# YuvalBahat/Explorable-Super-Resolution

Measured on AMD Instinct MI355X. Metric: HR pixels/sec (RRDB-23 x4, 128->512, bs32 per GPU, fwd + CEM), higher is better.
Workload: dtype bf16x3 (bf16 hi+lo operands = 16 significand bits per operand in every product, three MFMAs, f32 accumulate)

## Files before the change

### explorable-super-resolution_amd/csrc/esr_conv.hip

```cpp
#include "esr_common.h"
#include <type_traits>
#include <vector>

namespace {

constexpr int NW = 4;
constexpr int NTHREADS = 64 * NW;
constexpr int MAXS_BASE = 3;
constexpr int WGS_MT1 = 2, WGS_MT2 = 2;
constexpr int r_of(int mt) { return 3; }
constexpr int maxs_of(int mt) { return r_of(mt) > 3 ? MAXS_BASE + 1 : MAXS_BASE; }

typedef __attribute__((ext_vector_type(4))) unsigned int u32x4;
constexpr int EPI_RES1 = 1, EPI_RES2 = 2, EPI_MASK = 4, EPI_NCHW = 8, EPI_OUT2 = 16;
constexpr int EPI_RESIN = 32;
constexpr int EPI_PS = 64;

struct ConvArgs {
    int tiles_x, tiles_y, ntiles;
    int xcd_q, xcd_r;
    unsigned m_tx, m_ty;
    unsigned i_tx, i_ty;
    int TH, TW, P, NPIX_T, NPIX_L, nslots;
    unsigned m_P, m_ups;
    int H, W, Win_p, ups;
    unsigned share[NW];
    int ncp, lo_chunks, reverse, B;
    DView in0, in1;
    const uint4* wpack;
    long long wchunk;
    long long wslice;
    int wtap;
    int nslices;
    const float* zero_bias;
    int bias_stride;
    const float* bias;
    int cout, ncg_out;
    float act_slope, alpha, beta1, beta2;
    DView res1, res2, out, out2, mask;
    float* out_nchw;
    int mask_cg0, mask_cg1;
    float mask_slope;
    int resin_g0;
    float resin_scale;
    int ps, ps_rg0;
    unsigned m_ns, i_ns;
    int ph_off;
    int ksplit, kz_groups;
    long long kz_slab;
    int nchw_ctot;
    int stages_hint;
    unsigned* range_flag;
    unsigned range_tag;
#ifdef ESR_TRACE
    unsigned long long* trace;
#endif
};

typedef __attribute__((ext_vector_type(8))) _Float16 f16x8;
typedef __attribute__((ext_vector_type(2))) float f32x2;
template <int FMT>
__device__ __forceinline__ f32x16 mfma(uint4 a, uint4 b, f32x16 c) {
    if (FMT) return __builtin_amdgcn_mfma_f32_32x32x16_f16(__builtin_bit_cast(f16x8, a), __builtin_bit_cast(f16x8, b), c, 0, 0, 0);
    return __builtin_amdgcn_mfma_f32_32x32x16_bf16(__builtin_bit_cast(bf16x8, a), __builtin_bit_cast(bf16x8, b), c, 0, 0, 0);
}
template <int FMT>
__device__ __forceinline__ uint32_t cvt_pk(float lo, float hi);

__device__ __forceinline__ uint32_t cvt_pk_bf16(float lo, float hi) {
    uint32_t r;
    asm("v_cvt_pk_bf16_f32 %0, %1, %2" : "=v"(r) : "v"(lo), "v"(hi));
    return r;
}
template <> __device__ __forceinline__ uint32_t cvt_pk<0>(float lo, float hi) { return cvt_pk_bf16(lo, hi); }
template <> __device__ __forceinline__ uint32_t cvt_pk<1>(float lo, float hi) { return f2h(lo) | (f2h(hi) << 16); }

__device__ __forceinline__ void glds16s(const uint4* sbase, unsigned voff, unsigned lds_dst) {
    asm volatile("s_mov_b32 m0, %2\n\ts_nop 0\n\tglobal_load_lds_dwordx4 %0, %1" : : "v"(voff), "s"(sbase), "s"(__builtin_amdgcn_readfirstlane(lds_dst)) : "memory");
}

__device__ __forceinline__ unsigned udiv_magic(unsigned n, unsigned m, unsigned i) { return __umulhi(n, m) + n * i; }

__device__ __forceinline__ const uint4* in_plane(const ConvArgs& a, int g, int b, bool lo) {
    if (g < a.in0.ncg) return (lo ? a.in0.lo : a.in0.hi) + b * a.in0.bs + g * a.in0.cs;
    int g1 = g - a.in0.ncg;
    if (g1 >= a.in1.ncg) g1 = 0;
    return (lo ? a.in1.lo : a.in1.hi) + b * a.in1.bs + g1 * a.in1.cs;
}

template <int MAXS>
struct FetchState {
    unsigned soff[MAXS];
    int slot[MAXS];
};

template <int MAXS>
__device__ __forceinline__ FetchState<MAXS> setup_tile(const ConvArgs& a, int x0, int y0, int wave, int lane) {
    FetchState<MAXS> f;
#pragma unroll
    for (int s = 0; s < MAXS; ++s) {
        f.slot[s] = (wave + s * NW) < a.nslots ? wave + s * NW : wave;
        const unsigned p = (unsigned)f.slot[s] * 64 + lane;
        const unsigned rr = __umul24(p, a.m_P) >> 20, cc = p - rr * a.P;
        const unsigned Yp = y0 + rr, Xp = x0 + cc;
        const bool inb = (p < (unsigned)a.NPIX_T) && (Yp < (unsigned)a.H + 2) && (Xp < (unsigned)a.W + 2);
        const unsigned sy = __umul24(Yp + a.ups - 1, a.m_ups) >> 16, sx = __umul24(Xp + a.ups - 1, a.m_ups) >> 16;
        f.soff[s] = p >= (unsigned)a.NPIX_L ? ~0u : (inb ? (sy * a.Win_p + sx) * 16 : 0);
    }
    return f;
}

template <int NPL>
struct Bases {
    const uint4* p[2 * NPL];
    const uint4* w;
    int wtap;
};
template <int NPL, int MT, int NPW>
__device__ __forceinline__ Bases<NPL> make_bases(const ConvArgs& a, int cp, int b) {
    Bases<NPL> r;
#pragma unroll
    for (int i = 0; i < 2 * NPL; ++i) r.p[i] = in_plane(a, 2 * cp + i / NPL, b, (i % NPL) == 1);
    r.w = a.wpack + (size_t)cp * a.wchunk;
    r.wtap = a.wtap;
    return r;
}

struct DmaShare {
    int nsl;
    int w0, wc;
};
__device__ __forceinline__ DmaShare unpack_share(unsigned w) { return DmaShare{(int)(w & 0xFF), (int)((w >> 8) & 0xFF), (int)(w >> 16)}; }
template <int NPL, int MT = 1, int NPW = 1, int TMODE = 0>
__device__ __forceinline__ int dma_count(const DmaShare& d, bool xlo) { return (xlo ? 2 * NPL : 2) * d.nsl + (TMODE != 0 ? MT * NPW : d.wc); }

template <int NPL, int MT, int NPW, int TMODE = 0>
__device__ __forceinline__ void dma_chunk(const FetchState<maxs_of(MT)>& f, const Bases<NPL>& bs, const DmaShare& d, unsigned stage, int plane_bytes, bool xlo,
                                          int tsel = 0, int wave = 0) {
    constexpr int MAXS = maxs_of(MT);
#pragma unroll
    for (int s = 0; s < MAXS; ++s) {
        if (s >= d.nsl) break;
        const unsigned dst = stage + (unsigned)f.slot[s] * 1024;
        if (f.soff[s] != ~0u) {
#pragma unroll
            for (int cgpl = 0; cgpl < 2 * NPL; ++cgpl) {
                if (!xlo && (cgpl % NPL) == 1) continue;
                glds16s(bs.p[cgpl], f.soff[s], dst + cgpl * plane_bytes);
            }
        }
    }
    const unsigned vlane = (unsigned)(threadIdx.x & 63) * 16;
    if constexpr (TMODE == 0 && MT == 1) {
        for (int j = d.w0; j < d.w0 + d.wc; ++j) glds16s(bs.w + ((j / NPW) * bs.wtap + j % NPW) * 64, vlane, stage + 2 * NPL * plane_bytes + j * 1024);
    } else if constexpr (TMODE == 0) {
        for (int j = d.w0; j < d.w0 + d.wc; ++j) glds16s(bs.w + j * 64, vlane, stage + 2 * NPL * plane_bytes + j * 1024);
    } else {
        static_assert(TMODE == 0 || NW == 4, "one live tap per wave");
#pragma unroll
        for (int m = 0; m < MT; ++m) {
            const int r0 = TMODE == 1 ? 1 - (tsel >> 1) : tsel, c0 = TMODE == 1 ? 1 - (tsel & 1) : m;
            const int tap = (r0 + (wave >> 1)) * 3 + c0 + (wave & 1);
#pragma unroll
            for (int pl = 0; pl < NPW; ++pl) {
                const int j = (tap * MT + m) * NPW + pl;
                glds16s(bs.w + j * 64, vlane, stage + 2 * NPL * plane_bytes + j * 1024);
            }
        }
    }
}

template <int MAXN>
__device__ __forceinline__ void wait_vm_upto(int n) {
#define ESR_VMC(k) case k: if constexpr (k <= MAXN) { asm volatile("s_waitcnt vmcnt(" #k ")" ::: "memory"); break; }
    switch (n) {
        ESR_VMC(1) ESR_VMC(2) ESR_VMC(3) ESR_VMC(4) ESR_VMC(5) ESR_VMC(6) ESR_VMC(7) ESR_VMC(8) ESR_VMC(9) ESR_VMC(10) ESR_VMC(11) ESR_VMC(12)
        ESR_VMC(13) ESR_VMC(14) ESR_VMC(15) ESR_VMC(16) ESR_VMC(17) ESR_VMC(18) ESR_VMC(19) ESR_VMC(20) ESR_VMC(21) ESR_VMC(22) ESR_VMC(23)
        ESR_VMC(24) ESR_VMC(25) ESR_VMC(26) ESR_VMC(27) ESR_VMC(28) ESR_VMC(29) ESR_VMC(30) ESR_VMC(31) ESR_VMC(32)
        default: asm volatile("s_waitcnt vmcnt(0)" ::: "memory"); break;
    }
#undef ESR_VMC
}

struct ResRaw { uint4 h, l; };
__device__ __forceinline__ void swap_halves(const uint4& x, uint32_t (&d)[2][2]) {
    const auto s0 = __builtin_amdgcn_permlane32_swap(x.x, x.z, false, false);
    const auto s1 = __builtin_amdgcn_permlane32_swap(x.y, x.w, false, false);
    d[0][0] = s0[0]; d[0][1] = s1[0]; d[1][0] = s0[1]; d[1][1] = s1[1];
}
template <int FMT>
__device__ __forceinline__ void res_unpack(const ResRaw& q, bool has_lo, f32x2 (&rv)[2][2]) {
    uint32_t d[2][2];
    swap_halves(q.h, d);
#pragma unroll
    for (int k = 0; k < 2; ++k)
#pragma unroll
        for (int j = 0; j < 2; ++j) rv[k][j] = f32x2{e2f<FMT>(d[k][j] & 0xFFFF), e2f<FMT>(d[k][j] >> 16)};
    if (has_lo) {
        swap_halves(q.l, d);
#pragma unroll
        for (int k = 0; k < 2; ++k)
#pragma unroll
            for (int j = 0; j < 2; ++j) rv[k][j] += f32x2{e2f<FMT>(d[k][j] & 0xFFFF), e2f<FMT>(d[k][j] >> 16)};
    }
}

template <int NPL, int MT, int R, int FMT>
__device__ __forceinline__ void resin_accumulate(f32x16 (&acc)[MT][R], const ConvArgs& a, const unsigned char* stage, int cp, bool xlo, int P,
                                                 int plane_bytes, int wave, int lane) {
#pragma unroll
    for (int sgrp = 0; sgrp < 2; ++sgrp) {
        const int og = 2 * cp + sgrp - a.resin_g0;
        if (og < 0 || og * 8 >= a.cout) continue;
        float x[R][4];
#pragma unroll
        for (int r = 0; r < R; ++r) {
            const unsigned char* const pr = stage + sgrp * NPL * plane_bytes + ((wave + r * NW) * 32 + (lane & 31) + P + 1) * 16 + (lane >> 5) * 8;
            const uint2 h = *(const uint2*)pr;
            x[r][0] = e2f<FMT>(h.x & 0xFFFF); x[r][1] = e2f<FMT>(h.x >> 16); x[r][2] = e2f<FMT>(h.y & 0xFFFF); x[r][3] = e2f<FMT>(h.y >> 16);
            if (NPL == 2 && xlo) {
                const uint2 l = *(const uint2*)(pr + plane_bytes);
                x[r][0] += e2f<FMT>(l.x & 0xFFFF); x[r][1] += e2f<FMT>(l.x >> 16); x[r][2] += e2f<FMT>(l.y & 0xFFFF); x[r][3] += e2f<FMT>(l.y >> 16);
            }
        }
        auto add = [&](auto MG) {
            constexpr int mg = decltype(MG)::value;
            if constexpr (mg < MT * 4) {
#pragma unroll
                for (int r = 0; r < R; ++r)
#pragma unroll
                    for (int i = 0; i < 4; ++i) acc[mg / 4][r][(mg % 4) * 4 + i] = fmaf(a.resin_scale, x[r][i], acc[mg / 4][r][(mg % 4) * 4 + i]);
            }
        };
        switch (og) {
            case 0: add(std::integral_constant<int, 0>{}); break;
            case 1: add(std::integral_constant<int, 1>{}); break;
            case 2: add(std::integral_constant<int, 2>{}); break;
            case 3: add(std::integral_constant<int, 3>{}); break;
            case 4: add(std::integral_constant<int, 4>{}); break;
            case 5: add(std::integral_constant<int, 5>{}); break;
            case 6: add(std::integral_constant<int, 6>{}); break;
            default: add(std::integral_constant<int, 7>{}); break;
        }
    }
}

template <int NPL, int MT, int R, int NPW, int FMT, bool XLO, int NTERM_CAP, int TM0 = 0x1FF, int TM1 = 0x1FF>
__device__ __forceinline__ void chunk_mfma(f32x16 (&acc)[MT][R], const unsigned char* sa, const unsigned char* sb, int P, int plane_bytes) {
    constexpr int TMU = TM0 | (MT == 2 ? TM1 : 0);
#define ESR_TAP_LIVE(t, m) ((((m) == 0 ? TM0 : TM1) >> (t)) & 1)
    constexpr int NPB = XLO ? NPL : 1;
    constexpr int NT_FULL = 1 + (NPW == 2 ? 1 : 0) + (NPB == 2 ? 1 : 0);
    constexpr int NTERM = NT_FULL < NTERM_CAP ? NT_FULL : NTERM_CAP;
    constexpr int NM = MT * R * NTERM;
    constexpr int NLA = MT * NPW, NLB = R * NPB, NL = NLA + NLB;
    constexpr int NSLOT = NM > NL ? NM : NL;
    uint4 fa[2][MT][NPW], fb[2][R][NPB];
    auto load_frag = [&](int t, int k, int buf) {
        const int tapoff = ((t / 3) * P + (t % 3)) * 16;
        if (!((TMU >> t) & 1)) return;
        if (k < MT) {
            const int pl = NPW == 2 ? 1 : 0;
            if (ESR_TAP_LIVE(t, k)) fa[buf][k][pl] = *(const uint4*)(sa + ((t * MT + k) * NPW + pl) * 1024);
        } else if (k < MT + R) {
            fb[buf][k - MT][0] = *(const uint4*)(sb + (k - MT) * NW * 512 + tapoff);
        } else if (NPW == 2 && k < 2 * MT + R) {
            const int idx = k - MT - R;
            if (ESR_TAP_LIVE(t, idx)) fa[buf][idx][0] = *(const uint4*)(sa + ((t * MT + idx) * NPW) * 1024);
        } else {
            const int idx = k - (NPW == 2 ? 2 * MT + R : MT + R);
            fb[buf][idx][NPB - 1] = *(const uint4*)(sb + idx * NW * 512 + tapoff + (NPB - 1) * plane_bytes);
        }
    };
#pragma unroll
    for (int k = 0; k < NL; ++k) load_frag(0, k, 0);
#pragma unroll
    for (int t = 0; t < 9; ++t) {
        const int cb = t & 1;
#pragma unroll
        for (int i = 0; i < NSLOT; ++i) {
            if (i < NM) {
                const int ti = i / (MT * R), rem = i % (MT * R), r = rem % R, m = rem / R;
                constexpr int has0 = NPW == 2 ? 1 : 0, has1 = NPB == 2 ? 1 : 0;
                const int skip = NT_FULL - NTERM;
                const int idx = ti + skip;
                const int term = (idx < has0) ? 0 : ((idx < has0 + has1) ? 1 : 2);
                const int pa = term == 0 ? 1 : 0, pb = term == 1 ? 1 : 0;
                if (!ESR_TAP_LIVE(t, m)) {
                } else acc[m][r] = mfma<FMT>(fa[cb][m][pa], fb[cb][r][pb], acc[m][r]);
            }
            if (t < 8 && i < NL) load_frag(t + 1, i, cb ^ 1);
            __builtin_amdgcn_sched_barrier(0);
        }
    }
}

#undef ESR_TAP_LIVE

constexpr int S2D_FWD[4] = {432, 216, 54, 27}, S2D_FLIP[4] = {27, 54, 216, 432};

template <int R>
struct EpiCoord {
    int lim[R];
    unsigned poff[R];
};
template <int R, int KIND>
__device__ __forceinline__ EpiCoord<R> epi_coords(const ConvArgs& a, int x0, int y0, int wave, int lane) {
    EpiCoord<R> e;
    const int half = lane >> 5;
#pragma unroll
    for (int r = 0; r < R; ++r) {
        const unsigned q = (wave + r * NW) * 32 + (lane & 31);
        const unsigned rr = __umul24(q, a.m_P) >> 20, cc = q - rr * a.P;
        const unsigned Y = y0 + rr, X = x0 + cc;
        const bool valid = (rr < (unsigned)a.TH) && (cc < (unsigned)a.TW) && (Y < (unsigned)a.H) && (X < (unsigned)a.W);
        e.lim[r] = valid ? (KIND == 1 ? a.ncg_out : a.ncg_out - half) : (KIND == 1 ? 0 : -1);
        if (KIND == 1) e.poff[r] = (__umul24(Y, a.W) + X) * 4;
        else if (KIND == 2) e.poff[r] = (Y << 16) | X;
        else if (KIND == 3) e.poff[r] = valid ? (__umul24(2 * Y + 1, 2 * a.W + 2) + 2 * X + 1) * 16 : 0;
        else e.poff[r] = valid ? (__umul24(Y + 1, a.W + 2) + X + 1) * 16 : 0;
    }
    return e;
}

template <int NPL, int MT, int R, int EPI, int FMT, bool PARTLO, bool PHASE = false>
__device__ __forceinline__ void conv_epilogue(const ConvArgs& a, f32x16 (&acc)[MT][R], const int b, const EpiCoord<R>& ec, const int lane) {
    constexpr bool HAS_R1 = (EPI & EPI_RES1) != 0, HAS_R2 = (EPI & EPI_RES2) != 0, HAS_MK = (EPI & EPI_MASK) != 0;
    constexpr bool NCHW = (EPI & EPI_NCHW) != 0, OUT2 = (EPI & EPI_OUT2) != 0, PS = (EPI & EPI_PS) != 0;
    const int half = lane >> 5;
    const long long bl = b;
    const f32x2 slope2 = {a.act_slope, a.act_slope}, alpha2 = {a.alpha, a.alpha};
    const char *r1h = nullptr, *r1l = nullptr, *r2h = nullptr, *r2l = nullptr, *mkh = nullptr;
    unsigned h1 = 0, h2 = 0, ho = 0, ho2 = 0;
    if constexpr (HAS_R1) {
        r1h = (const char*)(a.res1.hi + bl * a.res1.bs);
        r1l = a.res1.lo ? (const char*)(a.res1.lo + bl * a.res1.bs) : nullptr;
        h1 = half ? (unsigned)a.res1.cs * 16 : 0;
    }
    if constexpr (HAS_R2) {
        r2h = (const char*)(a.res2.hi + bl * a.res2.bs);
        r2l = a.res2.lo ? (const char*)(a.res2.lo + bl * a.res2.bs) : nullptr;
        h2 = half ? (unsigned)a.res2.cs * 16 : 0;
    }
    if constexpr (HAS_MK) {
        mkh = (const char*)(a.mask.hi + bl * a.mask.bs);
    }
    char *oh = nullptr, *ol = nullptr, *o2h = nullptr, *o2l = nullptr;
    if constexpr (!NCHW) {
        oh = (char*)(a.out.hi + bl * a.out.bs);
        ol = (NPL == 2 && a.out.lo) ? (char*)(a.out.lo + bl * a.out.bs) : nullptr;
        ho = half ? (unsigned)a.out.cs * 16 : 0;
        if constexpr (OUT2) {
            o2h = (char*)(a.out2.hi + bl * a.out2.bs);
            o2l = (NPL == 2 && a.out2.lo) ? (char*)(a.out2.lo + bl * a.out2.bs) : nullptr;
            ho2 = half ? (unsigned)a.out2.cs * 16 : 0;
        }
    }
    constexpr int OPREGS_R = MT * 2 * (((HAS_R1 ? 1 : 0) + (HAS_R2 ? 1 : 0)) * NPL + (HAS_MK ? 1 : 0)) * 4;
    constexpr bool ALL_FIRST = OPREGS_R * R <= 96;
    constexpr int RQ = ALL_FIRST ? R : 1;
    ResRaw q1[HAS_R1 ? RQ : 1][MT * 2], q2[HAS_R2 ? RQ : 1][MT * 2];
    uint4 qm[HAS_MK ? RQ : 1][MT * 2];
    unsigned big = 0;
    auto issue = [&](const int r) {
        const int rq = ALL_FIRST ? r : 0;
#pragma unroll
        for (int mp = 0; mp < MT * 2; ++mp) {
            const int cg0 = mp * 2;
            const bool ok = cg0 < ec.lim[r];
            if constexpr (HAS_R1) {
                const unsigned off = ok ? ec.poff[r] + h1 + cg0 * ((unsigned)a.res1.cs * 16) : 0;
                q1[rq][mp].h = *(const uint4*)(r1h + off);
                if (NPL == 2 && r1l) q1[rq][mp].l = *(const uint4*)(r1l + off);
            }
            if constexpr (HAS_R2) {
                const unsigned off = ok ? ec.poff[r] + h2 + cg0 * ((unsigned)a.res2.cs * 16) : 0;
                q2[rq][mp].h = *(const uint4*)(r2h + off);
                if (NPL == 2 && r2l) q2[rq][mp].l = *(const uint4*)(r2l + off);
            }
            if constexpr (HAS_MK) {
                const int cgm = cg0 + half - a.mask_cg0;
                const bool okm = ok && cgm >= 0 && cg0 + half < a.mask_cg1;
                const unsigned off = okm ? ec.poff[r] + (unsigned)cgm * ((unsigned)a.mask.cs * 16) : 0;
                qm[rq][mp] = *(const uint4*)(mkh + off);
            }
        }
    };
    if constexpr (ALL_FIRST && (HAS_R1 || HAS_R2 || HAS_MK)) {
#pragma unroll
        for (int r = 0; r < R; ++r) issue(r);
    }
#pragma unroll
    for (int r = 0; r < R; ++r) {
        if constexpr (!ALL_FIRST && (HAS_R1 || HAS_R2 || HAS_MK)) issue(r);
        const int rq = ALL_FIRST ? r : 0;
#pragma unroll
        for (int m = 0; m < MT; ++m) {
#pragma unroll
            for (int gp = 0; gp < 2; ++gp) {
                const int cg0 = (PHASE ? 0 : m * 4) + gp * 2;
                if (!(cg0 < ec.lim[r] + (NCHW ? 0 : half))) continue;
                const bool store = cg0 < ec.lim[r];
                f32x2 v[2][2];
#pragma unroll
                for (int k = 0; k < 2; ++k)
#pragma unroll
                    for (int j = 0; j < 2; ++j) {
                        v[k][j] = f32x2{acc[m][r][(gp * 2 + k) * 4 + 2 * j], acc[m][r][(gp * 2 + k) * 4 + 2 * j + 1]} * alpha2;
                        v[k][j] = __builtin_elementwise_max(v[k][j], v[k][j] * slope2);
                    }
                if constexpr (HAS_R1) {
                    f32x2 rv[2][2];
                    res_unpack<FMT>(q1[rq][m * 2 + gp], NPL == 2 && a.res1.lo != nullptr, rv);
                    const f32x2 bb = {a.beta1, a.beta1};
#pragma unroll
                    for (int k = 0; k < 2; ++k)
#pragma unroll
                        for (int j = 0; j < 2; ++j) v[k][j] = __builtin_elementwise_fma(bb, rv[k][j], v[k][j]);
                }
                if constexpr (HAS_R2) {
                    f32x2 rv[2][2];
                    res_unpack<FMT>(q2[rq][m * 2 + gp], NPL == 2 && a.res2.lo != nullptr, rv);
                    const f32x2 bb = {a.beta2, a.beta2};
#pragma unroll
                    for (int k = 0; k < 2; ++k)
#pragma unroll
                        for (int j = 0; j < 2; ++j) v[k][j] = __builtin_elementwise_fma(bb, rv[k][j], v[k][j]);
                }
                if constexpr (HAS_MK) {
                    uint32_t d[2][2];
                    swap_halves(qm[rq][m * 2 + gp], d);
#pragma unroll
                    for (int k = 0; k < 2; ++k) {
                        const int cg = cg0 + k;
                        const float ms = (cg < a.mask_cg0 || cg >= a.mask_cg1) ? 1.f : a.mask_slope;
#pragma unroll
                        for (int j = 0; j < 2; ++j) {
                            const f32x2 s = v[k][j] * f32x2{ms, ms};
                            v[k][j].x = (int)(d[k][j] << 16) > 0 ? v[k][j].x : s.x;
                            v[k][j].y = (int)d[k][j] > 0xFFFF ? v[k][j].y : s.y;
                        }
                    }
                }
                if constexpr (NCHW) {
                    char* const ob = (char*)(a.out_nchw + bl * a.nchw_ctot * a.H * a.W);
                    const unsigned hw4 = (unsigned)(a.H * a.W) * 4;
#pragma unroll
                    for (int k = 0; k < 2; ++k) {
                        const int ch0 = (cg0 + k) * 8 + half * 4;
#pragma unroll
                        for (int i = 0; i < 4; ++i)
                            if (ch0 + i < a.cout) *(float*)(ob + (ec.poff[r] + (unsigned)(ch0 + i) * hw4)) = v[k][i >> 1][i & 1];
                    }
                    continue;
                }
                uint32_t hi[2][2], lo[2][2];
#pragma unroll
                for (int k = 0; k < 2; ++k)
#pragma unroll
                    for (int j = 0; j < 2; ++j) {
                        const uint32_t h = cvt_pk<FMT>(v[k][j].x, v[k][j].y);
                        hi[k][j] = h;
                        if constexpr (FMT == 1) big |= (h & 0x7FFF7FFFu) + 0x08000800u;
                        lo[k][j] = 0;
                        if (NPL == 2) lo[k][j] = cvt_pk<FMT>(v[k][j].x - e2f<FMT>(h & 0xFFFF), v[k][j].y - e2f<FMT>(h >> 16));
                    }
                const auto s0 = __builtin_amdgcn_permlane32_swap(hi[0][0], hi[1][0], false, false);
                const auto s1 = __builtin_amdgcn_permlane32_swap(hi[0][1], hi[1][1], false, false);
                const uint4 hv = make_uint4(s0[0], s1[0], s0[1], s1[1]);
                uint4 lv = hv;
                if (NPL == 2) {
                    const auto t0 = __builtin_amdgcn_permlane32_swap(lo[0][0], lo[1][0], false, false);
                    const auto t1 = __builtin_amdgcn_permlane32_swap(lo[0][1], lo[1][1], false, false);
                    lv = make_uint4(t0[0], t1[0], t0[1], t1[1]);
                }
                unsigned off;
                if constexpr (PS) {
                    const int cgs = cg0 + half, rg = a.ps_rg0 + cgs, r2 = a.ps * a.ps, sp = rg % r2;
                    const int Y = ec.poff[r] >> 16, X = ec.poff[r] & 0xFFFF;
                    off = ((unsigned)(rg / r2) * (unsigned)a.out.cs + (unsigned)(a.ps * Y + sp / a.ps + 1) * (a.ps * a.W + 2) + (a.ps * X + sp % a.ps + 1)) * 16;
                } else off = ec.poff[r] + ho + cg0 * ((unsigned)a.out.cs * 16) + (PHASE ? (unsigned)a.ph_off + m * 16 : 0u);
                if (store) {
                    *(uint4*)(oh + off) = hv;
                    if (NPL == 2 && (!PARTLO || ol)) *(uint4*)(ol + off) = lv;
                    if constexpr (OUT2) {
                        const unsigned off2 = ec.poff[r] + ho2 + cg0 * ((unsigned)a.out2.cs * 16);
                        *(uint4*)(o2h + off2) = hv;
                        if (NPL == 2 && o2l) *(uint4*)(o2l + off2) = lv;
                    }
                }
            }
        }
    }
    if constexpr (FMT == 1 && !NCHW) {
        if (a.range_flag && (big & 0x80008000u)) atomicMin(a.range_flag, a.range_tag);
    }
}

template <int MT>
__device__ __forceinline__ void bias_seed(const float* bias, int half, float (&bz)[MT][16]) {
    typedef const __attribute__((address_space(4))) float* cptr;
    const cptr cb = (cptr)(uintptr_t)bias;
#pragma unroll
    for (int m = 0; m < MT; ++m)
#pragma unroll
        for (int j = 0; j < 4; ++j)
#pragma unroll
            for (int k = 0; k < 4; ++k) {
                const int c0 = (m * 4 + j) * 8;
                const float lo = cb[c0 + k], hi = cb[c0 + 4 + k];
                bz[m][j * 4 + k] = half ? hi : lo;
            }
}

template <int NPL, int MT, int EPI, int NST, int FMT, int NPW, bool PARTLO, int TMODE = 0>
__global__ __launch_bounds__(NTHREADS, NST >= 2 ? 1 : (MT == 1 ? WGS_MT1 : WGS_MT2)) void conv3x3_tile_kernel(const ConvArgs a_in) {
    ConvArgs a = a_in;
    unsigned slice = blockIdx.y, tile3 = 0;
    if constexpr (TMODE == 3) {
        static_assert(TMODE != 3 || (MT == 2 && EPI == 0), "the phase launch: two phases per workgroup, plain epilogue");
        const unsigned xcd3 = blockIdx.x & 7;
        unsigned wg = xcd3 * a.xcd_q + (xcd3 < (unsigned)a.xcd_r ? xcd3 : (unsigned)a.xcd_r) + (blockIdx.x >> 3);
        if (a.reverse) wg = (unsigned)a.ntiles * a.nslices - 1 - wg;
        tile3 = udiv_magic(wg, a.m_ns, a.i_ns);
        slice = wg - tile3 * a.nslices;
        const long long blk = slice >> 1;
        a.wpack += (long long)slice * a.wslice;
        a.bias += blk * 32 * a.bias_stride;
        a.out.hi += blk * 4 * a.out.cs;
        if (a.out.lo) a.out.lo += blk * 4 * a.out.cs;
        a.ncg_out = a.ncg_out - 4 * (int)blk < 4 ? a.ncg_out - 4 * (int)blk : 4;
        a.ph_off = (slice & 1) ? (2 * a.W + 2) * 16 : 0;
    } else {
        const long long sl = blockIdx.y;
        a.wpack += sl * a.wslice;
        a.bias += sl * (MT * 32) * a.bias_stride;
        auto shift = [&](DView& v) { if (v.hi) { v.hi += sl * (MT * 4) * v.cs; if (v.lo) v.lo += sl * (MT * 4) * v.cs; } };
        shift(a.out); shift(a.out2); shift(a.res1); shift(a.res2);
        a.mask_cg0 -= (int)sl * (MT * 4);
        a.mask_cg1 -= (int)sl * (MT * 4);
        if constexpr ((EPI & EPI_RESIN) != 0) a.resin_g0 += (int)sl * (MT * 4);
        if constexpr ((EPI & EPI_NCHW) != 0) {
            a.out_nchw += sl * (MT * 32) * (long long)a.H * a.W;
            if (a.ksplit > 1) {
                const long long kz = blockIdx.z;
                a.in1.hi += kz * a.kz_groups * a.in1.cs;
                if (a.in1.lo) a.in1.lo += kz * a.kz_groups * a.in1.cs;
                a.wpack += kz * a.ncp * (9 * MT * NPW * 64);
                a.out_nchw += kz * a.kz_slab;
                if (kz) a.bias = a.zero_bias;
            }
        }
    }
    static_assert(!PARTLO || NPL == 2, "partial lo needs hi+lo activations");
    static_assert(NPW <= NPL, "a lo weight plane needs hi+lo activations");
    constexpr int R = r_of(MT), MAXS = maxs_of(MT);
    extern __shared__ __attribute__((aligned(16))) unsigned char smem[];
    const int tid = threadIdx.x;
    const int lane = tid & 63;
    const int wave = __builtin_amdgcn_readfirstlane(tid >> 6);
    const int P = a.P;
    const int plane_bytes = a.NPIX_L * 16;
    constexpr int NWI = 9 * MT * NPW;
    constexpr int MAXCNT = 2 * NPL * MAXS + (NWI + NW - 1) / NW;
    const int stage_bytes = 2 * NPL * plane_bytes + NWI * 1024;
    const unsigned xcd = blockIdx.x & 7;
    const unsigned tile_f = xcd * a.xcd_q + (xcd < (unsigned)a.xcd_r ? xcd : (unsigned)a.xcd_r) + (blockIdx.x >> 3);
    const unsigned tile = TMODE == 3 ? tile3 : (a.reverse ? a.ntiles - 1 - tile_f : tile_f);
    const unsigned trow = udiv_magic(tile, a.m_tx, a.i_tx);
    const int b = udiv_magic(trow, a.m_ty, a.i_ty);
    const int x0 = (tile - trow * a.tiles_x) * a.TW, y0 = (trow - b * a.tiles_y) * a.TH;
    const DmaShare share = unpack_share(a_in.share[wave]);
    const unsigned lds0 = (unsigned)(size_t)(__attribute__((address_space(3))) unsigned char*)smem;
#ifdef ESR_TRACE
    unsigned long long* const tr = a.trace ? a.trace + (size_t)blockIdx.x * 128 : nullptr;
    int tslot = 2;
    if (tr && tid == 0) { tr[0] = __builtin_amdgcn_s_getreg((31 << 11) | 4); tr[1] = __builtin_amdgcn_s_getreg((31 << 11) | 20); tr[126] = wall_clock64(); }
#define ESR_TR() do { if (tr && tid == 0 && tslot < 126) tr[tslot++] = __builtin_readcyclecounter(); } while (0)
    ESR_TR();
#else
#define ESR_TR() do { } while (0)
#endif
    const FetchState<MAXS> fs = setup_tile<MAXS>(a, x0, y0, wave, lane);
    ESR_TR();
    static_assert((TMODE != 2 && TMODE != 3) || MT == 2, "M-tile tap masks come in pairs");
    const unsigned char* const sb0 = smem + (lane >> 5) * NPL * plane_bytes + (wave * 32 + (lane & 31)) * 16;
    const unsigned char* const sa0 = smem + 2 * NPL * plane_bytes + lane * 16;
    constexpr int NTERM_CAP = 3;
    auto tsel_of = [&](const int c) { return TMODE == 1 ? ((c >> 1) & 3) : (TMODE == 2 || TMODE == 3 ? (int)(slice & 1) : 0); };
    auto issue = [&](const int c, const unsigned stage, const bool xlo) {
        const Bases<NPL> bs = make_bases<NPL, MT, NPW>(a, c, b);
        dma_chunk<NPL, MT, NPW, TMODE>(fs, bs, share, stage, plane_bytes, xlo, tsel_of(c), wave);
    };
    if (NST == 4) {
        static_assert(NST != 4 || !PARTLO, "the four-stage ring counts its copies per chunk: one count for all chunks");
#pragma unroll
        for (int c = 0; c < 3; ++c)
            if (c < a.ncp) issue(c, lds0 + c * stage_bytes, true);
    }
    constexpr int EKIND = TMODE == 3 ? 3 : ((EPI & EPI_NCHW) ? 1 : ((EPI & EPI_PS) ? 2 : 0));
    constexpr bool EARLY_COORDS = NST >= 2 || (MT == 1 && NPL == 1);
    f32x16 acc[MT][R];
    EpiCoord<R> ec;
    auto seed = [&]() {
        int lane_o = lane;
        asm volatile("" : "+v"(lane_o));
        constexpr int MB = TMODE == 3 ? 1 : MT;
        float bz[MB][16];
        bias_seed<MB>(a.bias, lane_o >> 5, bz);
#pragma unroll
        for (int m = 0; m < MT; ++m)
#pragma unroll
            for (int r = 0; r < R; ++r)
#pragma unroll
                for (int i = 0; i < 16; ++i) acc[m][r][i] = bz[m % MB][i];
        if constexpr (EARLY_COORDS) ec = epi_coords<R, EKIND>(a, x0, y0, wave, lane_o);
    };
    if (NST != 4) issue(0, lds0, !PARTLO || 0 < a.lo_chunks);
    __builtin_amdgcn_sched_barrier(0);
    ESR_TR();
    seed();
    ESR_TR();
    auto step = [&](auto XLO_T, const int cp) {
        constexpr bool xlo = decltype(XLO_T)::value;
        const int st = NST == 4 ? (cp & 3) : (NST >= 2 ? (cp & 1) : 0);
        const unsigned char* const sb = sb0 + st * stage_bytes;
        const unsigned char* const sa = sa0 + st * stage_bytes;
        ESR_TR();
        if (NST == 1) {
            if (cp > 0) issue(cp, lds0, xlo);
            ESR_TR();
            asm volatile("s_waitcnt vmcnt(0)" ::: "memory");
        } else if (NST == 4) {
            if (cp + 3 < a.ncp) issue(cp + 3, lds0 + ((cp + 3) & 3) * stage_bytes, true);
            const int ahead = a.ncp - 1 - cp < 3 ? a.ncp - 1 - cp : 3;
            ESR_TR();
            wait_vm_upto<3 * MAXCNT < 32 ? 3 * MAXCNT : 32>(ahead * dma_count<NPL, MT, NPW, TMODE>(share, true));
        } else {
            const bool more = cp + 1 < a.ncp;
            const bool xlo_next = !PARTLO || cp + 1 < a.lo_chunks;
            if (more) issue(cp + 1, lds0 + ((cp + 1) & 1) * stage_bytes, xlo_next);
            ESR_TR();
            wait_vm_upto<MAXCNT>(more ? dma_count<NPL, MT, NPW, TMODE>(share, xlo_next) : 0);
        }
        ESR_TR();
        __syncthreads();
        ESR_TR();
        if constexpr (TMODE == 1) {
            switch ((cp >> 1) & 3) {
                case 0: chunk_mfma<NPL, MT, R, NPW, FMT, xlo, NTERM_CAP, S2D_FWD[0], S2D_FWD[0]>(acc, sa, sb, P, plane_bytes); break;
                case 1: chunk_mfma<NPL, MT, R, NPW, FMT, xlo, NTERM_CAP, S2D_FWD[1], S2D_FWD[1]>(acc, sa, sb, P, plane_bytes); break;
                case 2: chunk_mfma<NPL, MT, R, NPW, FMT, xlo, NTERM_CAP, S2D_FWD[2], S2D_FWD[2]>(acc, sa, sb, P, plane_bytes); break;
                default: chunk_mfma<NPL, MT, R, NPW, FMT, xlo, NTERM_CAP, S2D_FWD[3], S2D_FWD[3]>(acc, sa, sb, P, plane_bytes); break;
            }
        } else if constexpr (TMODE == 2) {
            if (blockIdx.y & 1) chunk_mfma<NPL, MT, R, NPW, FMT, xlo, NTERM_CAP, S2D_FLIP[2], S2D_FLIP[3]>(acc, sa, sb, P, plane_bytes);
            else chunk_mfma<NPL, MT, R, NPW, FMT, xlo, NTERM_CAP, S2D_FLIP[0], S2D_FLIP[1]>(acc, sa, sb, P, plane_bytes);
        } else if constexpr (TMODE == 3) {
            const int py = slice & 1;
            chunk_mfma<NPL, MT, R, NPW, FMT, xlo, NTERM_CAP, S2D_FLIP[0], S2D_FLIP[1]>(acc, sa + py * (3 * MT * NPW * 1024), sb + py * (P * 16), P, plane_bytes);
        } else {
            chunk_mfma<NPL, MT, R, NPW, FMT, xlo, NTERM_CAP>(acc, sa, sb, P, plane_bytes);
        }
        if constexpr ((EPI & EPI_RESIN) != 0) resin_accumulate<NPL, MT, R, FMT>(acc, a, smem + st * stage_bytes, cp, xlo, P, plane_bytes, wave, lane);
        ESR_TR();
        __syncthreads();
    };
    const int lo_end = PARTLO ? (a.lo_chunks < a.ncp ? a.lo_chunks : a.ncp) : a.ncp;
    for (int cp = 0; cp < lo_end; ++cp) step(std::true_type{}, cp);
    if constexpr (PARTLO)
        for (int cp = lo_end; cp < a.ncp; ++cp) step(std::false_type{}, cp);
    ESR_TR();
    if constexpr (!EARLY_COORDS) ec = epi_coords<R, EKIND>(a, x0, y0, wave, lane);
    conv_epilogue<NPL, MT, R, EPI, FMT, PARTLO, TMODE == 3>(a, acc, b, ec, lane);
    ESR_TR();
#ifdef ESR_TRACE
    if (tr && tid == 0) tr[127] = wall_clock64();
#endif
}

__device__ __forceinline__ float fold2_tap(const float* w9, int t, int phase) {
    const int py = phase >> 1, px = phase & 1, ty = t / 3, tx = t % 3;
    if (ty < py || ty > py + 1 || tx < px || tx > px + 1) return 0.f;
    const int r0 = ty == py ? 0 : py + 1, r1 = ty == py ? py : 2;
    const int c0 = tx == px ? 0 : px + 1, c1 = tx == px ? px : 2;
    float a = w9[r0 * 3 + c0];
    if (r1 != r0) a = __fadd_rn(a, w9[r1 * 3 + c0]);
    if (c1 != c0) {
        float b = w9[r0 * 3 + c1];
        if (r1 != r0) b = __fadd_rn(b, w9[r1 * 3 + c1]);
        a = __fadd_rn(a, b);
    }
    return a;
}
__global__ void pack_weights_kernel(const float* __restrict__ w, int dim0, int dim1, const int* __restrict__ kmap, int ncg_in,
                                    const int* __restrict__ mmap, int mtiles, int transposed, int npl, int f16, float scale, uint4* __restrict__ out, int total) {
    const int idx = blockIdx.x * blockDim.x + threadIdx.x;
    if (idx >= total) return;
    const int lane = idx & 63;
    const int m = (idx >> 6) % mtiles;
    const int ks = (idx >> 6) / mtiles;
    const int cp = ks / 9, t = ks % 9;
    const int cg = 2 * cp + (lane >> 5);
    const int mch = mmap[m * 32 + (lane & 31)];
    float v8[8];
#pragma unroll
    for (int e = 0; e < 8; ++e) {
        const int kch = cg < ncg_in ? kmap[cg * 8 + e] : -1;
        float v = 0.f;
        if (kch >= 0 && mch >= 0) {
            if (transposed >= 2) v = fold2_tap(w + ((long long)mch * dim1 + kch) * 9, t, (transposed - 2 + m) & 3);
            else v = transposed ? w[((long long)kch * dim1 + mch) * 9 + (8 - t)] : w[((long long)mch * dim1 + kch) * 9 + t];
        }
        v8[e] = v * scale;
    }
    uint4* o = out + ((size_t)(ks * mtiles + m) * npl) * 64 + lane;
    store8(o, npl == 2 ? o + 64 : nullptr, 0, v8, f16 ? ESR_FMT_F16 : ESR_FMT_BF16);
}

struct PackEntry {
    const float* w; const int* kmap; const int* mmap; uint4* out;
    int dim0, dim1, ncg_in, mtiles, transposed, npl, f16, total; float scale;
};
__global__ __launch_bounds__(256) void pack_weights_batch_kernel(const PackEntry* __restrict__ table, const int2* __restrict__ map) {
    constexpr int PITCH = 16 * 9 + 1;
    __shared__ float tile[32 * PITCH];
    __shared__ int kch_s[16], mch_s[32];
    const int2 m = map[blockIdx.x];
    const PackEntry e = table[m.x];
    const int cp = m.y / e.mtiles, mt = m.y % e.mtiles;
    if (threadIdx.x < 16) {
        const int cg = 2 * cp + (threadIdx.x >> 3);
        kch_s[threadIdx.x] = cg < e.ncg_in ? e.kmap[cg * 8 + (threadIdx.x & 7)] : -1;
    } else if (threadIdx.x >= 32 && threadIdx.x < 64) mch_s[threadIdx.x - 32] = e.mmap[mt * 32 + (threadIdx.x - 32)];
    __syncthreads();
#pragma unroll
    for (int j = 0; j < 18; ++j) {
        const int f = j * 256 + threadIdx.x;
        int mr, kc, t;
        if (e.transposed == 1) { kc = f / 288; const int c = f - kc * 288; mr = c / 9; t = 8 - (c - mr * 9); }
        else { mr = f / 144; const int c = f - mr * 144; kc = c / 9; t = c - kc * 9; }
        const int kch = kch_s[kc], mch = mch_s[mr];
        float v = 0.f;
        if (kch >= 0 && mch >= 0) v = e.transposed == 1 ? e.w[((long long)kch * e.dim1 + mch) * 9 + (8 - t)] : e.w[((long long)mch * e.dim1 + kch) * 9 + t];
        tile[mr * PITCH + kc * 9 + t] = v;
    }
    __syncthreads();
    for (int v = threadIdx.x; v < 9 * 64; v += 256) {
        const int t = v >> 6, lane = v & 63;
        const float* src = tile + (lane & 31) * PITCH + (lane >> 5) * 72 + t;
        float x8[8];
#pragma unroll
        for (int c = 0; c < 8; ++c) x8[c] = (e.transposed >= 2 ? fold2_tap(src + c * 9 - t, t, (e.transposed - 2 + mt) & 3) : src[c * 9]) * e.scale;
        uint4* o = e.out + ((size_t)((cp * 9 + t) * e.mtiles + mt) * e.npl) * 64 + lane;
        store8(o, e.npl == 2 ? o + 64 : nullptr, 0, x8, e.f16 ? ESR_FMT_F16 : ESR_FMT_BF16);
    }
}

struct TileCfg { int TH, TW, P, NPIX_T, NPIX_L, tiles_x, tiles_y; size_t lds; };
constexpr size_t stage_bytes(int npl, int npix_l, int mt, int npw) { return (size_t)2 * npl * npix_l * 16 + (size_t)9 * mt * npw * 1024; }

TileCfg pick_tile_search(int H, int W, int npl, int mt, int nwg);
TileCfg pick_tile(int H, int W, int npl, int mt, int nwg) {
    struct Entry { int H, W, npl, mt, nwg; TileCfg cfg; };
    static thread_local Entry cache[8];
    static thread_local int next = 0;
    for (const Entry& e : cache)
        if (e.H == H && e.W == W && e.npl == npl && e.mt == mt && e.nwg == nwg && e.cfg.P) return e.cfg;
    Entry& e = cache[next];
    next = (next + 1) % 8;
    e = Entry{H, W, npl, mt, nwg, pick_tile_search(H, W, npl, mt, nwg)};
    return e.cfg;
}
TileCfg pick_tile_search(int H, int W, int npl, int mt, int nwg) {
    const int R = r_of(mt), MAXS = maxs_of(mt);
    TileCfg best{};
    double best_cost = -1;
    const size_t budget = 160 * 1024;
    const int max_px = 32 * NW * R;
    for (int ntx = 1; ntx <= W; ++ntx) {
        const int TW = (W + ntx - 1) / ntx;
        const int P = TW + 2;
        if (P > max_px) continue;
        if (ntx > 1 && TW < 6) break;
        int THmax = max_px / P;
        if (THmax > H) THmax = H;
        for (int TH = THmax; TH >= 1 && TH >= THmax - 6; --TH) {
            const int npix_t = (TH + 2) * P;
            int npix_l = max_px + 2 * P + 2;
            if (npix_l < npix_t) npix_l = npix_t;
            if (npix_l > MAXS * NW * 64) continue;
            const size_t lds = nwg * stage_bytes(npl, npix_l, mt, npl);
            if (lds > budget) continue;
            const int nty = (H + TH - 1) / TH;
            const double halo = (double)(TH + 2) * P / ((double)TH * TW);
            const double cost = (double)ntx * nty * (1.0 + 0.05 * halo);
            if (best_cost < 0 || cost < best_cost) {
                best_cost = cost;
                best = TileCfg{TH, TW, P, npix_t, npix_l, ntx, nty, lds};
            }
        }
    }
    return best;
}

#ifdef ESR_TRACE
unsigned long long* g_trace = nullptr;
#endif

__device__ float g_zero_bias[64];
const float* zero_bias() {
    static const float* ptr[64] = {};
    int dev = 0;
    (void)hipGetDevice(&dev);
    const float*& p = ptr[dev & 63];
    if (!p) {
        void* q = nullptr;
        if (hipGetSymbolAddress(&q, HIP_SYMBOL(g_zero_bias)) != hipSuccess) return nullptr;
        p = (const float*)q;
    }
    return p;
}

void dma_share_host(int npl, int nwi, int nslots, unsigned (&out)[NW]) {
    const int target = (2 * npl * nslots + nwi + NW - 1) / NW;
    int start = 0;
    for (int v = 0; v < NW; ++v) {
        const int nv = nslots > v ? (nslots - v + NW - 1) / NW : 0;
        int c = target - 2 * npl * nv;
        c = c < 0 ? 0 : c;
        if (c > nwi - start || v == NW - 1) c = nwi - start;
        out[v] = (unsigned)nv | ((unsigned)start << 8) | ((unsigned)c << 16);
        start += c;
    }
}

constexpr int CONV_SMALL_WGS = 320;

struct ConvPlan {
    bool phases, mslice;
    int npl, ps, nslices, mt;
    int mt_k, kslices;
    TileCfg tile;
    int ups, fmt, wpl;
    bool partlo;
    int in0g, ncp, lo_chunks;
    int tmode, epi, nst, S;
    int resin_g0;
    float resin_scale;
    dim3 grid;
    size_t lds;
};

template <int... V> struct Ints {};
template <int... V> constexpr bool among(Ints<V...>, int v) { return ((v == V) || ...); }

typedef Ints<0, EPI_RES1, EPI_RES1 | EPI_RES2, EPI_RESIN, EPI_RESIN | EPI_RES2, EPI_NCHW, EPI_OUT2, EPI_RES1 | EPI_MASK, EPI_MASK, EPI_PS> ConvEpis;
constexpr bool has_ring4(int mt, int epi, int fmt, bool partlo, int tmode) { return (epi == 0 || epi == EPI_NCHW) && !partlo && fmt == 0 && mt == 2 && tmode != 3; }
constexpr bool two_stages_only(int npl, int tmode) { return (tmode == 1 || tmode == 2) && npl == 2; }

constexpr bool conv_kernel_exists(int npl, int mt, int epi, int nst, int fmt, int npw, bool partlo, int tmode) {
    if (fmt == 0 ? (npw != npl || partlo) : (npw > npl || (partlo && npl == 1))) return false;
    if (nst == 4 ? !has_ring4(mt, epi, fmt, partlo, tmode) : (nst == 1 && two_stages_only(npl, tmode))) return false;
    if (tmode == 0) return among(ConvEpis{}, epi);
    if (mt != 2 || partlo) return false;
    return tmode == 3 ? epi == 0 : (fmt == 0 && (epi == 0 || epi == EPI_NCHW));
}

typedef void (*ConvKernel)(const ConvArgs);
template <int NPL, int MT, int EPI, int NST, int FMT, int NPW, int PARTLO, int TMODE>
ConvKernel conv_pick(Ints<NPL, MT, EPI, NST, FMT, NPW, PARTLO, TMODE>, const int*) {
    if constexpr (conv_kernel_exists(NPL, MT, EPI, NST, FMT, NPW, PARTLO != 0, TMODE)) {
        ConvKernel k = conv3x3_tile_kernel<NPL, MT, EPI, NST, FMT, NPW, PARTLO != 0, TMODE>;
        ESR_ALLOW_160K_LDS(k);
        return k;
    } else return nullptr;
}
template <int... C, int... V, class... More>
ConvKernel conv_pick(Ints<C...>, const int* v, Ints<V...>, More... more) {
    ConvKernel k = nullptr;
    ((*v == V ? void(k = conv_pick(Ints<C..., V>{}, v + 1, more...)) : void()), ...);
    return k;
}
ConvKernel conv_kernel(const ConvPlan& p) {
    const int v[8] = {p.npl, p.mt_k, p.epi, p.nst, p.fmt, p.wpl, p.partlo, p.tmode};
    return conv_pick(Ints<>{}, v, Ints<1, 2>{}, Ints<1, 2>{}, ConvEpis{}, Ints<1, 2, 4>{}, Ints<0, 1>{}, Ints<1, 2>{}, Ints<0, 1>{}, Ints<0, 1, 2, 3>{});
}

__global__ void splitk_finish_kernel(const float* __restrict__ ws, int S, long long slab, DView out, int C, int H, int W, long long total) {
    const long long idx = (long long)blockIdx.x * blockDim.x + threadIdx.x;
    if (idx >= total) return;
    const ActPos q = act_pos(idx, C >> 3, H, W);
    const int b = q.b, cg = q.cg, y = q.y, x = q.x;
    float v8[8];
#pragma unroll
    for (int e = 0; e < 8; ++e) {
        const float* p = ws + ((long long)(b * C + cg * 8 + e) * H + y) * W + x;
        float v = 0.f;
        for (int k = 0; k < S; ++k) v += p[k * slab];
        v8[e] = v;
    }
    store8(mut(out.hi), mut(out.lo), act_off(out.bs, out.cs, W, b, cg, y, x), v8, ESR_FMT_BF16);
}

}

#ifdef ESR_TRACE
extern "C" void esr_debug_trace(void* buf) { g_trace = (unsigned long long*)buf; }
#endif

extern "C" size_t esr_conv_wpack_bytes(int ncg_in, int cout, int split) {
    const int ncp = (ncg_in + 1) / 2, mt = (cout + 31) / 32;
    return (size_t)ncp * 9 * mt * ((split == 1 || split == 3) ? 2 : 1) * 64 * 16;
}

extern "C" int esr_pack_conv_weights(const float* w, int cout_w, int cin_w, const int32_t* kmap, int ncg_in, const int32_t* mmap,
                                     int mtiles, int transposed, int split, float scale, void* wpack, esr_stream_t stream) {
    if (!w || !kmap || !mmap || !wpack || ncg_in <= 0 || mtiles <= 0 || transposed < 0 || transposed > 5) return ESR_E_ARG;
    const int ncp = (ncg_in + 1) / 2;
    const int total = ncp * 9 * mtiles * 64;
    ESR_CLEAR_ERR();
    hipLaunchKernelGGL(pack_weights_kernel, dim3((total + 255) / 256), dim3(256), 0, (hipStream_t)stream, w, cout_w, cin_w, kmap,
                       ncg_in, mmap, mtiles, transposed, (split == 1 || split == 3) ? 2 : 1, split >= 2 ? 1 : 0, scale, (uint4*)wpack, total);
    ESR_CHECK_LAUNCH();
    return ESR_OK;
}

static int64_t pack_batch_blocks(const esr_pack_desc* descs, int n) {
    int64_t nb = 0;
    for (int i = 0; i < n; ++i) {
        if (!descs[i].w || !descs[i].kmap || !descs[i].mmap || !descs[i].wpack || descs[i].ncg_in <= 0 || descs[i].mtiles <= 0 || descs[i].transposed < 0 ||
            descs[i].transposed > 5)
            return ESR_E_ARG;
        nb += (int64_t)((descs[i].ncg_in + 1) / 2) * descs[i].mtiles;
    }
    return nb;
}

extern "C" int64_t esr_pack_batch_workspace_bytes(const esr_pack_desc* descs, int n) {
    if (!descs || n <= 0) return ESR_E_ARG;
    const int64_t nb = pack_batch_blocks(descs, n);
    if (nb < 0) return nb;
    return ((int64_t)n * sizeof(PackEntry) + 255) / 256 * 256 + nb * (int64_t)sizeof(int2);
}

extern "C" int64_t esr_pack_batch_upload(const esr_pack_desc* descs, int n, void* workspace, int64_t workspace_bytes, esr_stream_t stream) {
    if (!descs || n <= 0 || !workspace) return ESR_E_ARG;
    const int64_t need = esr_pack_batch_workspace_bytes(descs, n);
    if (need < 0 || workspace_bytes < need) return ESR_E_ARG;
    const int64_t nb = pack_batch_blocks(descs, n);
    std::vector<PackEntry> table(n);
    std::vector<int2> map((size_t)nb);
    int64_t b = 0;
    for (int i = 0; i < n; ++i) {
        PackEntry& e = table[i];
        e.w = descs[i].w; e.kmap = descs[i].kmap; e.mmap = descs[i].mmap; e.out = (uint4*)descs[i].wpack;
        e.dim0 = descs[i].cout_w; e.dim1 = descs[i].cin_w; e.ncg_in = descs[i].ncg_in; e.mtiles = descs[i].mtiles;
        e.transposed = descs[i].transposed; e.npl = (descs[i].split == 1 || descs[i].split == 3) ? 2 : 1; e.f16 = descs[i].split >= 2 ? 1 : 0; e.scale = descs[i].scale;
        e.total = ((descs[i].ncg_in + 1) / 2) * 9 * descs[i].mtiles * 64;
        for (int j = 0; j < ((descs[i].ncg_in + 1) / 2) * descs[i].mtiles; ++j) map[(size_t)b++] = make_int2(i, j);
    }
    const size_t tb = ((size_t)n * sizeof(PackEntry) + 255) / 256 * 256;
    hipStream_t s = (hipStream_t)stream;
    if (hipMemcpyAsync(workspace, table.data(), (size_t)n * sizeof(PackEntry), hipMemcpyHostToDevice, s) != hipSuccess) return ESR_E_LAUNCH;
    if (hipMemcpyAsync((char*)workspace + tb, map.data(), (size_t)nb * sizeof(int2), hipMemcpyHostToDevice, s) != hipSuccess) return ESR_E_LAUNCH;
    return nb;
}

extern "C" int esr_pack_batch_run(const void* workspace, int n, int64_t nblocks, esr_stream_t stream) {
    if (!workspace || n <= 0 || nblocks <= 0) return ESR_E_ARG;
    const size_t tb = ((size_t)n * sizeof(PackEntry) + 255) / 256 * 256;
    ESR_CLEAR_ERR();
    hipLaunchKernelGGL(pack_weights_batch_kernel, dim3((unsigned)nblocks), dim3(256), 0, (hipStream_t)stream, (const PackEntry*)workspace,
                       (const int2*)((const char*)workspace + tb));
    ESR_CHECK_LAUNCH();
    return ESR_OK;
}


static bool all_taps(const int32_t (&m)[4]) { return (m[0] == 0 || m[0] == 0x1FF) && (m[1] == 0 || m[1] == 0x1FF) && (m[2] == 0 || m[2] == 0x1FF) && (m[3] == 0 || m[3] == 0x1FF); }
static bool same_taps(const int32_t (&m)[4], const int (&p)[4]) { return m[0] == p[0] && m[1] == p[1] && m[2] == p[2] && m[3] == p[3]; }

static int conv_validate(const esr_conv3x3_desc* d) {
    if (!d || !d->in1.hi || !d->wpack || d->B <= 0 || d->H <= 0 || d->W <= 0 || d->cout <= 0) return ESR_E_ARG;
    if (!d->out.hi && !d->out_nchw) return ESR_E_ARG;
    const int ups = d->upsample <= 0 ? 1 : d->upsample;
    if (ups > 8 || ups == 5 || ups == 7) return ESR_E_UNSUPPORTED;
    if (ups > 1 && d->in0.hi) return ESR_E_UNSUPPORTED;
    if (d->upsample_phases != 0 && d->upsample_phases != 2) return ESR_E_UNSUPPORTED;
    const bool phases = d->upsample_phases == 2;
    if (phases) {
        if (ups > 1) return ESR_E_ARG;
        if (d->in0.hi || d->res1.hi || d->res2.hi || d->mask_src.hi || d->out2.hi || d->out_nchw || d->pixel_shuffle > 1) return ESR_E_UNSUPPORTED;
        if (!d->out.hi || d->out.H != 2 * d->H || d->out.W != 2 * d->W) return ESR_E_ARG;
    }
    if (d->in1.H * ups != d->H || d->in1.W * ups != d->W) return ESR_E_ARG;
    if (d->in0.hi && (d->in0.H != d->H || d->in0.W != d->W)) return ESR_E_ARG;
    const bool split = d->in1.lo != nullptr;
    if ((d->in0.hi && d->in0.fmt != d->in1.fmt) || (d->out.hi && d->out.fmt != d->in1.fmt) || (d->out2.hi && d->out2.fmt != d->in1.fmt) ||
        (d->res1.hi && d->res1.fmt != d->in1.fmt) || (d->res2.hi && d->res2.fmt != d->in1.fmt))
        return ESR_E_ARG;
    if (d->in0.hi && ((d->in0.lo != nullptr) != split)) return ESR_E_ARG;
    if (!phases && d->cout > 64 && (d->cout % 64 || d->out_nchw || d->pixel_shuffle > 1 || !d->out.hi)) return ESR_E_UNSUPPORTED;
    const int ps = d->pixel_shuffle > 1 ? d->pixel_shuffle : 0;
    if (ps) {
        if (!d->out.hi || d->out_nchw || d->out2.hi || d->res1.hi || d->res2.hi || d->mask_src.hi || d->cout % 8) return ESR_E_UNSUPPORTED;
        if (d->out.H != ps * d->H || d->out.W != ps * d->W || (d->ps_rowgroup0 + d->cout / 8 + ps * ps - 1) / (ps * ps) > d->out.ncg) return ESR_E_ARG;
    } else if (!phases && d->out.hi && (d->out.H != d->H || d->out.W != d->W)) return ESR_E_ARG;
    if (!ps && d->out.hi && d->out.ncg * 8 < d->cout) return ESR_E_ARG;
    if (d->out.hi && d->out.lo && !split) return ESR_E_ARG;
    if (d->out2.hi && (!d->out.hi || (d->out2.lo && !d->out.lo))) return ESR_E_ARG;
    if (d->act_slope < 0.f || d->act_slope > 1.f || !(d->alpha >= 0.f)) return ESR_E_ARG;
    auto fits = [](const esr_act_view& v) { return !v.hi || (long long)v.ncg * v.cg_stride * 16 < 0x100000000ll; };
    if (d->H + 2 >= 32768 || d->W + 2 >= 32768 || !fits(d->in0) || !fits(d->in1) || !fits(d->out) || !fits(d->out2) || !fits(d->res1) || !fits(d->res2) ||
        !fits(d->mask_src) || (d->out_nchw && (long long)d->cout * d->H * d->W * 4 >= 0x100000000ll))
        return ESR_E_UNSUPPORTED;
    return ESR_OK;
}

static int conv_plan_shape(const esr_conv3x3_desc* d, ConvPlan& p) {
    p.phases = d->upsample_phases == 2;
    if (!p.phases && d->cout > 64 && d->cout % 64) return ESR_E_UNSUPPORTED;
    p.nslices = p.phases ? 2 * ((d->cout + 31) / 32) : (d->cout > 64 ? d->cout / 64 : 1);
    p.mt = p.nslices > 1 ? 2 : (d->cout + 31) / 32;
    p.npl = d->in1.lo ? 2 : 1;
    p.ps = d->pixel_shuffle > 1 ? d->pixel_shuffle : 0;
    p.mslice = false;
    if (p.nslices == 1 && p.mt == 2 && d->cout == 64 && !d->out_nchw && !p.ps && d->lds_stages == 0 && !d->k_split_ws && all_taps(d->tap_mask_k) &&
        all_taps(d->tap_mask_m) && (!d->mask_src.hi || (d->mask_cg0 == 0 && d->mask_cg1 >= 8))) {
        const TileCfg t2 = pick_tile(d->H, d->W, p.npl, 2, WGS_MT2);
        p.mslice = t2.TH != 0 && (long long)t2.tiles_x * t2.tiles_y * d->B <= CONV_SMALL_WGS;
    }
    p.mt_k = p.mslice ? 1 : p.mt;
    p.kslices = p.mslice ? 2 : p.nslices;
    p.tile = pick_tile(d->H, d->W, p.npl, p.mt_k, p.mt_k == 1 ? WGS_MT1 : WGS_MT2);
    return p.tile.TH ? ESR_OK : ESR_E_UNSUPPORTED;
}

static int conv_plan(const esr_conv3x3_desc* d, ConvPlan& p) {
    if (int rc = conv_plan_shape(d, p)) return rc;
    const TileCfg& t = p.tile;
    const bool split = p.npl == 2, f16 = d->in1.fmt == ESR_FMT_F16;
    const int ntiles = t.tiles_x * t.tiles_y * d->B;
    if ((p.phases && (long long)ntiles * p.nslices * p.nslices >= 0x100000000ll) || (long long)ntiles * t.tiles_x >= 0x100000000ll ||
        (long long)d->B * t.tiles_y * t.tiles_y >= 0x100000000ll)
        return ESR_E_UNSUPPORTED;
    const int ncg_all = (d->cout + 7) >> 3;
    if ((d->res1.hi && d->res1.ncg < ncg_all) || (d->res2.hi && d->res2.ncg < ncg_all)) return ESR_E_ARG;
    if (d->mask_src.hi && d->mask_src.ncg < (d->mask_cg1 < ncg_all ? d->mask_cg1 : ncg_all) - d->mask_cg0) return ESR_E_ARG;
    p.ups = d->upsample <= 0 ? 1 : d->upsample;
    p.fmt = f16 ? 1 : 0;
    p.in0g = d->in0.hi ? d->in0.ncg : 0;
    p.ncp = (p.in0g + d->in1.ncg + 1) / 2;

    p.epi = d->res1.hi ? EPI_RES1 : 0;
    if (p.nslices == 1 && d->res1.hi && d->act_slope == 1.f && d->alpha != 0.f && p.ups == 1 && !d->mask_src.hi && !d->out_nchw &&
        d->res1.batch_stride == d->in1.batch_stride && d->res1.cg_stride == d->in1.cg_stride && ((d->res1.lo != nullptr) == split) &&
        d->in1_lo_groups >= 0) {
        const long long unit = (long long)d->in1.cg_stride * 16;
        const long long off = (const char*)d->res1.hi - (const char*)d->in1.hi;
        const bool lo_ok = !split || ((const char*)d->res1.lo - (const char*)d->in1.lo) == off;
        if (lo_ok && off >= 0 && off % unit == 0 && off / unit + (d->cout + 7) / 8 <= d->in1.ncg) {
            p.resin_g0 = p.in0g + (int)(off / unit);
            p.resin_scale = d->beta1 / d->alpha;
            p.epi = EPI_RESIN;
        }
    }
    p.epi |= (d->res2.hi ? EPI_RES2 : 0) | (d->mask_src.hi ? EPI_MASK : 0) | (d->out_nchw ? EPI_NCHW : 0) | (d->out2.hi ? EPI_OUT2 : 0) | (p.ps ? EPI_PS : 0);
    if ((p.epi & EPI_NCHW) && d->out.hi) return ESR_E_UNSUPPORTED;
    p.wpl = d->weight_planes ? d->weight_planes : (f16 ? 1 : p.npl);
    if (p.wpl < 1 || p.wpl > p.npl || (!f16 && p.wpl != p.npl)) return ESR_E_ARG;
    p.lo_chunks = p.ncp;
    p.partlo = split && (d->in1_lo_groups < 0 || (d->in1_lo_groups > 0 && d->in1_lo_groups < d->in1.ncg) || (d->out.hi && !d->out.lo));
    if (split && d->in1_lo_groups > 0 && d->in1_lo_groups < d->in1.ncg) p.lo_chunks = (p.in0g + d->in1_lo_groups + 1) / 2;
    if (split && d->in1_lo_groups < 0) p.lo_chunks = 0;
    if (p.partlo && !f16) return ESR_E_UNSUPPORTED;
    if (p.phases && p.partlo) return ESR_E_UNSUPPORTED;
    if (!among(ConvEpis{}, p.epi) || (f16 && p.epi == (EPI_RES1 | EPI_MASK))) return ESR_E_UNSUPPORTED;

    const bool plain = p.epi == 0 && !f16 && !p.partlo && p.mt == 2 && p.in0g == 0;
    const bool tm1 = plain && same_taps(d->tap_mask_k, S2D_FWD) && d->tap_mask_k_shift == 1 && all_taps(d->tap_mask_m) && (d->in1.ncg % 4) == 0;
    const bool tm2 = plain && !tm1 && same_taps(d->tap_mask_m, S2D_FLIP) && all_taps(d->tap_mask_k);
    p.tmode = p.phases ? 3 : (tm1 ? 1 : (tm2 ? 2 : 0));
    const int gslices = p.mslice || (p.nslices > 1 && p.ncp) ? p.kslices : 1;
    p.S = 1;
    if (!p.phases && plain && d->k_split_ws && d->act_slope == 1.f && p.ups == 1 && d->cout % 64 == 0) {
        const long long slab = (long long)d->B * d->cout * d->H * d->W, wgs = (long long)ntiles * p.nslices;
        for (int c = 8; c >= 2 && p.S == 1; c /= 2) {
            if (p.ncp % c || p.ncp / c < 8 || (tm1 && (p.ncp / c) % 8)) continue;
            if (wgs * c <= CONV_SMALL_WGS && slab * c <= d->k_split_ws_floats) p.S = c;
        }
        if (p.S > 1) p.epi = EPI_NCHW;
    }

    const int force = (d->lds_stages == 1 || d->lds_stages == 2) ? d->lds_stages : 0;
    const bool small = ntiles * gslices * p.S <= CONV_SMALL_WGS;
    const size_t stage = stage_bytes(p.npl, t.NPIX_L, p.mt_k, p.wpl);
    if (has_ring4(p.mt_k, p.epi, p.fmt, p.partlo, p.tmode) && !force && small && p.ncp / p.S >= (p.epi == EPI_NCHW ? 8 : 16) && 4 * stage <= 160 * 1024) p.nst = 4;
    else if (two_stages_only(p.npl, p.tmode)) p.nst = 2;
    else p.nst = force ? force : (small ? 2 : 1);
    p.lds = p.nst * stage;
    p.grid = p.tmode == 3 ? dim3(ntiles * gslices) : dim3(ntiles, gslices, p.S);
    return ESR_OK;
}

static ConvArgs conv_args(const esr_conv3x3_desc* d, const ConvPlan& p, const float* zero) {
    const TileCfg& t = p.tile;
    ConvArgs a{};
    a.in0 = to_dview(d->in0); a.in1 = to_dview(d->in1);
    a.ups = p.ups; a.Win_p = d->in1.W + 2;
    a.wpack = (const uint4*)d->wpack;
    a.zero_bias = zero;
    a.bias = d->bias ? d->bias : zero; a.bias_stride = d->bias ? 1 : 0;
    a.cout = p.mslice ? 32 : (p.nslices > 1 && !p.phases ? 64 : d->cout);
    a.nslices = p.kslices;
    a.B = d->B; a.H = d->H; a.W = d->W;
    a.TH = t.TH; a.TW = t.TW; a.P = t.P; a.NPIX_T = t.NPIX_T; a.NPIX_L = t.NPIX_L;
    a.tiles_x = t.tiles_x; a.tiles_y = t.tiles_y;
    a.ntiles = a.tiles_x * a.tiles_y * a.B;
    const long long wgs = p.phases ? (long long)a.ntiles * p.nslices : a.ntiles;
    a.xcd_q = (int)(wgs / 8); a.xcd_r = (int)(wgs % 8);
    if (p.phases) a.m_ns = (unsigned)((0x100000000ull + p.nslices - 1) / p.nslices);
    a.m_tx = a.tiles_x == 1 ? 0 : (unsigned)((0x100000000ull + a.tiles_x - 1) / a.tiles_x);
    a.m_ty = a.tiles_y == 1 ? 0 : (unsigned)((0x100000000ull + a.tiles_y - 1) / a.tiles_y);
    a.i_tx = a.tiles_x == 1; a.i_ty = a.tiles_y == 1;
    a.m_P = ((1u << 20) + a.P - 1) / a.P; a.m_ups = ((1u << 16) + p.ups - 1) / p.ups;
    a.nslots = (a.NPIX_L + 63) / 64;
    a.ncg_out = (a.cout + 7) >> 3;
    a.ncp = p.ncp / p.S; a.lo_chunks = p.lo_chunks;
    a.act_slope = d->act_slope; a.alpha = d->alpha; a.beta1 = d->beta1; a.beta2 = d->beta2;
    a.res1 = to_dview(d->res1); a.res2 = to_dview(d->res2); a.mask = to_dview(d->mask_src);
    a.out = to_dview(d->out); a.out2 = to_dview(d->out2);
    a.out_nchw = d->out_nchw; a.nchw_ctot = d->cout;
    a.mask_cg0 = d->mask_cg0; a.mask_cg1 = d->mask_cg1; a.mask_slope = d->mask_slope;
    a.resin_g0 = p.resin_g0; a.resin_scale = p.resin_scale;
    a.reverse = d->reverse_order;
    a.stages_hint = (d->lds_stages == 1 || d->lds_stages == 2) ? d->lds_stages : 0;
    a.range_flag = p.fmt ? d->range_flag : nullptr; a.range_tag = d->range_tag;
    a.ps = p.ps; a.ps_rg0 = d->ps_rowgroup0;
#ifdef ESR_TRACE
    a.trace = g_trace;
#endif
    a.wslice = p.mslice ? (long long)p.wpl * 64 : (p.nslices > 1 ? (long long)p.ncp * 9 * 2 * p.wpl * 64 : 0);
    a.wchunk = (long long)9 * p.mt * p.wpl * 64;
    a.wtap = p.mt * p.wpl;
    dma_share_host(p.npl, 9 * p.mt_k * p.wpl, a.nslots, a.share);
    if (p.S > 1) {
        a.ksplit = p.S;
        a.kz_groups = 2 * a.ncp;
        a.in1.ncg = a.kz_groups;
        a.kz_slab = (long long)d->B * d->cout * d->H * d->W;
        a.out_nchw = d->k_split_ws;
    }
    return a;
}

static int conv_launch(const esr_conv3x3_desc* d, const ConvPlan& p, const ConvArgs& a, hipStream_t s) {
    const ConvKernel k = conv_kernel(p);
    if (!k) return ESR_E_UNSUPPORTED;
    ESR_CLEAR_ERR();
    hipLaunchKernelGGL(k, p.grid, dim3(NTHREADS), p.lds, s, a);
    ESR_CHECK_LAUNCH();
    if (p.S > 1) {
        const long long total = (long long)d->B * (d->cout / 8) * d->H * d->W;
        ESR_CLEAR_ERR();
        hipLaunchKernelGGL(splitk_finish_kernel, dim3((unsigned)((total + 255) / 256)), dim3(256), 0, s, (const float*)d->k_split_ws, p.S, a.kz_slab, a.out,
                           d->cout, d->H, d->W, total);
        ESR_CHECK_LAUNCH();
    }
    return ESR_OK;
}

extern "C" int esr_conv3x3_tiling(const esr_conv3x3_desc* d, int32_t* tiling) {
    if (!d || !tiling || d->B <= 0 || d->H <= 0 || d->W <= 0 || d->cout <= 0) return ESR_E_ARG;
    ConvPlan p{};
    if (int rc = conv_plan_shape(d, p)) return rc;
    tiling[0] = p.tile.tiles_x; tiling[1] = p.tile.tiles_y;
    tiling[2] = p.mt_k; tiling[3] = p.kslices;
    return ESR_OK;
}

extern "C" int esr_conv3x3(const esr_conv3x3_desc* d, esr_stream_t stream) {
    if (int rc = conv_validate(d)) return rc;
    ConvPlan p{};
    if (int rc = conv_plan(d, p)) return rc;
    const float* zero = zero_bias();
    if (!zero) return ESR_E_LAUNCH;
    return conv_launch(d, p, conv_args(d, p, zero), (hipStream_t)stream);
}
```

### explorable-super-resolution_amd/csrc/esr_run.hip

```cpp
#include "esr_common.h"

extern "C" int esr_run(const esr_cmd* cmds, int n, int* failed, esr_stream_t stream) {
    if (failed) *failed = -1;
    if (n < 0 || (n > 0 && !cmds)) return ESR_E_ARG;
    for (int i = 0; i < n; ++i) {
        const esr_cmd& c = cmds[i];
        int rc;
        switch (c.op) {
            case ESR_OP_CONV3X3: rc = esr_conv3x3(&c.u.conv, stream); break;
            case ESR_OP_PACK_NCHW: {
                const esr_cmd_pack_nchw& a = c.u.pack_nchw;
                rc = esr_pack_nchw(a.src, a.src_batch_stride, a.B, a.C, a.h, a.w, a.c0, a.nc, a.pad, a.down, &a.dst, stream);
            } break;
            case ESR_OP_UNPACK_GRAD_NCHW: {
                const esr_cmd_unpack_grad_nchw& a = c.u.unpack_grad_nchw;
                rc = esr_unpack_grad_nchw(&a.G, a.dst, a.dst_batch_stride, a.B, a.C, a.h, a.w, a.c0, a.nc, a.pad, a.down, a.accumulate, stream);
            } break;
            case ESR_OP_ACT_COMBINE: {
                const esr_cmd_act_combine& a = c.u.act_combine;
                rc = esr_act_combine(a.A.hi ? &a.A : nullptr, a.alpha, a.Bv.hi ? &a.Bv : nullptr, a.beta, a.s, a.mask.hi ? &a.mask : nullptr, a.mask_slope,
                                     &a.out, a.B, stream);
            } break;
            case ESR_OP_PIXEL_UNSHUFFLE: rc = esr_pixel_unshuffle(&c.u.pixel_unshuffle.src, c.u.pixel_unshuffle.r, &c.u.pixel_unshuffle.dst, c.u.pixel_unshuffle.B, stream); break;
            case ESR_OP_GRAD_ABSMAX: rc = esr_grad_absmax(&c.u.grad_absmax.v, c.u.grad_absmax.B, c.u.grad_absmax.slot, stream); break;
            case ESR_OP_GRAD_SCALE: {
                const esr_cmd_grad_scale& a = c.u.grad_scale;
                rc = esr_grad_scale(&a.src, &a.dst, a.B, a.slot, a.exp, a.scale_in, a.scale_den, a.scale_out, stream);
            } break;
            case ESR_OP_WGRAD_BATCH_RUN: rc = esr_conv3x3_wgrad_batch_run(c.u.wgrad_batch_run.workspace, &c.u.wgrad_batch_run.plan, stream); break;
            case ESR_OP_PACK_BATCH_RUN: rc = esr_pack_batch_run(c.u.pack_batch_run.workspace, c.u.pack_batch_run.n, c.u.pack_batch_run.nblocks, stream); break;
            case ESR_OP_ZERO: rc = esr_zero(c.u.zero.p, c.u.zero.n16, stream); break;
            case ESR_OP_UNPACK_NCHW: rc = esr_unpack_nchw(&c.u.unpack_nchw.src, c.u.unpack_nchw.B, c.u.unpack_nchw.nc, c.u.unpack_nchw.dst, stream); break;
            case ESR_OP_WGRAD: rc = esr_conv3x3_wgrad(&c.u.wgrad, stream); break;
            case ESR_OP_BN_REDUCE: rc = esr_bn_reduce(&c.u.bn.d, c.u.bn.mode, c.u.bn.sums, stream); break;
            case ESR_OP_BN_APPLY: rc = esr_bn_apply(&c.u.bn.d, c.u.bn.mode, stream); break;
            case ESR_OP_BN_FINALIZE: {
                const esr_cmd_bn_finalize& a = c.u.bn_finalize;
                rc = esr_bn_finalize(a.sums, a.groups, a.C, a.n_per_group, a.eps, a.momentum, a.gamma, a.beta, a.mean, a.rstd, a.scale, a.shift, a.running_mean,
                                     a.running_var, stream);
            } break;
            case ESR_OP_BN_PARAM_GRADS: {
                const esr_cmd_bn_param_grads& a = c.u.bn_param_grads;
                rc = esr_bn_param_grads(a.sums2, a.sums3, a.rstd, a.groups, a.C, a.n_per_group, a.dgamma, a.dbeta, a.g_gamma, stream);
            } break;
            case ESR_OP_BN_FINALIZE_APPLY: rc = esr_bn_finalize_apply(&c.u.bn_finalize_apply.d, &c.u.bn_finalize_apply.f, stream); break;
            default: rc = ESR_E_ARG;
        }
        if (rc != ESR_OK) {
            if (failed) *failed = i;
            return rc;
        }
    }
    return ESR_OK;
}

extern "C" int64_t esr_cmd_bytes(void) { return (int64_t)sizeof(esr_cmd); }
```

### explorable-super-resolution_amd/esr_hip/_lib.py

```python
import ctypes as C
import os

_HERE = os.path.dirname(os.path.abspath(__file__))
_LIB_NAME = 'libesr_hip.so'


class EsrError(RuntimeError):
    pass


class ActView(C.Structure):
    _fields_ = [('hi', C.c_void_p), ('lo', C.c_void_p), ('ncg', C.c_int32), ('H', C.c_int32), ('W', C.c_int32),
                ('batch_stride', C.c_int64), ('cg_stride', C.c_int64), ('fmt', C.c_int32)]


class Conv3x3Desc(C.Structure):
    _fields_ = [('in0', ActView), ('in1', ActView), ('upsample', C.c_int32), ('wpack', C.c_void_p), ('bias', C.c_void_p),
                ('cout', C.c_int32), ('B', C.c_int32), ('H', C.c_int32), ('W', C.c_int32),
                ('act_slope', C.c_float), ('alpha', C.c_float),
                ('res1', ActView), ('beta1', C.c_float), ('res2', ActView), ('beta2', C.c_float),
                ('out', ActView), ('out2', ActView), ('out_nchw', C.c_void_p),
                ('mask_src', ActView), ('mask_cg0', C.c_int32), ('mask_cg1', C.c_int32), ('mask_slope', C.c_float),
                ('reverse_order', C.c_int32), ('weight_planes', C.c_int32), ('in1_lo_groups', C.c_int32),
                ('pixel_shuffle', C.c_int32), ('ps_rowgroup0', C.c_int32), ('tap_mask_k', C.c_int32 * 4), ('tap_mask_k_shift', C.c_int32),
                ('tap_mask_m', C.c_int32 * 4), ('k_split_ws', C.c_void_p), ('k_split_ws_floats', C.c_int64), ('lds_stages', C.c_int32),
                ('range_flag', C.c_void_p), ('range_tag', C.c_uint32), ('upsample_phases', C.c_int32)]


class WgradDesc(C.Structure):
    _fields_ = [('dy', ActView), ('x', ActView), ('xlat', ActView), ('lat', C.c_int32), ('upsample', C.c_int32), ('cout', C.c_int32),
                ('cin_main', C.c_int32), ('B', C.c_int32), ('H', C.c_int32), ('W', C.c_int32), ('alpha', C.c_float), ('dw', C.c_void_p),
                ('db', C.c_void_p), ('workspace', C.c_void_p), ('workspace_floats', C.c_int64), ('tap_masks', C.c_int32 * 4)]


class WgradBatchPlan(C.Structure):
    _fields_ = [('nwg', C.c_int64), ('table_bytes', C.c_int64), ('n', C.c_int32), ('max_red', C.c_int32), ('split', C.c_int32), ('f16', C.c_int32), ('s2d', C.c_int32), ('reserved', C.c_int32)]


class PackDesc(C.Structure):
    _fields_ = [('w', C.c_void_p), ('cout_w', C.c_int32), ('cin_w', C.c_int32), ('kmap', C.c_void_p), ('ncg_in', C.c_int32), ('mmap', C.c_void_p),
                ('mtiles', C.c_int32), ('transposed', C.c_int32), ('split', C.c_int32), ('scale', C.c_float), ('wpack', C.c_void_p)]


class BnDesc(C.Structure):
    _fields_ = [('y', ActView), ('dz', ActView), ('u', ActView), ('out0', ActView), ('out1', ActView), ('B', C.c_int32), ('groups', C.c_int32),
                ('C', C.c_int32), ('scale', C.c_void_p), ('shift', C.c_void_p), ('mean', C.c_void_p), ('rstd', C.c_void_p), ('gamma', C.c_void_p),
                ('sums2', C.c_void_p), ('sums3', C.c_void_p), ('slope', C.c_float), ('const_stats', C.c_int32), ('s2d', C.c_int32)]


class AdamTensor(C.Structure):
    _fields_ = [('p', C.c_void_p), ('g', C.c_void_p), ('m', C.c_void_p), ('v', C.c_void_p), ('n', C.c_int64)]


OP_CONV3X3, OP_PACK_NCHW, OP_UNPACK_GRAD_NCHW, OP_ACT_COMBINE, OP_PIXEL_UNSHUFFLE, OP_GRAD_ABSMAX, OP_GRAD_SCALE, OP_WGRAD_BATCH_RUN, \
    OP_PACK_BATCH_RUN, OP_ZERO, OP_UNPACK_NCHW, OP_WGRAD, OP_BN_REDUCE, OP_BN_APPLY, OP_BN_FINALIZE, OP_BN_PARAM_GRADS, \
    OP_BN_FINALIZE_APPLY = range(1, 18)


class CmdPackNchw(C.Structure):
    _fields_ = [('src', C.c_void_p), ('src_batch_stride', C.c_int64), ('B', C.c_int32), ('C', C.c_int32), ('h', C.c_int32), ('w', C.c_int32),
                ('c0', C.c_int32), ('nc', C.c_int32), ('pad', C.c_int32), ('down', C.c_int32), ('dst', ActView)]


class CmdUnpackGradNchw(C.Structure):
    _fields_ = [('G', ActView), ('dst', C.c_void_p), ('dst_batch_stride', C.c_int64), ('B', C.c_int32), ('C', C.c_int32), ('h', C.c_int32),
                ('w', C.c_int32), ('c0', C.c_int32), ('nc', C.c_int32), ('pad', C.c_int32), ('down', C.c_int32), ('accumulate', C.c_int32)]


class CmdActCombine(C.Structure):
    _fields_ = [('A', ActView), ('alpha', C.c_float), ('Bv', ActView), ('beta', C.c_float), ('s', C.c_int32), ('mask', ActView),
                ('mask_slope', C.c_float), ('out', ActView), ('B', C.c_int32)]


class CmdPixelUnshuffle(C.Structure):
    _fields_ = [('src', ActView), ('r', C.c_int32), ('dst', ActView), ('B', C.c_int32)]


class CmdGradAbsmax(C.Structure):
    _fields_ = [('v', ActView), ('B', C.c_int32), ('slot', C.c_void_p)]


class CmdGradScale(C.Structure):
    _fields_ = [('src', ActView), ('dst', ActView), ('B', C.c_int32), ('slot', C.c_void_p), ('exp', C.c_int32), ('scale_in', C.c_void_p),
                ('scale_den', C.c_void_p), ('scale_out', C.c_void_p)]


class CmdWgradBatchRun(C.Structure):
    _fields_ = [('workspace', C.c_void_p), ('plan', WgradBatchPlan)]


class CmdPackBatchRun(C.Structure):
    _fields_ = [('workspace', C.c_void_p), ('n', C.c_int32), ('nblocks', C.c_int64)]


class CmdZero(C.Structure):
    _fields_ = [('p', C.c_void_p), ('n16', C.c_int64)]


class CmdUnpackNchw(C.Structure):
    _fields_ = [('src', ActView), ('B', C.c_int32), ('nc', C.c_int32), ('dst', C.c_void_p)]


class CmdBn(C.Structure):
    _fields_ = [('d', BnDesc), ('mode', C.c_int32), ('sums', C.c_void_p)]


class CmdBnFinalize(C.Structure):
    _fields_ = [('sums', C.c_void_p), ('groups', C.c_int32), ('C', C.c_int32), ('n_per_group', C.c_int64), ('eps', C.c_float), ('momentum', C.c_float),
                ('gamma', C.c_void_p), ('beta', C.c_void_p), ('mean', C.c_void_p), ('rstd', C.c_void_p), ('scale', C.c_void_p), ('shift', C.c_void_p),
                ('running_mean', C.c_void_p), ('running_var', C.c_void_p)]


class CmdBnFinalizeApply(C.Structure):
    _fields_ = [('d', BnDesc), ('f', CmdBnFinalize)]


class CmdBnParamGrads(C.Structure):
    _fields_ = [('sums2', C.c_void_p), ('sums3', C.c_void_p), ('rstd', C.c_void_p), ('groups', C.c_int32), ('C', C.c_int32), ('n_per_group', C.c_int64),
                ('dgamma', C.c_void_p), ('dbeta', C.c_void_p), ('g_gamma', C.c_void_p)]


class CmdUnion(C.Union):
    _fields_ = [('conv', Conv3x3Desc), ('pack_nchw', CmdPackNchw), ('unpack_grad_nchw', CmdUnpackGradNchw), ('act_combine', CmdActCombine),
                ('pixel_unshuffle', CmdPixelUnshuffle), ('grad_absmax', CmdGradAbsmax), ('grad_scale', CmdGradScale),
                ('wgrad_batch_run', CmdWgradBatchRun), ('pack_batch_run', CmdPackBatchRun), ('zero', CmdZero), ('unpack_nchw', CmdUnpackNchw),
                ('wgrad', WgradDesc), ('bn', CmdBn), ('bn_finalize', CmdBnFinalize), ('bn_param_grads', CmdBnParamGrads), ('bn_finalize_apply', CmdBnFinalizeApply)]


class Cmd(C.Structure):
    _fields_ = [('op', C.c_int32), ('reserved', C.c_int32), ('u', CmdUnion)]


CMD_MEMBER = {OP_CONV3X3: 'conv', OP_PACK_NCHW: 'pack_nchw', OP_UNPACK_GRAD_NCHW: 'unpack_grad_nchw', OP_ACT_COMBINE: 'act_combine',
              OP_PIXEL_UNSHUFFLE: 'pixel_unshuffle', OP_GRAD_ABSMAX: 'grad_absmax', OP_GRAD_SCALE: 'grad_scale',
              OP_WGRAD_BATCH_RUN: 'wgrad_batch_run', OP_PACK_BATCH_RUN: 'pack_batch_run', OP_ZERO: 'zero', OP_UNPACK_NCHW: 'unpack_nchw',
              OP_WGRAD: 'wgrad', OP_BN_REDUCE: 'bn', OP_BN_APPLY: 'bn', OP_BN_FINALIZE: 'bn_finalize', OP_BN_PARAM_GRADS: 'bn_param_grads', OP_BN_FINALIZE_APPLY: 'bn_finalize_apply'}


_SIGS = {
    'esr_bn_reduce': (C.c_int, [C.POINTER(BnDesc), C.c_int, C.c_void_p, C.c_void_p]),
    'esr_bn_apply': (C.c_int, [C.POINTER(BnDesc), C.c_int, C.c_void_p]),
    'esr_bn_finalize_apply': (C.c_int, [C.POINTER(BnDesc), C.POINTER(CmdBnFinalize), C.c_void_p]),
    'esr_bn_finalize': (C.c_int, [C.c_void_p, C.c_int, C.c_int, C.c_int64, C.c_float, C.c_float, C.c_void_p, C.c_void_p, C.c_void_p, C.c_void_p, C.c_void_p,
                                  C.c_void_p, C.c_void_p, C.c_void_p, C.c_void_p]),
    'esr_bn_param_grads': (C.c_int, [C.c_void_p, C.c_void_p, C.c_void_p, C.c_int, C.c_int, C.c_int64, C.c_void_p, C.c_void_p, C.c_void_p, C.c_void_p]),
    'esr_adam_workspace_bytes': (C.c_int64, [C.POINTER(AdamTensor), C.c_int]),
    'esr_adam_upload': (C.c_int64, [C.POINTER(AdamTensor), C.c_int, C.c_void_p, C.c_int64, C.c_void_p]),
    'esr_adam_table': (C.c_int64, [C.POINTER(AdamTensor), C.c_int, C.c_void_p, C.c_int64]),
    'esr_adam_run': (C.c_int, [C.c_void_p, C.c_int, C.c_int64, C.c_float, C.c_float, C.c_float, C.c_float, C.c_float, C.c_float, C.c_float, C.c_void_p]),
    'esr_run': (C.c_int, [C.POINTER(Cmd), C.c_int, C.POINTER(C.c_int), C.c_void_p]),
    'esr_cmd_bytes': (C.c_int64, []),
    'esr_version': (C.c_int, []),
    'esr_conv3x3': (C.c_int, [C.POINTER(Conv3x3Desc), C.c_void_p]),
    'esr_conv3x3_tiling': (C.c_int, [C.POINTER(Conv3x3Desc), C.POINTER(C.c_int32)]),
    'esr_pixel_unshuffle': (C.c_int, [C.POINTER(ActView), C.c_int, C.POINTER(ActView), C.c_int, C.c_void_p]),
    'esr_conv_wpack_bytes': (C.c_size_t, [C.c_int, C.c_int, C.c_int]),
    'esr_pack_conv_weights': (C.c_int, [C.c_void_p, C.c_int, C.c_int, C.c_void_p, C.c_int, C.c_void_p, C.c_int, C.c_int, C.c_int,
                                        C.c_float, C.c_void_p, C.c_void_p]),
    'esr_pack_batch_workspace_bytes': (C.c_int64, [C.POINTER(PackDesc), C.c_int]),
    'esr_pack_batch_upload': (C.c_int64, [C.POINTER(PackDesc), C.c_int, C.c_void_p, C.c_int64, C.c_void_p]),
    'esr_pack_batch_run': (C.c_int, [C.c_void_p, C.c_int, C.c_int64, C.c_void_p]),
    'esr_pack_nchw': (C.c_int, [C.c_void_p, C.c_int64, C.c_int, C.c_int, C.c_int, C.c_int, C.c_int, C.c_int, C.c_int, C.c_int,
                                C.POINTER(ActView), C.c_void_p]),
    'esr_unpack_nchw': (C.c_int, [C.POINTER(ActView), C.c_int, C.c_int, C.c_void_p, C.c_void_p]),
    'esr_zero': (C.c_int, [C.c_void_p, C.c_int64, C.c_void_p]),
    'esr_act_combine': (C.c_int, [C.POINTER(ActView), C.c_float, C.POINTER(ActView), C.c_float, C.c_int, C.POINTER(ActView), C.c_float,
                                  C.POINTER(ActView), C.c_int, C.c_void_p]),
    'esr_grad_absmax': (C.c_int, [C.POINTER(ActView), C.c_int, C.c_void_p, C.c_void_p]),
    'esr_grad_scale': (C.c_int, [C.POINTER(ActView), C.POINTER(ActView), C.c_int, C.c_void_p, C.c_int, C.c_void_p, C.c_void_p, C.c_void_p, C.c_void_p]),
    'esr_unpack_grad_nchw': (C.c_int, [C.POINTER(ActView), C.c_void_p, C.c_int64, C.c_int, C.c_int, C.c_int, C.c_int, C.c_int, C.c_int, C.c_int,
                                       C.c_int, C.c_int, C.c_void_p]),
    'esr_cem_adjoint': (C.c_int, [C.c_void_p, C.c_int, C.c_int, C.c_int, C.c_int, C.c_int, C.c_int, C.c_int, C.c_int, C.c_void_p, C.c_int,
                                  C.c_int, C.c_int, C.c_int, C.c_int, C.c_void_p, C.c_int, C.c_void_p]),
    'esr_cem_adjoint_sep': (C.c_int, [C.c_void_p, C.c_int, C.c_int, C.c_int, C.c_int, C.c_int, C.c_int, C.c_int, C.c_int, C.c_void_p, C.c_void_p, C.c_int,
                                      C.c_int, C.c_int, C.c_int, C.c_int, C.c_void_p, C.c_void_p, C.c_float, C.c_void_p, C.c_void_p]),
    'esr_conv3x3_wgrad': (C.c_int, [C.POINTER(WgradDesc), C.c_void_p]),
    'esr_conv3x3_wgrad_workspace_floats': (C.c_int64, [C.POINTER(WgradDesc)]),
    'esr_conv3x3_wgrad_tiling': (C.c_int, [C.POINTER(WgradDesc), C.POINTER(C.c_int32)]),
    'esr_conv3x3_wgrad_batch_workspace_bytes': (C.c_int64, [C.POINTER(WgradDesc), C.c_int]),
    'esr_conv3x3_wgrad_batch': (C.c_int, [C.POINTER(WgradDesc), C.c_int, C.c_void_p, C.c_int64, C.c_void_p]),
    'esr_conv3x3_wgrad_batch_upload': (C.c_int, [C.POINTER(WgradDesc), C.c_int, C.c_void_p, C.c_int64, C.POINTER(WgradBatchPlan), C.c_void_p]),
    'esr_conv3x3_wgrad_batch_unit': (C.c_int64, [C.POINTER(WgradDesc), C.c_int]),
    'esr_conv3x3_wgrad_batch_part_workspace_bytes': (C.c_int64, [C.POINTER(WgradDesc), C.c_int, C.c_int64]),
    'esr_conv3x3_wgrad_batch_part_upload': (C.c_int, [C.POINTER(WgradDesc), C.c_int, C.c_void_p, C.c_int64, C.POINTER(WgradBatchPlan), C.c_int64, C.c_void_p]),
    'esr_conv3x3_wgrad_batch_run': (C.c_int, [C.c_void_p, C.POINTER(WgradBatchPlan), C.c_void_p]),
    'esr_conv3x3_wgrad_batch_run_side': (C.c_int, [C.c_void_p, C.POINTER(WgradBatchPlan), C.c_void_p]),
    'esr_conv3x3_wgrad_side_occupancy': (C.c_int, [C.c_int]),
    'esr_conv3x3_wgrad_batch_rebase': (C.c_int, [C.c_void_p, C.POINTER(WgradBatchPlan), C.c_int64, C.c_void_p]),
    'esr_soft_hist_slabs': (C.c_int64, [C.c_int64]),
    'esr_soft_hist_fwd': (C.c_int, [C.c_void_p, C.c_int64, C.c_int, C.c_float, C.c_float, C.c_float, C.c_float, C.c_void_p, C.c_void_p]),
    'esr_soft_hist_bwd': (C.c_int, [C.c_void_p, C.c_int64, C.c_int, C.c_float, C.c_float, C.c_float, C.c_float, C.c_void_p, C.c_void_p, C.c_void_p]),
    'esr_kde_dim_supported': (C.c_int, [C.c_int]),
    'esr_kde_fwd': (C.c_int, [C.c_void_p, C.c_int64, C.c_void_p, C.c_void_p, C.c_int, C.c_int, C.c_float, C.c_float, C.c_void_p, C.c_void_p, C.c_void_p]),
    'esr_kde_bwd': (C.c_int, [C.c_void_p, C.c_int64, C.c_void_p, C.c_int, C.c_void_p, C.c_int, C.c_int, C.c_int, C.c_int, C.c_float, C.c_float,
                              C.c_void_p, C.c_void_p, C.c_void_p, C.c_void_p, C.c_void_p, C.c_void_p]),
    'esr_kde_dedup': (C.c_int, [C.c_void_p, C.c_int, C.c_int, C.c_float, C.c_void_p, C.c_void_p]),
    'esr_img_stats': (C.c_int, [C.c_void_p, C.c_int, C.c_int, C.c_int, C.c_int, C.c_void_p, C.c_int, C.c_int, C.c_void_p, C.c_void_p]),
    'esr_img_stats_grad': (C.c_int, [C.c_void_p, C.c_int, C.c_int, C.c_int, C.c_int, C.c_void_p, C.c_int, C.c_int, C.c_void_p, C.c_void_p, C.c_int, C.c_void_p]),
    'esr_patch_std': (C.c_int, [C.c_void_p, C.c_int, C.c_int, C.c_int, C.c_int, C.c_void_p, C.c_void_p, C.c_void_p, C.c_void_p]),
    'esr_patch_std_grad': (C.c_int, [C.c_void_p, C.c_int, C.c_int, C.c_int, C.c_int, C.c_void_p, C.c_void_p, C.c_void_p, C.c_void_p, C.c_void_p, C.c_int,
                                     C.c_void_p]),
    'esr_shift_l1': (C.c_int, [C.c_void_p, C.c_int, C.c_int, C.c_int, C.c_int, C.c_void_p, C.c_int, C.c_int, C.c_void_p, C.c_void_p, C.c_void_p, C.c_void_p,
                               C.c_void_p, C.c_void_p]),
    'esr_shift_l1_grad': (C.c_int, [C.c_void_p, C.c_int, C.c_int, C.c_int, C.c_int, C.c_void_p, C.c_int, C.c_int, C.c_void_p, C.c_void_p, C.c_void_p,
                                    C.c_void_p, C.c_void_p, C.c_void_p, C.c_void_p, C.c_void_p, C.c_void_p, C.c_int, C.c_void_p]),
    'esr_scribble': (C.c_int, [C.c_void_p, C.c_int, C.c_int, C.c_int, C.c_int, C.c_void_p, C.c_void_p, C.c_void_p, C.c_int, C.c_void_p, C.c_void_p]),
    'esr_scribble_grad': (C.c_int, [C.c_void_p, C.c_int, C.c_int, C.c_int, C.c_int, C.c_void_p, C.c_void_p, C.c_void_p, C.c_int, C.c_void_p, C.c_float,
                                    C.c_void_p, C.c_int, C.c_void_p]),
    'esr_patch_mag_blocks': (C.c_int64, [C.c_int, C.c_int]),
    'esr_patch_mag': (C.c_int, [C.c_void_p, C.c_int, C.c_int, C.c_int, C.c_int, C.c_void_p, C.c_void_p, C.c_int, C.c_void_p, C.c_void_p]),
    'esr_patch_mag_grad': (C.c_int, [C.c_void_p, C.c_int, C.c_int, C.c_int, C.c_int, C.c_void_p, C.c_void_p, C.c_int, C.c_void_p, C.c_void_p, C.c_int,
                                     C.c_void_p]),
    'esr_pairmin_blocks': (C.c_int64, [C.c_int, C.c_int, C.c_int]),
    'esr_pairmin_work_floats': (C.c_int64, [C.c_int, C.c_int, C.c_int, C.c_int, C.c_int, C.c_int, C.c_int]),
    'esr_pairmin': (C.c_int, [C.c_void_p, C.c_int, C.c_int, C.c_int, C.c_int, C.c_int, C.c_int, C.c_int, C.c_void_p, C.c_void_p, C.c_int, C.c_float,
                              C.c_void_p, C.c_void_p, C.c_void_p]),
    'esr_pairmin_grad': (C.c_int, [C.c_void_p, C.c_int, C.c_int, C.c_int, C.c_int, C.c_int, C.c_int, C.c_int, C.c_void_p, C.c_void_p, C.c_int, C.c_float,
                                   C.c_float, C.c_void_p, C.c_void_p, C.c_void_p]),
    'esr_cem_downscale': (C.c_int, [C.c_void_p, C.c_int, C.c_int, C.c_int, C.c_int, C.c_int, C.c_int, C.c_void_p, C.c_int,
                                    C.c_void_p, C.c_int, C.c_void_p, C.c_void_p]),
    'esr_cem_lrfilter': (C.c_int, [C.c_void_p, C.c_int, C.c_int, C.c_int, C.c_int, C.c_void_p, C.c_int, C.c_void_p, C.c_void_p]),
    'esr_cem_upscale': (C.c_int, [C.c_void_p, C.c_void_p, C.c_int, C.c_int, C.c_int, C.c_int, C.c_int, C.c_int, C.c_void_p, C.c_int,
                                  C.c_void_p, C.c_int, C.c_int, C.c_float, C.c_void_p, C.c_void_p, C.c_void_p]),
    'esr_cem_downscale_sep': (C.c_int, [C.c_void_p, C.c_int, C.c_int, C.c_int, C.c_int, C.c_int, C.c_int, C.c_void_p, C.c_void_p, C.c_int,
                                        C.c_void_p, C.c_int, C.c_void_p, C.c_void_p]),
    'esr_cem_lrfilter_sep': (C.c_int, [C.c_void_p, C.c_int, C.c_int, C.c_int, C.c_int, C.c_void_p, C.c_void_p, C.c_int, C.c_void_p, C.c_void_p]),
    'esr_cem_upscale_sep': (C.c_int, [C.c_void_p, C.c_void_p, C.c_int, C.c_int, C.c_int, C.c_int, C.c_int, C.c_int, C.c_void_p, C.c_void_p, C.c_int,
                                      C.c_void_p, C.c_int, C.c_int, C.c_float, C.c_void_p, C.c_void_p, C.c_void_p]),
    'esr_cem_filter_upscale_sep': (C.c_int, [C.c_void_p, C.c_void_p, C.c_int, C.c_int, C.c_int, C.c_int, C.c_int, C.c_int, C.c_void_p, C.c_void_p, C.c_int,
                                             C.c_void_p, C.c_void_p, C.c_int, C.c_void_p, C.c_int, C.c_int, C.c_float, C.c_void_p, C.c_void_p, C.c_void_p]),
    'esr_cem_sep_form': (C.c_int, [C.c_int, C.c_int, C.c_int, C.c_int, C.c_int, C.c_int]),
    'esr_pack_nchw_norm': (C.c_int, [C.c_void_p, C.c_int, C.c_int, C.c_int, C.c_int, C.c_void_p, C.c_void_p, C.POINTER(ActView), C.c_void_p]),
    'esr_unpack_grad_nchw_norm': (C.c_int, [C.POINTER(ActView), C.c_int, C.c_int, C.c_void_p, C.c_void_p, C.c_void_p]),
    'esr_maxpool2x2': (C.c_int, [C.POINTER(ActView), C.POINTER(ActView), C.c_int, C.c_void_p]),
    'esr_maxpool2x2_grad': (C.c_int, [C.POINTER(ActView), C.POINTER(ActView), C.c_int, C.POINTER(ActView), C.c_int, C.c_void_p]),
    'esr_jpeg_compress': (C.c_int, [C.c_void_p, C.c_int, C.c_int, C.c_int, C.c_void_p, C.c_int, C.c_void_p, C.POINTER(ActView), C.c_void_p]),
    'esr_jpeg_extract': (C.c_int, [C.c_void_p, C.c_void_p, C.c_int, C.c_int, C.c_int, C.c_void_p, C.c_void_p, C.c_void_p, C.c_void_p]),
    'esr_jpeg_extract_grad': (C.c_int, [C.c_void_p, C.c_void_p, C.c_int, C.c_int, C.c_int, C.c_void_p, C.c_void_p, C.c_void_p, C.c_void_p]),
    'esr_jpeg_compress_grad': (C.c_int, [C.c_void_p, C.c_int, C.c_int, C.c_int, C.c_void_p, C.c_void_p, C.c_void_p]),
    'esr_jpeg16_compress': (C.c_int, [C.c_void_p, C.c_int, C.c_int, C.c_int, C.c_void_p, C.c_int, C.c_void_p, C.c_void_p]),
    'esr_jpeg16_extract': (C.c_int, [C.c_void_p, C.c_int, C.c_int, C.c_void_p, C.c_int, C.c_int, C.c_int, C.c_int, C.c_void_p, C.c_void_p, C.c_void_p,
                                     C.c_void_p]),
    'esr_jpeg16_extract_grad': (C.c_int, [C.c_void_p, C.c_void_p, C.c_int, C.c_int, C.c_int, C.c_int, C.c_void_p, C.c_void_p, C.c_void_p, C.c_void_p]),
    'esr_jpeg16_compress_grad': (C.c_int, [C.c_void_p, C.c_int, C.c_int, C.c_int, C.c_int, C.c_void_p, C.c_void_p, C.c_void_p]),
    'esr_psnr_ssim_partials': (C.c_int64, [C.c_int, C.c_int, C.c_int, C.c_int]),
    'esr_psnr_ssim': (C.c_int, [C.c_void_p, C.c_void_p, C.c_int, C.c_int, C.c_int, C.c_int, C.c_float, C.c_float, C.c_int, C.c_int, C.c_void_p, C.c_void_p,
                                C.c_void_p]),
    'esr_sample_std_partials': (C.c_int64, [C.c_int, C.c_int, C.c_int]),
    'esr_sample_std': (C.c_int, [C.c_void_p, C.c_int, C.c_int, C.c_int, C.c_int, C.c_int, C.c_void_p, C.c_void_p, C.c_void_p, C.c_void_p]),
}
EXPORTS = tuple(_SIGS)

_lib = None


def library_path():
    return os.environ.get('ESR_HIP_LIBRARY') or os.path.join(_HERE, _LIB_NAME)


def load_library():
    global _lib
    if _lib is not None:
        return _lib
    import torch
    path = library_path()
    if not os.path.exists(path):
        raise EsrError('%s not found: build it with `make -C explorable-super-resolution_amd/csrc` (or __graft_entry__.build()). '
                       'There is no CPU fallback for the RRDB/CEM kernels.' % path)
    try:
        h = C.CDLL(path)
    except OSError as e:
        raise EsrError('cannot load %s: %s' % (path, e))
    for name, (res, args) in _SIGS.items():
        try:
            f = getattr(h, name)
        except AttributeError:
            raise EsrError('%s does not export %s (stale build?)' % (path, name))
        f.restype = res
        f.argtypes = args
    if h.esr_cmd_bytes() != C.sizeof(Cmd):
        raise EsrError('%s: esr_cmd is %d bytes in the library, %d in this binding (stale build?)' % (path, h.esr_cmd_bytes(), C.sizeof(Cmd)))
    _lib = h
    return h


class _LazyLib:
    def __getattr__(self, name):
        return getattr(load_library(), name)


lib = _LazyLib()

ESR_OK, ESR_E_ARG, ESR_E_UNSUPPORTED, ESR_E_LAUNCH = 0, -1, -2, -3
PIXELS_FLOAT, PIXELS_ROUND, PIXELS_RAW = 0, 1, 2
PACK_FOLD2 = 2
_ERR = {-1: 'ESR_E_ARG (bad argument)', -2: 'ESR_E_UNSUPPORTED (unsupported shape)', -3: 'ESR_E_LAUNCH (HIP launch error)'}


def check(rc, what):
    if rc != 0:
        raise EsrError('%s failed: %s' % (what, _ERR.get(rc, rc)))
```

### explorable-super-resolution_amd/esr_hip/act.py

```python
import ctypes as C
import functools
import itertools
import math
import threading

import torch

from . import _lib
from ._image import detach_f32
from ._lib import ActView, EsrError, check


def require_gpu(t, what='tensor'):
    if not (torch.is_tensor(t) and t.is_cuda):
        raise EsrError('%s must live on an AMD GPU: the RRDB/CEM kernels have no CPU fallback' % what)


_tls = threading.local()


def stream_ptr():
    s = getattr(_tls, 'stream', None)
    return s if s is not None else C.c_void_p(torch.cuda.current_stream().cuda_stream)

# ... 248 lines not shown
            require_gpu(w, 'conv weight')
            self._build(w.device)
            self._built = True
        return self

    def _bind_bias(self, n, dev, rows=None):
        bp = self._fwd_bias()
        self._bias_shared = bp is not None and rows is None and bp.dtype == torch.float32 and bp.is_contiguous() and bp.numel() == n
        self.bias = bp.detach() if self._bias_shared else torch.zeros(n, dtype=torch.float32, device=dev)
        if bp is not None and rows is not None:
            self._bias_rows = torch.tensor(rows, dtype=torch.long, device=dev)

    @property
    def needs_after_pack(self):
        return self._fwd_bias() is not None and not self._bias_shared

    def after_pack(self):
        bp = self._fwd_bias()
        if self._bias_shared:
            if self.bias.data_ptr() != bp.data_ptr():
                self.bias = bp.detach()
        elif bp is not None:
            b = bp.detach().float()
            if self._bias_rows is not None:
                b = b[self._bias_rows]
            self.bias[:b.numel()].copy_(b)
        self._key = self.key()

    def get(self):
        if self.stale():
            self.prepare()
            run_pack_jobs(self.jobs(), self.split)
            self.after_pack()
        return self


def _fp32(w):
    wd = w.detach()
    return wd if wd.dtype == torch.float32 and wd.is_contiguous() else wd.float().contiguous()


class PackedConv(_Pack):

    def __init__(self, weight, bias, lat, split=True, transposed=False, m_slice=None, rows=None, fold=None):
        super().__init__(split, transposed, bias)
        self.weight, self.lat = weight, lat
        self.fold = fold
        assert fold is None or not transposed
        self.m_slice = m_slice
        self.rows = rows

    def _maps(self, dev):
        w = self.weight
        cout_w, cin_w = w.shape[0], w.shape[1]
        lat = self.lat
        main = cin_w - lat
        if not self.transposed:
            kmap = []
            if lat:
                kmap += [e if e < lat else -1 for e in range(8)]
            ncg_main = (main + 7) // 8
            kmap += [lat + c if c < main else -1 for c in range(ncg_main * 8)]
            if self.rows is not None:
                mt = (len(self.rows) + 31) // 32
                mmap = list(self.rows) + [-1] * (mt * 32 - len(self.rows))
            else:
                mt = (cout_w + 31) // 32
                mmap = [m if m < cout_w else -1 for m in range(mt * 32)]
        else:
            ncg_k = (cout_w + 7) // 8
            kmap = [c if c < cout_w else -1 for c in range(ncg_k * 8)]
            if self.rows is not None:
                assert len(self.rows) % 8 == 0
                kmap = list(self.rows)
            if self.m_slice == 'latent':
                mlist = list(range(lat))
            else:
                lo, hi = self.m_slice if self.m_slice is not None else (0, main)
                mlist = [lat + c for c in range(lo, hi)]
            mt = (len(mlist) + 31) // 32
            assert 1 <= mt <= 2, 'a data-gradient pack covers at most 64 output channels'
            mmap = mlist + [-1] * (mt * 32 - len(mlist))
        self.ncg_in = len(kmap) // 8
        self.mtiles = mt
        self.m_channels = len([m for m in mmap if m >= 0])
        return (torch.tensor(kmap, dtype=torch.int32, device=dev), torch.tensor(mmap, dtype=torch.int32, device=dev))

    def _build(self, dev):
        self.kmap, self.mmap = self._maps(dev)
        nbytes = _lib.lib.esr_conv_wpack_bytes(self.ncg_in, self.mtiles * 32, fmt_code(self.split))
        if self.wpack is None:
            self.wpack = torch.empty(nbytes, dtype=torch.uint8, device=dev)
        assert self.wpack.numel() == nbytes
        self._bind_bias(self.mtiles * 32, dev, self.rows)

    def jobs(self):
        self._wd = _fp32(self.weight)
        form = _lib.PACK_FOLD2 + self.fold if self.fold is not None else (1 if self.transposed else 0)
        return [(self._wd, self.kmap, self.ncg_in, self.mmap, self.mtiles, form, 1.0, self.wpack.data_ptr())]


class _PackedParts(_Pack):

    def _build_parts(self, ncg_in, m, dev):
        per = _lib.lib.esr_conv_wpack_bytes(ncg_in, m, fmt_code(self.split))
        self.wpack = torch.empty(len(self.parts) * per, dtype=torch.uint8, device=dev)
        for s, pk in enumerate(self.parts):
            pk.wpack = self.wpack[s * per:(s + 1) * per]
            pk.prepare()

    def jobs(self):
        return [j for pk in self.parts for j in pk.jobs()]


class PackedConvSlices(_PackedParts):

    def __init__(self, weight, bias, lat=0, split=True, transposed=False):
        super().__init__(split, transposed, None if transposed else bias)
        self.weight, self.lat = weight, lat
        cout, cin = weight.shape[0], weight.shape[1]
        if transposed:
            assert lat == 0
            if cin > 64 and cin % 64:
                raise EsrError('conv weight %s: the data gradient needs up to 64 or a multiple of 64 input channels' % (tuple(weight.shape),))
            self.parts = [PackedConv(weight, None, 0, split=split, transposed=True, m_slice=(m0, min(cin, m0 + 64))) for m0 in range(0, cin, 64)]
        else:
            assert cout <= 64 or cout % 64 == 0
            self.parts = [PackedConv(weight, None, lat, split=split, rows=list(range(m0, min(cout, m0 + 64)))) for m0 in range(0, cout, 64)]

    def _build(self, dev):
        cout, cin = self.weight.shape[0], self.weight.shape[1]
        if self.transposed:
            self._build_parts((cout + 7) // 8, min(cin, 64), dev)
        else:
            self._build_parts((1 if self.lat else 0) + (cin - self.lat + 7) // 8, min(cout, 64), dev)
        self._bind_bias(cout, dev)


class PackedConvPhases(_PackedParts):

    def __init__(self, weight, bias, split=True):
        super().__init__(split, False, bias)
        self.weight, self.lat, self.parts = weight, 0, []
        cout = weight.shape[0]
        for c in range((cout + 31) // 32):
            rows = [m if m < cout else -1 for m in range(32 * c, 32 * c + 32)]
            self.parts += [PackedConv(weight, None, 0, split=split, rows=rows + rows, fold=p0) for p0 in (0, 2)]

    def _build(self, dev):
        self._build_parts((self.weight.shape[1] + 7) // 8, 64, dev)
        self._bind_bias(32 * (len(self.parts) // 2), dev)


def run_pack_jobs(jobs, split):
    for wd, kmap, ncg_in, mmap, mtiles, transposed, scale, dst in jobs:
        check(_lib.lib.esr_pack_conv_weights(wd.data_ptr(), wd.shape[0], wd.shape[1], kmap.data_ptr(), ncg_in, mmap.data_ptr(), mtiles,
                                             transposed, fmt_code(split), float(scale), dst, stream_ptr()), 'esr_pack_conv_weights')


class PackBatch:

    def __init__(self):
        self.pack_ids, self.wptrs, self.ws, self.n, self.nblocks = None, None, None, 0, 0
        self.epoch, self.npacks, self.post = None, 0, []

    def run(self, packs, epoch=None):
        if epoch is not None:
            same = epoch == self.epoch and len(packs) == self.npacks and self.wptrs is not None
        else:
            ids = tuple(id(pk) for pk in packs)
            wptrs = tuple(w.data_ptr() for pk in packs for w in pk.weights())
            same = ids == self.pack_ids and wptrs == self.wptrs
        if not same:
            jobs = []
            for pk in packs:
                pk.prepare()
                jobs += [j + (fmt_code(pk.split),) for j in pk.jobs()]
            wptrs = tuple(w.data_ptr() for pk in packs for w in pk.weights())
            if any(j[0].dtype != torch.float32 or not j[0].is_contiguous() for j in jobs):
                wptrs = None
            arr = (_lib.PackDesc * len(jobs))()
            for d, (wd, kmap, ncg_in, mmap, mtiles, transposed, scale, dst, code) in zip(arr, jobs):
                d.w, d.cout_w, d.cin_w = wd.data_ptr(), wd.shape[0], wd.shape[1]
                d.kmap, d.ncg_in, d.mmap, d.mtiles = kmap.data_ptr(), ncg_in, mmap.data_ptr(), mtiles
                d.transposed, d.split, d.scale, d.wpack = transposed, code, float(scale), dst
            need = _lib.lib.esr_pack_batch_workspace_bytes(arr, len(jobs))
            check(min(need, 0), 'esr_pack_batch_workspace_bytes')
            self.ws = torch.empty(int(need), dtype=torch.uint8, device=jobs[0][0].device)
            nb = _lib.lib.esr_pack_batch_upload(arr, len(jobs), self.ws.data_ptr(), self.ws.numel(), stream_ptr())
            check(min(nb, 0), 'esr_pack_batch_upload')
            self.n, self.nblocks = len(jobs), int(nb)
            self.pack_ids, self.wptrs, self.epoch, self.npacks = tuple(id(pk) for pk in packs), wptrs, epoch, len(packs)
            self.post = [pk for pk in packs if pk.needs_after_pack]
        check(_lib.lib.esr_pack_batch_run(self.ws.data_ptr(), self.n, self.nblocks, stream_ptr()), 'esr_pack_batch_run')
        for pk in (self.post if same else packs):
            pk.after_pack()


class PackedSum(_Pack):

    def __init__(self, pieces, rows, split=True):
        super().__init__(split, True)
        self.pieces, self.rows = pieces, rows

    def weights(self):
        return tuple(w for w, _ in self.pieces)

    def _build(self, dev):
        nrows = len(self.rows[0])
        mt = (nrows + 31) // 32
        self.mtiles, self.m_channels = mt, nrows
        self.maps, g = [], 0
        for (w, _), rows in zip(self.pieces, self.rows):
            assert w.shape[0] % 16 == 0 and len(rows) == nrows
            kmap = torch.arange(w.shape[0], dtype=torch.int32, device=dev)
            mmap = torch.tensor(list(rows) + [-1] * (mt * 32 - nrows), dtype=torch.int32, device=dev)
            self.maps.append((kmap, mmap, g))
            g += w.shape[0] // 8
        self.ncg_in = g
        self.wpack = torch.empty(_lib.lib.esr_conv_wpack_bytes(g, mt * 32, fmt_code(self.split)), dtype=torch.uint8, device=dev)
        self._bind_bias(mt * 32, dev)
        self.chunk_bytes = _lib.lib.esr_conv_wpack_bytes(2, mt * 32, fmt_code(self.split))

    def jobs(self):
        self._wd = [_fp32(w) for w, _ in self.pieces]
        return [(wd, kmap, wd.shape[0] // 8, mmap, self.mtiles, 1, scale, self.wpack.data_ptr() + (g0 // 2) * self.chunk_bytes)
                for wd, (_, scale), (kmap, mmap, g0) in zip(self._wd, self.pieces, self.maps)]


_launch_parity = 0
LDS_STAGES = 0


def reset_launch_parity():
    global _launch_parity
    _launch_parity = 0


class RangeWatch:

    def __init__(self, device):
        self.flag = torch.full((1,), -1, dtype=torch.int32, device=device)
        self.names = []


_range_watch = None


class watching:

    def __init__(self, w):
        self.w = w

    def __enter__(self):
        global _range_watch
        self.prev, _range_watch = _range_watch, self.w
        return self.w

    def __exit__(self, *exc):
        global _range_watch
        _range_watch = self.prev


def conv3x3(pc, in1, B, H, W, cout, in0=None, upsample=1, act_slope=1.0, alpha=1.0, res1=None, beta1=0.0, res2=None, beta2=0.0,
            out=None, out2=None, out_nchw=None, use_bias=True, mask_src=None, mask_cg=(0, 0), mask_slope=0.2, reverse=None, in1_lo_groups=0,
            pixel_shuffle=0, ps_rowgroup0=0, tap_mask_k=None, tap_mask_k_shift=0, tap_mask_m=None, k_split_ws=None, name=None, upsample_phases=0):
    d = _lib.Conv3x3Desc()
    d.upsample_phases = upsample_phases
    if _range_watch is not None:
        d.range_flag, d.range_tag = _range_watch.flag.data_ptr(), len(_range_watch.names)
        _range_watch.names.append(name or 'conv %d' % len(_range_watch.names))
    d.in0 = in0 if in0 is not None else NO_VIEW
    d.in1 = in1
    d.upsample = upsample
    d.wpack = pc.wpack.data_ptr()
    d.bias = pc.bias.data_ptr() if use_bias else None
    d.cout = cout
    d.B, d.H, d.W = B, H, W
    d.act_slope, d.alpha = act_slope, alpha
    d.res1 = res1 if res1 is not None else NO_VIEW
    d.beta1 = beta1
    d.res2 = res2 if res2 is not None else NO_VIEW
    d.beta2 = beta2
    d.out = out if out is not None else NO_VIEW
    d.out2 = out2 if out2 is not None else NO_VIEW
    d.out_nchw = out_nchw.data_ptr() if out_nchw is not None else None
    d.mask_src = mask_src if mask_src is not None else NO_VIEW
    d.mask_cg0, d.mask_cg1 = mask_cg
    d.mask_slope = mask_slope
    global _launch_parity
    if reverse is None:
        reverse = bool(_launch_parity & 1)
        _launch_parity += 1
    d.reverse_order = 1 if reverse else 0
    d.lds_stages = LDS_STAGES
    d.weight_planes = {0: 1, 1: 2, 2: 1, 3: 2}[fmt_code(pc.split)]
    d.in1_lo_groups = in1_lo_groups
    d.pixel_shuffle, d.ps_rowgroup0 = pixel_shuffle, ps_rowgroup0
    if tap_mask_k is not None:
        d.tap_mask_k[:] = tap_mask_k
        d.tap_mask_k_shift = tap_mask_k_shift
    if tap_mask_m is not None:
        d.tap_mask_m[:] = tap_mask_m
    if k_split_ws is not None:
        d.k_split_ws, d.k_split_ws_floats = k_split_ws.data_ptr(), k_split_ws.numel()
    rec = _rec()
    if rec is not None:
        rec.emit(_lib.OP_CONV3X3, d, ('out_nchw',))
        return
    check(_lib.lib.esr_conv3x3(C.byref(d), stream_ptr()), 'esr_conv3x3')


def pixel_unshuffle(src, r, dst, B):
    rec = _rec()
    if rec is not None:
        rec.emit(_lib.OP_PIXEL_UNSHUFFLE, _lib.CmdPixelUnshuffle(src, r, dst, B))
        return
    check(_lib.lib.esr_pixel_unshuffle(C.byref(src), r, C.byref(dst), B, stream_ptr()), 'esr_pixel_unshuffle')


def act_combine(out, B, A_=None, alpha=1.0, Bv=None, beta=1.0, s=1, mask=None, mask_slope=0.2):
    rec = _rec()
    if rec is not None:
        nv = lambda v: v if v is not None else NO_VIEW
        rec.emit(_lib.OP_ACT_COMBINE, _lib.CmdActCombine(nv(A_), alpha, nv(Bv), beta, s, nv(mask), mask_slope, out, B))
        return
    ref = lambda v: C.byref(v) if v is not None else None
    check(_lib.lib.esr_act_combine(ref(A_), alpha, ref(Bv), beta, s, ref(mask), mask_slope, C.byref(out), B, stream_ptr()), 'esr_act_combine')


class GradScaler:

    def __init__(self, device, first, max_rescales=64):
        self.n = max_rescales
        self.slots = torch.zeros(self.n, dtype=torch.int32, device=device)
        self.scales = torch.ones(self.n + 1, dtype=torch.float32, device=device)
        self.scales[0:1].copy_(first.reshape(1))
        self.i = 0

    @property
    def current(self):
        return self.scales[self.i]

    def _ptr(self, t, i):
        return t.data_ptr() + 4 * i

    def rescale(self, B, views, exp):
        assert self.i < self.n
        slot = self._ptr(self.slots, self.i)
        rec = _rec()
        if rec is not None:
            rec.emit(_lib.OP_GRAD_ABSMAX, _lib.CmdGradAbsmax(views[0], B, slot))
            for j, v in enumerate(views):
                rec.emit(_lib.OP_GRAD_SCALE, _lib.CmdGradScale(v, v, B, slot, exp, self._ptr(self.scales, self.i), None,
                                                               self._ptr(self.scales, self.i + 1) if j == 0 else None))
            self.i += 1
            return
        check(_lib.lib.esr_grad_absmax(C.byref(views[0]), B, slot, stream_ptr()), 'esr_grad_absmax')
        for j, v in enumerate(views):
            check(_lib.lib.esr_grad_scale(C.byref(v), C.byref(v), B, slot, exp, self._ptr(self.scales, self.i), None,
                                          self._ptr(self.scales, self.i + 1) if j == 0 else None, stream_ptr()), 'esr_grad_scale')
        self.i += 1

    def rescaled_copy(self, B, src, dst, scale_then):
        rec = _rec()
        if rec is not None:
            rec.emit(_lib.OP_GRAD_SCALE, _lib.CmdGradScale(src, dst, B, None, 0, self._ptr(self.scales, self.i), scale_then.data_ptr(), None))
            return
        check(_lib.lib.esr_grad_scale(C.byref(src), C.byref(dst), B, None, 0, self._ptr(self.scales, self.i), scale_then.data_ptr(), None,
                                      stream_ptr()), 'esr_grad_scale')


def unpack_grad_nchw(G, dst, C_, h, w, c0, nc, pad=0, down=1, accumulate=False, batch_stride=0):
    require_gpu(dst, 'gradient')
    assert dst.dtype == torch.float32 and dst.is_contiguous()
    rec = _rec()
    if rec is not None:
        rec.emit(_lib.OP_UNPACK_GRAD_NCHW, _lib.CmdUnpackGradNchw(G, dst.data_ptr(), batch_stride, dst.shape[0], C_, h, w, c0, nc, pad, down,
                                                                  1 if accumulate else 0), ('dst',))
        return
    check(_lib.lib.esr_unpack_grad_nchw(C.byref(G), dst.data_ptr(), batch_stride, dst.shape[0], C_, h, w, c0, nc, pad, down,
                                        1 if accumulate else 0, stream_ptr()), 'esr_unpack_grad_nchw')


def conv3x3_nchw_parts(parts, in1, B, H, W, out, **kw):
    m0 = 0
    for pc in parts:
        mc = pc.m_channels
        tmp = out if mc == out.shape[1] else torch.empty(B, mc, H, W, dtype=torch.float32, device=out.device)
        conv3x3(pc, in1, B, H, W, mc, out_nchw=tmp, **kw)
        if tmp is not out:
            out[:, m0:m0 + mc] = tmp
        m0 += mc
    return out


def conv3x3_nchw(x, weight, bias, act_slope=1.0, split=True):
    require_gpu(x, 'conv input')
    x = x.detach()
    x = (x if x.dtype == torch.float32 else x.float()).contiguous()
    B, Cin, H, W = x.shape
    cout = weight.shape[0]
    assert weight.shape[1] == Cin
    ncg = (Cin + 7) // 8
    src = ActBuf(B, ncg, H, W, x.device, split)
    pack_nchw(x, src.view(), 0, Cin)
    parts = [PackedConv(weight.detach()[m0:m0 + 64].contiguous(), None if bias is None else bias.detach()[m0:m0 + 64].contiguous(), 0, split=split).get()
             for m0 in range(0, cout, 64)]
    return conv3x3_nchw_parts(parts, src.view(), B, H, W, torch.empty(B, cout, H, W, dtype=torch.float32, device=x.device), act_slope=act_slope)


def conv3x3_dgrad_nchw(dy, weight, split=True):
    require_gpu(dy, 'gradient')
    dy = dy.detach()
    dy = (dy if dy.dtype == torch.float32 else dy.float()).contiguous()
    B, Cout, H, W = dy.shape
    cin = weight.shape[1]
    assert weight.shape[0] == Cout
    src = ActBuf(B, (Cout + 7) // 8, H, W, dy.device, split)
    pack_nchw(dy, src.view(), 0, Cout)
    parts = [PackedConv(weight, None, 0, split=split, transposed=True, m_slice=(lo, min(cin, lo + 64))).get() for lo in range(0, cin, 64)]
    return conv3x3_nchw_parts(parts, src.view(), B, H, W, torch.empty(B, cin, H, W, dtype=torch.float32, device=dy.device), use_bias=False)


def wgrad_desc(dy, x_main, x_lat, lat, wshape, B, H, W, alpha, upsample, device, out=None, tap_masks=None):
    cout, cin = wshape[0], wshape[1]
    if out is None:
        dw = torch.zeros(cout, cin, 3, 3, dtype=torch.float32, device=device)
        db = torch.zeros(cout, dtype=torch.float32, device=device)
    else:
        dw, db = out
    nlat = lat if x_lat is not None else 0
    d = _lib.WgradDesc()
    d.dy, d.x = dy, x_main
    d.xlat = x_lat if x_lat is not None else NO_VIEW
    d.lat, d.upsample = nlat, upsample
    d.cout, d.cin_main = cout, cin - nlat
    d.B, d.H, d.W = B, H, W
    d.alpha = alpha
    d.dw, d.db = dw.data_ptr(), db.data_ptr()
    if tap_masks is not None:
        d.tap_masks[:] = tap_masks
    return d, dw, db


def conv3x3_wgrad(dy, x_main, x_lat, lat, wshape, B, H, W, alpha, upsample, device, tap_masks=None):
    d, dw, db = wgrad_desc(dy, x_main, x_lat, lat, wshape, B, H, W, alpha, upsample, device, tap_masks=tap_masks)
    need = _lib.lib.esr_conv3x3_wgrad_workspace_floats(C.byref(d))
    check(min(need, 0), 'esr_conv3x3_wgrad_workspace_floats')
    ws = _wgrad_workspace(device, need)
    d.workspace, d.workspace_floats = ws.data_ptr(), ws.numel()
    check(_lib.lib.esr_conv3x3_wgrad(C.byref(d), stream_ptr()), 'esr_conv3x3_wgrad')
    return dw, db


class WgradTable:

    def __init__(self, descs, device, unit=0, ptr=0):
        self.arr, self.unit, self.ptr, n = (_lib.WgradDesc * len(descs))(*descs), unit, ptr, len(descs)
        need = _lib.lib.esr_conv3x3_wgrad_batch_part_workspace_bytes(self.arr, n, unit) if unit else _lib.lib.esr_conv3x3_wgrad_batch_workspace_bytes(self.arr, n)
        check(min(need, 0), 'esr_conv3x3_wgrad_batch_workspace_bytes')
        self.ws, self.plan = torch.empty(int(need), dtype=torch.uint8, device=device), _lib.WgradBatchPlan()
        args = (self.arr, n, self.ws.data_ptr(), self.ws.numel(), C.byref(self.plan))
        if unit:
            check(_lib.lib.esr_conv3x3_wgrad_batch_part_upload(*args, unit, stream_ptr()), 'esr_conv3x3_wgrad_batch_part_upload')
# ... 124 lines not shown
```

### explorable-super-resolution_amd/esr_hip/engine.py

```python
import weakref

import torch

import ctypes as C

from . import _lib
from . import act as A
from ._lib import EsrError


class _Lease:
    pass


class RRDBEngine:
    def __init__(self, net):
        self.net = net
        self.split = True
        self._convs_cache = None
        self._params_cache, self._params_probe = None, None
        self._packed = None
        self._packed_t = None
        self._packed_rdb_t = None
        self._bufs = {}
        self._gpool, self._gpool_key = {}, None
        self._pack_batch = A.PackBatch()
        self._packs_fp = None
        self._pack_sets = 0
        self._pack_gen = [0, 0, 0]
        self._wgb = {}
        self.use_plans = True
        self.stash = 'masks'
        self._ptr_fp, self._ptr_epoch = None, 0
        self.generation = 0
        self._ev = None
        self._watch, self._watch_host, self._watch_ev = None, None, None
        self.wgrad_exchange = None
        self.wgrad_overlap = WGRAD_OVERLAP
        self._side, self._xs = None, None
        self.n_up = 1 if net.upscale == 3 else len([1 for mod in net.model if isinstance(mod, torch.nn.Sequential)])
        self.ng = net.nf // 8
        self.nd = self.ng + 16

    def set_precision(self, precision):
        split = {'split': True, 'bf16': False, 'f16': 'f16', 'f16x2': 'f16x2', 'mixed': 'mixed'}[precision]
        if split != self.split:
            self.split = split
            if self._watch is not None:
                self._watch.flag.fill_(-1)
                self._watch_host.fill_(-1)
                self._watch_ev = None
            self._packed = None
            self._packed_t = None
            self._packed_rdb_t = None
            self._bufs = {}
            self._packs_fp = None
            self._pack_sets += 1

    def _watching(self, device):
        if self.split not in ('f16', 'f16x2', 'mixed'):
            return None
        if self._watch is None or self._watch.flag.device != device:
            self._watch = A.RangeWatch(device)
            self._watch_host = torch.full((1,), -1, dtype=torch.int32).pin_memory()
            self._watch_ev = None
        return self._watch

    def _post_range(self):
        if self._watch is None or A._rec() is not None or torch.cuda.is_current_stream_capturing():
            return
        self._watch_host.copy_(self._watch.flag, non_blocking=True)
        self._watch_ev = torch.cuda.Event()
        self._watch_ev.record()

    def check_range(self, wait=True):
        ev = self._watch_ev
        if self._watch is None or torch.cuda.is_current_stream_capturing():
            return
        if ev is None:
            if not wait:
                return
            self._watch_host.copy_(self._watch.flag)
        elif wait:
            ev.synchronize()
        elif not ev.query():
            return
        self._watch_ev = None
        tag = int(self._watch_host[0])
        if tag == -1:
            return
        names = self._watch.names
        name = names[tag] if 0 <= tag < len(names) else 'launch %d' % tag
        self._watch.flag.fill_(-1)
        self._watch_host.fill_(-1)
        raise EsrError("precision %r: the activations stored by layer '%s' reached fp16's last binade (|x| >= 32768) or are not finite — the "
                       "fp16 modes cannot hold this network's range; use set_precision('split') (fp32-class) or 'bf16'" % (
                           self.split if isinstance(self.split, str) else 'split', name))

    def invalidate(self):
        for d in (self._packed, self._packed_t, self._packed_rdb_t):
            for p in (d or {}).values():
                p._key = None
        self.generation += 1

    def _convs(self):
        if self._convs_cache is None:
            self._convs_cache = self._walk_convs()
        return self._convs_cache

    def parameters(self):
        convs = self._convs()
        probe = (convs[0][1].weight, convs[-1][1].weight)
        if self._params_cache is None or self._params_probe[0] is not probe[0] or self._params_probe[1] is not probe[1]:
            self._params_cache = [p for _, c, _ in convs for p in (c.weight, c.bias) if p is not None]
            self._params_probe = probe
        return self._params_cache

    def _walk_convs(self):
        net = self.net
        m = net.model
        lat_first, lat = net.num_latent_channels if net.latent_input is not None else 0, net._lat_all_layers
        out = [('fea', m[0], lat_first)]
        sub = m[1].sub
        for r in range(net.nb):
            for k, rdb in enumerate((sub[r].RDB1, sub[r].RDB2, sub[r].RDB3)):
                for i in range(5):
                    out.append(('rrdb%d.rdb%d.conv%d' % (r, k, i), rdb.convs[i][0], lat))
        out.append(('lr_conv', sub[net.nb], lat))
        idx = 2
        for j in range(self.n_up):
            out.append(('up%d' % j, m[idx][1] if net.upsample_mode == 'upconv' else m[idx][0], 0))
            idx += 1
        out.append(('hr0', m[idx], lat))
        out.append(('hr1', m[idx + 2], lat))
        return out

    def _refresh_packs(self):
        dicts = (self._packed, self._packed_t, self._packed_rdb_t)
        fp = (tuple((p.data_ptr(), p._version) for p in self.parameters()), tuple(d is not None for d in dicts), self._pack_sets, self.generation)
        if fp == self._packs_fp:
            return
        ptrs = tuple(a for a, _ in fp[0])
        if ptrs != self._ptr_fp:
            self._ptr_fp, self._ptr_epoch = ptrs, self._ptr_epoch + 1
        packs = [p for d in dicts if d for p in d.values()]
        if packs:
            self._pack_batch.run(packs, epoch=(self._ptr_epoch, self._pack_sets))
        self._packs_fp = fp

    def _wfmt(self, rdb):
        if self.split != 'mixed':
            return self.split
        return 'f16x2' if rdb else 'f16x3'

    @property
    def _pshuf(self):
        return 0 if self.net.upsample_mode == 'upconv' else (3 if self.net.upscale == 3 else 2)

    def _ps_rows(self, q=None):
        r2 = self._pshuf ** 2
        groups = range(8 * r2) if q is None else range(8 * q, min(8 * q + 8, 8 * r2))
        return [((g // r2) * 8 + e) * r2 + g % r2 for g in groups for e in range(8)]

    def packed(self):
        if self._packed is None:
            d = {}
            for name, c, lat in self._convs():
                if name.startswith('up') and self._pshuf:
                    for q in range(self._pshuf ** 2):
                        d[name, q] = A.PackedConv(c.weight, c.bias, lat, split=self._wfmt(name.startswith('rrdb')), rows=self._ps_rows(q))
                elif name.startswith('up') and self.net.upscale != 3:
                    d[name] = A.PackedConvPhases(c.weight, c.bias, split='f16x3' if self.split == 'f16x2' else self._wfmt(False))
                    d[name, 'taps9'] = (A.PackedConvSlices if c.weight.shape[0] > 64 else A.PackedConv)(c.weight, c.bias, lat, split=self._wfmt(False))
                elif c.weight.shape[0] > 64:
                    d[name] = A.PackedConvSlices(c.weight, c.bias, lat, split=self._wfmt(name.startswith('rrdb')))
                else:
                    d[name] = A.PackedConv(c.weight, c.bias, lat, split=self._wfmt(name.startswith('rrdb')))
            self._packed = d
            self._pack_sets += 1
            self._pack_gen[0] = self._pack_sets
        self._refresh_packs()
        return self._packed

    def packed_t(self):
        if self._packed_t is None:
            d = {}
            for name, c, lat in self._convs():
                if name.startswith('rrdb'):
                    continue
                main = c.weight.shape[1] - lat
                rows = self._ps_rows() if (name.startswith('up') and self._pshuf) else None
                for j in range((main + 63) // 64):
                    d[name, 'm%d' % j] = A.PackedConv(c.weight, None, lat, split=self._wfmt(False), transposed=True, m_slice=(64 * j, min(main, 64 * j + 64)), rows=rows)
                if lat:
                    d[name, 'z'] = A.PackedConv(c.weight, None, lat, split=self._wfmt(False), transposed=True, m_slice='latent')
            self._packed_t = d
            self._pack_sets += 1
            self._pack_gen[1] = self._pack_sets
        self._refresh_packs()
        return self._packed_t

    def packed_rdb_t(self):
        if self._packed_rdb_t is None:
            d = {}
            mods = {name: (c, lat) for name, c, lat in self._convs()}
            nf = self.net.nf
            for r in range(self.net.nb):
                for k in range(3):
                    name = 'rrdb%d.rdb%d' % (r, k)
                    ws = [mods['%s.conv%d' % (name, i)][0].weight for i in range(5)]
                    lat = mods[name + '.conv0'][1]
                    s4 = 0.2 * (0.2 if k == 2 else 1.0)
                    pieces = [(ws[4], s4), (ws[3], 1.0), (ws[2], 1.0), (ws[1], 1.0), (ws[0], 1.0)]
                    for c in (3, 2, 1, 0):
                        rows = list(range(lat + nf + 32 * c, lat + nf + 32 + 32 * c))
                        d[name, 'g%d' % c] = A.PackedSum(pieces[:4 - c], [rows] * (4 - c), split=self._wfmt(True))
                    for j in range((nf + 63) // 64):
                        d[name, 'gx%d' % j] = A.PackedSum(pieces, [list(range(lat + 64 * j, lat + min(nf, 64 * j + 64)))] * 5, split=self._wfmt(True))
                    if lat:
                        d[name, 'gz'] = A.PackedSum(pieces, [list(range(lat))] * 5, split=self._wfmt(True))
            self._packed_rdb_t = d
            self._pack_sets += 1
            self._pack_gen[2] = self._pack_sets
        self._refresh_packs()
        return self._packed_rdb_t

    def _buffers(self, B, h, w, dev, keep):
        key = (B, h, w, str(dev), keep)
        cached = self._bufs.get(key)
        if cached is not None:
            busy = cached.get('_busy')
            if not keep or busy is None or busy() is None:
                return self._lease(cached) if keep else cached
            fresh = self._new_buffers(B, h, w, dev, keep)
            fresh['_ephemeral'] = True
            return self._lease(fresh)
        if len(self._bufs) > 2:
            self._bufs.clear()
        d = self._new_buffers(B, h, w, dev, keep)
        self._bufs[key] = d
        return self._lease(d) if keep else d

    @staticmethod
    def _lease(d):
        lease = _Lease()
        d['_busy'] = weakref.ref(lease)
        out = dict(d)
        out['_lease'] = lease
        return out

    def _new_buffers(self, B, h, w, dev, keep):
        net, sp = self.net, self.split
        sf, ng = net.upscale, self.ng
        d = {}
        has_lat = net.latent_input is not None and net.num_latent_channels > 0
        if has_lat:
            d['zlr'] = A.ActBuf(B, 1, h, w, dev, sp)
            if net._lat_all_layers:
                d['zhr'] = A.ActBuf(B, 1, sf * h, sf * w, dev, sp)
        d['xin'] = A.ActBuf(B, 1, h, w, dev, sp)
        d['fea'] = A.ActBuf(B, ng, h, w, dev, sp)
        d['rdb'] = [A.ActBuf(B, self.nd, h, w, dev, sp) for _ in range(3 * net.nb if keep is True else 3)]
        if keep == 'masks':
            one_plane = 'f16' if sp in ('mixed', 'f16', 'f16x2', 'f16x3') else False
            d['stash'] = [A.ActBuf(B, 16, h, w, dev, one_plane) for _ in range(3 * net.nb)]
        d['last'] = A.ActBuf(B, ng, h, w, dev, sp)
        d['trunk'] = A.ActBuf(B, ng, h, w, dev, sp)
        ups = []
        s = 1
        for j in range(self.n_up):
            s *= 3 if sf == 3 else 2
            ups.append(A.ActBuf(B, ng, s * h, s * w, dev, sp))
        d['ups'] = ups
        d['hr0'] = A.ActBuf(B, ng, sf * h, sf * w, dev, sp)
        d['_plans'] = {}
        return d

    def forward(self, x, pad=0):
        A.require_gpu(x, 'generator input')
        if torch.is_grad_enabled() and (x.requires_grad or any(p.requires_grad for p in self.parameters())):
            from . import autograd as AG
            return AG.rrdb_forward_with_grad(self, x, pad)
        return self.run_forward(x, pad, keep=False)[0]

    def _check(self, x):
        net = self.net
        sf = net.upscale
        has_lat = net.latent_input is not None and net.num_latent_channels > 0
        lat1 = net.num_latent_channels if has_lat else 0
        if x.shape[1] != lat1 * sf * sf + 3:
            raise EsrError('expected %d input channels (latent %d x sf^2 + 3), got %d' % (lat1 * sf * sf + 3, lat1, x.shape[1]))
        return sf, has_lat, lat1

    def keep_mode(self):
        if self.stash == 'masks' and not any(p.requires_grad for p in self.parameters()):
            return 'masks'
        return True

    def _plan_key(self, kind, *what):
        packs = self._pack_gen[0] if kind == 'fwd' else tuple(self._pack_gen)
        return (kind,) + what + (self.split, self._ptr_epoch, packs, A.LDS_STAGES)

    @A.one_stream
    def run_forward(self, x, pad=0, keep=False):
        net = self.net
        x = x.detach()
        if x.dtype != torch.float32 or not x.is_contiguous():
            x = x.float().contiguous()
        sf, has_lat, lat1 = self._check(x)
        B, Ct, h0, w0 = x.shape
        self.packed()
        self.check_range(wait=False)
        watch = self._watching(x.device)
        bufs = self._buffers(B, h0 + 2 * pad, w0 + 2 * pad, x.device, keep)
        g = torch.empty(B, net.out_nc, sf * (h0 + 2 * pad), sf * (w0 + 2 * pad), dtype=torch.float32, device=x.device)
        if not self.use_plans or bufs.get('_ephemeral') or A._rec() is not None:
            if watch is not None:
                watch.names = []
            with A.watching(watch):
                self._forward_launches(x, pad, keep, bufs, g)
            self._post_range()
            return g, bufs
        key = self._plan_key('fwd', tuple(x.shape), pad, keep)
        plan = bufs['_plans'].get(key)
        if plan is None:
            rec = A.Recorder({'x': x, 'g': g})
            if watch is not None:
                watch.names = []
            with A.recording(rec), A.watching(watch):
                self._forward_launches(x, pad, keep, bufs, g)
            plan = bufs['_plans'][key] = rec.finish()
        plan.run({'x': x, 'g': g})
        self._post_range()
        return g, bufs

    def _forward_launches(self, x, pad, keep, bufs, g):
        net = self.net
        sf, has_lat, lat1 = self._check(x)
        B, Ct, h0, w0 = x.shape
        pk = self.packed()
        h, w = h0 + 2 * pad, w0 + 2 * pad
        H, W = sf * h, sf * w
        conv = A.conv3x3
        nf, ng, nd = net.nf, self.ng, self.nd
        A.reset_launch_parity()

        A.pack_nchw(x, bufs['xin'].view(), c0=Ct - 3, nc=3, pad=pad)
        zlr = zhr = None
        if has_lat:
            kw = dict(hw=(sf * h0, sf * w0), batch_stride=Ct * h0 * w0, channels=lat1)
            A.pack_nchw(x, bufs['zlr'].view(), 0, lat1, pad=sf * pad, down=sf, **kw)
            zlr = bufs['zlr'].view()
            if net._lat_all_layers:
                A.pack_nchw(x, bufs['zhr'].view(), 0, lat1, pad=sf * pad, **kw)
                zhr = bufs['zhr'].view()
        zall = zlr if net._lat_all_layers else None

        A.host_op(lambda ctx: self._ev and self._ev[0].record())
        rdb = bufs['rdb']
        nrdb = 3 * net.nb

        def buf_of(j):
            if j == nrdb:
                return bufs['last']
            return rdb[j] if keep is True else rdb[j % 3]

        conv(pk['fea'], bufs['xin'].view(), B, h, w, nf, in0=zlr, out=bufs['fea'].view(), out2=buf_of(0).view(0, ng) if net.nb else None, name='fea_conv')
        mixed = self.split == 'mixed'
        hi_only = dict(in1_lo_groups=-1) if mixed else {}
        for r in range(net.nb):
            rrdb_in = buf_of(3 * r)
            for k in range(3):
                buf, nxt = buf_of(3 * r + k), buf_of(3 * r + k + 1)
                for i in range(4):
                    o2 = dict(out2=bufs['stash'][3 * r + k].view(4 * i, 4)) if keep == 'masks' else {}
                    conv(pk['rrdb%d.rdb%d.conv%d' % (r, k, i)], buf.view(0, ng + 4 * i), B, h, w, 32, in0=zall, act_slope=0.2,
                         out=buf.view(ng + 4 * i, 4, with_lo=not mixed), name='rrdb%d.rdb%d.conv%d' % (r, k, i), **hi_only, **o2)
                name = 'rrdb%d.rdb%d.conv4' % (r, k)
                if k < 2:
                    conv(pk[name], buf.view(0, nd), B, h, w, nf, in0=zall, alpha=0.2, res1=buf.view(0, ng), beta1=1.0, out=nxt.view(0, ng), name=name, **hi_only)
                else:
                    conv(pk[name], buf.view(0, nd), B, h, w, nf, in0=zall, alpha=0.04, res1=buf.view(0, ng), beta1=0.2,
                         res2=rrdb_in.view(0, ng), beta2=1.0, out=nxt.view(0, ng), name=name, **hi_only)
        last = buf_of(nrdb).view(0, ng) if net.nb else bufs['fea'].view()
        conv(pk['lr_conv'], last, B, h, w, nf, in0=zall, res1=bufs['fea'].view(), beta1=1.0, out=bufs['trunk'].view(), name='LR_conv')
        src, s = bufs['trunk'], 1
        for j in range(self.n_up):
            f = 3 if sf == 3 else 2
            s *= f
            if self._pshuf:
                for q in range(f * f):
                    conv(pk['up%d' % j, q], src.view(), B, s // f * h, s // f * w, 64, act_slope=0.2, out=bufs['ups'][j].view(), pixel_shuffle=f, ps_rowgroup0=8 * q, name='upconv%d' % j)
            elif f == 2 and keep is False:
                conv(pk['up%d' % j], src.view(), B, s // f * h, s // f * w, nf, upsample_phases=2, act_slope=0.2, out=bufs['ups'][j].view(), name='upconv%d' % j)
            else:
                conv(pk[('up%d' % j, 'taps9') if f == 2 else 'up%d' % j], src.view(), B, s * h, s * w, nf, upsample=f, act_slope=0.2, out=bufs['ups'][j].view(),
                     name='upconv%d' % j)
            src = bufs['ups'][j]
        conv(pk['hr0'], src.view(), B, H, W, nf, in0=zhr, act_slope=0.2, out=bufs['hr0'].view(), name='HR_conv0')
        conv(pk['hr1'], bufs['hr0'].view(), B, H, W, net.out_nc, in0=zhr, out_nchw=g)
        A.host_op(lambda ctx: self._ev and self._ev[1].record())

    @A.one_stream
    def run_backward(self, x_shape, pad, bufs, dg, need_dx=True, need_dw=False):
        if self.split in ('f16', 'f16x2'):
            raise NotImplementedError("the fp16 precisions are inference modes: fp16 gradients underflow without loss scaling; "
                                      "use 'split' (fp32-class) or 'bf16' for training / Z optimisation")
        if need_dw and 'stash' in bufs:
            raise EsrError('this forward kept LeakyReLU masks only (no parameter asked for a gradient when it ran): weight gradients need the activations')
        dg = dg.detach()
        dg = (dg if dg.dtype == torch.float32 else dg.float()).contiguous()
        self.packed_t()
        if self.net.nb:
            self.packed_rdb_t()
        planned = self.use_plans and self.split != 'mixed' and not self._pshuf and not bufs.get('_ephemeral') and A._rec() is None \
            and '_plans' in bufs
        if not planned:
            return self._backward_launches(x_shape, pad, bufs, dg, need_dx, need_dw)
        B, Ct, h0, w0 = x_shape
        dx = torch.zeros(B, Ct, h0, w0, dtype=torch.float32, device=dg.device) if need_dx else None
        ext = {'dg': dg}
        if dx is not None:
            ext['dx'] = dx
        key = self._plan_key('bwd', tuple(x_shape), pad, bool(need_dx), bool(need_dw), None if self.wgrad_exchange is None else int(self.wgrad_exchange.bucket_bytes), str(self.wgrad_overlap or 0))
        entry = bufs['_plans'].get(key)
        if entry is None:
            wg = WGrad(self, need_dw, B)
            rec = A.Recorder(ext)
            with A.recording(rec):
                _, grads = self._backward_launches(x_shape, pad, bufs, dg, need_dx, need_dw, dx=dx, wg=wg, pool={}, keep=rec.keep)
            entry = bufs['_plans'][key] = (rec.finish(), wg)
        else:
            grads = entry[1].rebind()
        entry[0].run(ext)
        return dx, grads

    def _backward_launches(self, x_shape, pad, bufs, dg, need_dx, need_dw, dx=None, wg=None, pool=None, keep=None):
        net, sp = self.net, self.split
        sf = net.upscale
        has_lat = net.latent_input is not None and net.num_latent_channels > 0
        lat1 = net.num_latent_channels if has_lat else 0
        lat = net._lat_all_layers
        B, Ct, h0, w0 = x_shape
        h, w = h0 + 2 * pad, w0 + 2 * pad
        H, W = sf * h, sf * w
        dev = dg.device
        pt = self.packed_t()
        conv = A.conv3x3
        nf, ng, nd = net.nf, self.ng, self.nd
        A.reset_launch_parity()
        f16_bwd = sp == 'mixed'
        gscale = None
        if f16_bwd:
            scaler = A.GradScaler(dev, _pow2_scale(dg, 4), max_rescales=net.nb + 2)
            gscale = scaler.current
            dg = dg * gscale
        hi_only = dict(in1_lo_groups=-1) if f16_bwd else {}
        if wg is None:
            wg = WGrad(self, need_dw, B, hi_only=f16_bwd)
        wg.gscale = gscale
        pool_key = (B, h, w, str(dev), sp)
        if pool is None:
            if self._gpool_key != pool_key:
                self._gpool, self._gpool_key = {}, pool_key
            pool = self._gpool
        taken = []

        def galloc(Bb, ncg, Hh, Ww):
            free = pool.setdefault((ncg, Hh, Ww), [])
            buf = free.pop() if free else A.ActBuf(Bb, ncg, Hh, Ww, dev, sp)
            taken.append(buf)
            return buf

        def zview(bufname):
            return bufs[bufname].view() if bufname in bufs else None

        def dgrad(name, dy, out, cg_lo, cg_hi, Hh, Ww, alpha=1.0, accumulate=False, extra=None, extra_beta=1.0, mask=None, upsample=1):
            for j in range(cg_lo // 8, (cg_hi + 7) // 8):
                lo, hi = max(cg_lo, 8 * j), min(cg_hi, 8 * j + 8)
                if lo >= hi:
                    continue
                kw = {}
                ov = out.view(lo, hi - lo)
                if accumulate:
                    kw.update(res1=ov, beta1=1.0)
                    if extra is not None and lo < 8:
                        kw.update(res2=extra, beta2=extra_beta)
                elif extra is not None and lo < 8:
                    kw.update(res1=extra, beta1=extra_beta)
                if mask is not None:
                    mb, m0, m1 = mask
                    a0, a1 = max(m0, lo), min(m1, hi)
                    if a0 < a1:
                        kw.update(mask_src=mb.view(a0, a1 - a0), mask_cg=(a0 - lo, a1 - lo), mask_slope=0.2)
                conv(pt[name, 'm%d' % j], dy, B, Hh, Ww, (hi - lo) * 8, alpha=alpha, out=ov, use_bias=False, **kw)

        def dgrad_z(name, dy, gz, Hh, Ww, alpha, first):
            kw = {} if first else dict(res1=gz.view(), beta1=1.0)
            conv(pt[name, 'z'], dy, B, Hh, Ww, lat1, alpha=alpha, out=gz.view(), use_bias=False, **kw)

        G_g = galloc(B, 1, H, W)
        A.pack_nchw(dg, G_g.view(), 0, net.out_nc)
        G_hr0 = galloc(B, ng, H, W)
        zgrad = need_dx and lat
        GZ_hr = galloc(B, 1, H, W) if (has_lat and zgrad) else None
        GZ_lr = galloc(B, 1, h, w) if (has_lat and need_dx) else None
        wg.conv('hr1', G_g.view(), bufs['hr0'].view(), zview('zhr') if lat else None, H, W, keep=(G_g,))
        dgrad('hr1', G_g.view(), G_hr0, 0, ng, H, W, mask=(bufs['hr0'], 0, ng))
        if GZ_hr is not None:
            dgrad_z('hr1', G_g.view(), GZ_hr, H, W, 1.0, first=True)
        G_up = galloc(B, ng, H, W)
        src_act = bufs['ups'][-1] if self.n_up else bufs['trunk']
        wg.conv('hr0', G_hr0.view(), src_act.view(), zview('zhr') if lat else None, H, W, keep=(G_hr0,))
        dgrad('hr0', G_hr0.view(), G_up, 0, ng, H, W, mask=(src_act, 0, ng) if self.n_up else None)
        if GZ_hr is not None:
            dgrad_z('hr0', G_hr0.view(), GZ_hr, H, W, 1.0, first=False)
        del G_hr0, G_g
        cur_g, s = G_up, sf if sf != 3 else 3
        for j in reversed(range(self.n_up)):
            f = 3 if sf == 3 else 2
            Hj, Wj = s * h, s * w
            below = bufs['ups'][j - 1] if j > 0 else bufs['trunk']
            if self._pshuf:
                s //= f
                Gc = galloc(B, 8 * f * f, s * h, s * w)
                A.pixel_unshuffle(cur_g.view(), f, Gc.view(), B)
                wg.conv('up%d' % j, Gc.view(), below.view(), None, s * h, s * w, keep=(Gc, cur_g), rows=self._ps_rows())
                nxt_g = galloc(B, 8, s * h, s * w)
                dgrad('up%d' % j, Gc.view(), nxt_g, 0, 8, s * h, s * w, mask=(below, 0, 8) if j > 0 else None)
                cur_g = nxt_g
                continue
            wg.conv('up%d' % j, cur_g.view(), below.view(), None, Hj, Wj, upsample=f, keep=(cur_g,))
            tmp = galloc(B, ng, Hj, Wj)
            dgrad('up%d' % j, cur_g.view(), tmp, 0, ng, Hj, Wj)
            s //= f
            nxt_g = galloc(B, ng, s * h, s * w)
            A.act_combine(nxt_g.view(), B, Bv=tmp.view(), beta=1.0, s=f, mask=below.view() if j > 0 else None)
            cur_g = nxt_g
            del tmp
        G_trunk = cur_g
        if f16_bwd:
            scaler.rescale(B, [G_trunk.view()], 10)
            gscale_hr, gscale = gscale, scaler.current
            gscale_trunk = gscale
            wg.gscale = gscale
        last_act = bufs['last'] if net.nb else bufs['fea']
        pr = self.packed_rdb_t() if net.nb else {}
        ring = [galloc(B, nd, h, w) for _ in range(4)] if (net.nb and not need_dw) else []
        nseq = 3 * net.nb

        def gbuf(n):
            return ring[n % 4] if ring else galloc(B, nd, h, w)

# ... 277 lines not shown
```

### include/esr_hip.h

```cpp
#ifndef ESR_HIP_H
#define ESR_HIP_H

#include <stddef.h>
#include <stdint.h>

#ifdef __cplusplus
extern "C" {
#endif

#define ESR_OK 0
#define ESR_E_ARG (-1)
#define ESR_E_UNSUPPORTED (-2)
#define ESR_E_LAUNCH (-3)

typedef void* esr_stream_t;

#define ESR_FMT_BF16 0
#define ESR_FMT_F16 1

typedef struct {
    void* hi;
    void* lo;
    int32_t ncg;
    int32_t H, W;
    int64_t batch_stride;
    int64_t cg_stride;
    int32_t fmt;
} esr_act_view;

typedef struct {
    esr_act_view in0;
    esr_act_view in1;
    int32_t upsample;
    const void* wpack;
    const float* bias;
    int32_t cout;
    int32_t B, H, W;
    float act_slope;
    float alpha;
    esr_act_view res1; float beta1;
    esr_act_view res2; float beta2;
    esr_act_view out;
    esr_act_view out2;
    float* out_nchw;
    esr_act_view mask_src; int32_t mask_cg0, mask_cg1; float mask_slope;
    int32_t reverse_order;
    int32_t weight_planes;
    int32_t in1_lo_groups;
    int32_t pixel_shuffle;
    int32_t ps_rowgroup0;
    int32_t tap_mask_k[4];
    int32_t tap_mask_k_shift;
    int32_t tap_mask_m[4];
    float* k_split_ws;
    int64_t k_split_ws_floats;
    int32_t lds_stages;
    uint32_t* range_flag;
    uint32_t range_tag;
    int32_t upsample_phases;
} esr_conv3x3_desc;

int esr_conv3x3(const esr_conv3x3_desc* d, esr_stream_t stream);

int esr_conv3x3_tiling(const esr_conv3x3_desc* d, int32_t* tiling);

int esr_pixel_unshuffle(const esr_act_view* src, int r, const esr_act_view* dst, int B, esr_stream_t stream);

size_t esr_conv_wpack_bytes(int ncg_in, int cout, int split);

#define ESR_PACK_FOLD2 2
int esr_pack_conv_weights(const float* w, int cout_w, int cin_w, const int32_t* kmap, int ncg_in,
                          const int32_t* mmap, int mtiles, int transposed, int split, float scale, void* wpack,
                          esr_stream_t stream);

typedef struct {
    const float* w; int32_t cout_w, cin_w; const int32_t* kmap; int32_t ncg_in; const int32_t* mmap;
    int32_t mtiles, transposed, split; float scale; void* wpack;
} esr_pack_desc;
int64_t esr_pack_batch_workspace_bytes(const esr_pack_desc* descs, int n);
int64_t esr_pack_batch_upload(const esr_pack_desc* descs, int n, void* workspace, int64_t workspace_bytes, esr_stream_t stream);
int esr_pack_batch_run(const void* workspace, int n, int64_t nblocks, esr_stream_t stream);

int esr_pack_nchw(const float* src, int64_t src_batch_stride, int B, int C, int h, int w, int c0, int nc, int pad, int down,
                  const esr_act_view* dst, esr_stream_t stream);
int esr_unpack_nchw(const esr_act_view* src, int B, int nc, float* dst, esr_stream_t stream);
int esr_zero(void* p, int64_t n16, esr_stream_t stream);

int esr_pack_nchw_norm(const float* src, int B, int C, int h, int w, const float* mean, const float* std, const esr_act_view* dst, esr_stream_t stream);
int esr_unpack_grad_nchw_norm(const esr_act_view* G, int B, int C, const float* std, float* dst, esr_stream_t stream);
int esr_maxpool2x2(const esr_act_view* x, const esr_act_view* y, int B, esr_stream_t stream);
int esr_maxpool2x2_grad(const esr_act_view* x, const esr_act_view* dy, int relu_mask, const esr_act_view* dx, int B, esr_stream_t stream);


int esr_cem_downscale(const float* y, int B, int C, int h, int w, int sf, int pre, const float* taps, int k,
                      const float* lr, int lr_pad, float* d, esr_stream_t stream);
int esr_cem_lrfilter(const float* x, int B, int C, int h, int w, const float* taps, int k, float* out,
                     esr_stream_t stream);
int esr_cem_upscale(const float* f, const float* f2, int B, int C, int h, int w, int sf, int pre,
                    const float* taps, int k, const float* g, int crop, int mode, float range,
                    float* out, float* out2, esr_stream_t stream);

int esr_cem_downscale_sep(const float* y, int B, int C, int h, int w, int sf, int pre, const float* tv, const float* th, int k, const float* lr,
                          int lr_pad, float* d, esr_stream_t stream);
int esr_cem_lrfilter_sep(const float* x, int B, int C, int h, int w, const float* tv, const float* th, int k, float* out, esr_stream_t stream);
int esr_cem_upscale_sep(const float* f, const float* f2, int B, int C, int h, int w, int sf, int pre, const float* tv, const float* th, int k,
                        const float* g, int crop, int mode, float range, float* out, float* out2, esr_stream_t stream);
int esr_cem_filter_upscale_sep(const float* e, const float* e2, int B, int C, int h, int w, int sf, int pre, const float* tvf, const float* thf, int kf,
                               const float* tv, const float* th, int k, const float* g, int crop, int mode, float range, float* out, float* out2,
                               esr_stream_t stream);

int esr_cem_sep_form(int op, int sf, int k, int pre, int h, int w);

int esr_act_combine(const esr_act_view* A, float alpha, const esr_act_view* Bv, float beta, int s, const esr_act_view* mask,
                    float mask_slope, const esr_act_view* out, int B, esr_stream_t stream);
int esr_unpack_grad_nchw(const esr_act_view* G, float* dst, int64_t dst_batch_stride, int B, int C, int h, int w, int c0, int nc,
                         int pad, int down, int accumulate, esr_stream_t stream);
int esr_grad_absmax(const esr_act_view* v, int B, uint32_t* slot, esr_stream_t stream);
int esr_grad_scale(const esr_act_view* src, const esr_act_view* dst, int B, const uint32_t* slot, int exp, const float* scale_in,
                   const float* scale_den, float* scale_out, esr_stream_t stream);
int esr_cem_adjoint(const float* dy, int B, int C, int hq, int wq, int sq, int oq, int Ny, int Nx, const float* tabs, int k,
                    int hn, int wn, int sn, int on, float* dx, int accumulate, esr_stream_t stream);
int esr_cem_adjoint_sep(const float* dy, int B, int C, int hq, int wq, int sq, int oq, int Ny, int Nx, const float* tabs_v, const float* tabs_h, int k,
                        int hn, int wn, int sn, int on, float* tmp, const float* base, float alpha, float* dx, esr_stream_t stream);

typedef struct {
    esr_act_view dy;
    esr_act_view x;
    esr_act_view xlat;
    int32_t lat;
    int32_t upsample;
    int32_t cout, cin_main;
    int32_t B, H, W;
    float alpha;
    float* dw;
    float* db;
    float* workspace;
    int64_t workspace_floats;
    int32_t tap_masks[4];
} esr_wgrad_desc;
int64_t esr_conv3x3_wgrad_workspace_floats(const esr_wgrad_desc* d);
int esr_conv3x3_wgrad(const esr_wgrad_desc* d, esr_stream_t stream);
#define ESR_WGRAD_FORM_LAT27 1
#define ESR_WGRAD_FORM_MAIN27 2
#define ESR_WGRAD_FORM_S2D 4
#define ESR_WGRAD_FORM_FAST_COPY 8
int esr_conv3x3_wgrad_tiling(const esr_wgrad_desc* d, int32_t* out);
int64_t esr_conv3x3_wgrad_batch_workspace_bytes(const esr_wgrad_desc* descs, int n);
int esr_conv3x3_wgrad_batch(const esr_wgrad_desc* descs, int n, void* workspace, int64_t workspace_bytes, esr_stream_t stream);
typedef struct { int64_t nwg, table_bytes; int32_t n, max_red, split, f16, s2d, reserved; } esr_wgrad_batch_plan;
int esr_conv3x3_wgrad_batch_upload(const esr_wgrad_desc* descs, int n, void* workspace, int64_t workspace_bytes, esr_wgrad_batch_plan* plan,
                                   esr_stream_t stream);
int esr_conv3x3_wgrad_batch_run(const void* workspace, const esr_wgrad_batch_plan* plan, esr_stream_t stream);
int esr_conv3x3_wgrad_batch_run_side(const void* workspace, const esr_wgrad_batch_plan* plan, esr_stream_t stream);
int esr_conv3x3_wgrad_side_occupancy(int f16);
int64_t esr_conv3x3_wgrad_batch_unit(const esr_wgrad_desc* descs, int n);
int64_t esr_conv3x3_wgrad_batch_part_workspace_bytes(const esr_wgrad_desc* descs, int n, int64_t unit);
int esr_conv3x3_wgrad_batch_part_upload(const esr_wgrad_desc* descs, int n, void* workspace, int64_t workspace_bytes, esr_wgrad_batch_plan* plan,
                                        int64_t unit, esr_stream_t stream);
int esr_conv3x3_wgrad_batch_rebase(void* workspace, const esr_wgrad_batch_plan* plan, int64_t delta_bytes, esr_stream_t stream);

int64_t esr_soft_hist_slabs(int64_t n);
int esr_soft_hist_fwd(const float* v, int64_t n, int K, float lo, float hi, float T, float eps, double* partial, esr_stream_t stream);
int esr_soft_hist_bwd(const float* v, int64_t n, int K, float lo, float hi, float T, float eps, const float* gh, float* gv, esr_stream_t stream);

int esr_kde_dim_supported(int D);
int esr_kde_fwd(const float* outer, int64_t n_outer, const float* inner, const int32_t* ranges, int n_ranges, int D, float period, float scale, float* pmax,
                double* psum, esr_stream_t stream);
int esr_kde_bwd(const float* X, int64_t R, const int32_t* tiles, int n_tiles, const float* bins, int M, int bins_per_slab, int n_slabs, int D, float period,
                float scale, const float* g_row, const float* l_row, const float* g_bin, const float* l_bin, float* dxpart, esr_stream_t stream);
int esr_kde_dedup(const float* bins, int M, int D, float half_width, int32_t* keep, esr_stream_t stream);

typedef struct { float* p; const float* g; float* m; float* v; int64_t n; } esr_adam_tensor;
int64_t esr_adam_workspace_bytes(const esr_adam_tensor* tensors, int n);
int64_t esr_adam_upload(const esr_adam_tensor* tensors, int n, void* workspace, int64_t workspace_bytes, esr_stream_t stream);
int64_t esr_adam_table(const esr_adam_tensor* tensors, int n, void* host_table, int64_t host_bytes);
int esr_adam_run(const void* workspace, int n, int64_t nchunks, float lr, float beta1, float beta2, float eps, float weight_decay,
                 float bias_correction1, float bias_correction2_sqrt, esr_stream_t stream);

int esr_img_stats(const float* x, int B, int C, int H, int W, const float* mask, int clamp01, int kind, double* sums, esr_stream_t stream);
int esr_img_stats_grad(const float* x, int B, int C, int H, int W, const float* mask, int clamp01, int kind, const float* coef, float* dx, int accumulate,
                       esr_stream_t stream);

int esr_patch_std(const float* x, int B, int C, int H, int W, const uint8_t* corners, float* S, float* mean, esr_stream_t stream);
int esr_patch_std_grad(const float* x, int B, int C, int H, int W, const uint8_t* corners, const float* S, const float* mean, const float* dS, float* dx,
                       int accumulate, esr_stream_t stream);
int esr_shift_l1(const float* x, int B, int C, int H, int W, const float* mask, int nx, int ny, const int32_t* base_x, const float* frac_x,
                 const int32_t* base_y, const float* frac_y, double* partial, esr_stream_t stream);
int esr_shift_l1_grad(const float* x, int B, int C, int H, int W, const float* mask, int nx, int ny, const int32_t* base_x, const float* frac_x,
                      const int32_t* base_y, const float* frac_y, const int32_t* ranges_x, const int32_t* ranges_y, const float* g, float* work, float* dx,
                      int accumulate, esr_stream_t stream);

int esr_scribble(const float* x, int B, int C, int H, int W, const float* desired, const uint8_t* labels, const float* i0, int i0_batch, double* partial,
                 esr_stream_t stream);
int esr_scribble_grad(const float* x, int B, int C, int H, int W, const float* desired, const uint8_t* labels, const float* i0, int i0_batch, const float* g,
                      float g_con, float* dx, int accumulate, esr_stream_t stream);

int64_t esr_patch_mag_blocks(int H, int W);
int esr_patch_mag(const float* x, int B, int C, int H, int W, const int32_t* corner_index, const float* desired, int P, double* partial,
                  esr_stream_t stream);
int esr_patch_mag_grad(const float* x, int B, int C, int H, int W, const int32_t* corner_index, const float* desired, int P, const float* g, float* dx,
                       int accumulate, esr_stream_t stream);

int64_t esr_pairmin_blocks(int C, int H, int W);
int64_t esr_pairmin_work_floats(int Bg, int C, int H, int W, int lo, int hi, int grad);
int esr_pairmin(const float* x, int Bg, int C, int H, int W, int lo, int hi, int clamp01, const float* mask, const float* init, int init_batch, float w,
                float* work, double* partial, esr_stream_t stream);
int esr_pairmin_grad(const float* x, int Bg, int C, int H, int W, int lo, int hi, int clamp01, const float* mask, const float* init, int init_batch,
                     float w, float scale, float* work, float* dx, esr_stream_t stream);

typedef struct {
    esr_act_view y;
    esr_act_view dz, u;
    esr_act_view out0, out1;
    int32_t B, groups, C;
    const float* scale; const float* shift; const float* mean; const float* rstd;
    const float* gamma;
    const double* sums2; const double* sums3;
    float slope;
    int32_t const_stats, s2d;
} esr_bn_desc;
int esr_bn_reduce(const esr_bn_desc* d, int mode, double* sums, esr_stream_t stream);
int esr_bn_apply(const esr_bn_desc* d, int mode, esr_stream_t stream);
int esr_bn_finalize(const double* sums, int groups, int C, int64_t n_per_group, float eps, float momentum, const float* gamma, const float* beta,
                    float* mean, float* rstd, float* scale, float* shift, float* running_mean, float* running_var, esr_stream_t stream);
int esr_bn_param_grads(const double* sums2, const double* sums3, const float* rstd, int groups, int C, int64_t n_per_group, float* dgamma, float* dbeta,
                       float* g_gamma, esr_stream_t stream);

enum {
    ESR_OP_CONV3X3 = 1, ESR_OP_PACK_NCHW = 2, ESR_OP_UNPACK_GRAD_NCHW = 3, ESR_OP_ACT_COMBINE = 4, ESR_OP_PIXEL_UNSHUFFLE = 5,
    ESR_OP_GRAD_ABSMAX = 6, ESR_OP_GRAD_SCALE = 7, ESR_OP_WGRAD_BATCH_RUN = 8, ESR_OP_PACK_BATCH_RUN = 9, ESR_OP_ZERO = 10,
    ESR_OP_UNPACK_NCHW = 11, ESR_OP_WGRAD = 12, ESR_OP_BN_REDUCE = 13, ESR_OP_BN_APPLY = 14, ESR_OP_BN_FINALIZE = 15, ESR_OP_BN_PARAM_GRADS = 16,
    ESR_OP_BN_FINALIZE_APPLY = 17
};
typedef struct { const float* src; int64_t src_batch_stride; int32_t B, C, h, w, c0, nc, pad, down; esr_act_view dst; } esr_cmd_pack_nchw;
typedef struct { esr_act_view G; float* dst; int64_t dst_batch_stride; int32_t B, C, h, w, c0, nc, pad, down, accumulate; } esr_cmd_unpack_grad_nchw;
typedef struct { esr_act_view A; float alpha; esr_act_view Bv; float beta; int32_t s; esr_act_view mask; float mask_slope; esr_act_view out; int32_t B; } esr_cmd_act_combine;
typedef struct { esr_act_view src; int32_t r; esr_act_view dst; int32_t B; } esr_cmd_pixel_unshuffle;
typedef struct { esr_act_view v; int32_t B; uint32_t* slot; } esr_cmd_grad_absmax;
typedef struct { esr_act_view src, dst; int32_t B; const uint32_t* slot; int32_t exp; const float* scale_in; const float* scale_den; float* scale_out; } esr_cmd_grad_scale;
typedef struct { const void* workspace; esr_wgrad_batch_plan plan; } esr_cmd_wgrad_batch_run;
typedef struct { const void* workspace; int32_t n; int64_t nblocks; } esr_cmd_pack_batch_run;
typedef struct { void* p; int64_t n16; } esr_cmd_zero;
typedef struct { esr_act_view src; int32_t B, nc; float* dst; } esr_cmd_unpack_nchw;
typedef struct { esr_bn_desc d; int32_t mode; double* sums; } esr_cmd_bn;
typedef struct { const double* sums; int32_t groups, C; int64_t n_per_group; float eps, momentum; const float* gamma; const float* beta;
                 float* mean; float* rstd; float* scale; float* shift; float* running_mean; float* running_var; } esr_cmd_bn_finalize;
typedef struct { const double* sums2; const double* sums3; const float* rstd; int32_t groups, C; int64_t n_per_group; float* dgamma; float* dbeta;
                 float* g_gamma; } esr_cmd_bn_param_grads;
typedef struct { esr_bn_desc d; esr_cmd_bn_finalize f; } esr_cmd_bn_finalize_apply;
int esr_bn_finalize_apply(const esr_bn_desc* d, const esr_cmd_bn_finalize* f, esr_stream_t stream);
typedef struct {
    int32_t op;
    int32_t reserved;
    union {
        esr_conv3x3_desc conv;
        esr_cmd_pack_nchw pack_nchw;
        esr_cmd_unpack_grad_nchw unpack_grad_nchw;
        esr_cmd_act_combine act_combine;
        esr_cmd_pixel_unshuffle pixel_unshuffle;
        esr_cmd_grad_absmax grad_absmax;
        esr_cmd_grad_scale grad_scale;
        esr_cmd_wgrad_batch_run wgrad_batch_run;
        esr_cmd_pack_batch_run pack_batch_run;
        esr_cmd_zero zero;
        esr_cmd_unpack_nchw unpack_nchw;
        esr_wgrad_desc wgrad;
        esr_cmd_bn bn;
        esr_cmd_bn_finalize bn_finalize;
        esr_cmd_bn_param_grads bn_param_grads;
        esr_cmd_bn_finalize_apply bn_finalize_apply;
    } u;
} esr_cmd;
int esr_run(const esr_cmd* cmds, int n, int* failed, esr_stream_t stream);
int64_t esr_cmd_bytes(void);

int esr_jpeg_compress(const float* x, int B, int H, int W, const float* qtab, int round, float* coef, const esr_act_view* act_out,
                      esr_stream_t stream);
int esr_jpeg_extract(const float* coef, const float* y, int B, int h, int w, const float* qtab, float* coef_out, float* img,
                     esr_stream_t stream);
int esr_jpeg_extract_grad(const float* d_img, const float* y, int B, int h, int w, const float* qtab, float* d_coef, float* d_y,
                          esr_stream_t stream);
int esr_jpeg_compress_grad(const float* d_coef, int B, int h, int w, const float* qtab, float* d_x, esr_stream_t stream);

#define ESR_JPEG16_ALL 0
#define ESR_JPEG16_DOWNSAMPLE 1
#define ESR_JPEG16_QUANTIZE 2
int esr_jpeg16_compress(const float* x, int B, int H, int W, const float* qtab, int mode, float* coef, esr_stream_t stream);
int esr_jpeg16_extract(const float* coef, int coef_C, int coef_c0, const float* y, int form, int B, int h, int w, const float* qtab,
                       float* coef_out, float* img, esr_stream_t stream);
int esr_jpeg16_extract_grad(const float* d_img, const float* y, int form, int B, int h, int w, const float* qtab, float* d_coef, float* d_y,
                            esr_stream_t stream);
int esr_jpeg16_compress_grad(const float* d_coef, int mode, int B, int h, int w, const float* qtab, float* d_x, esr_stream_t stream);

#define ESR_PIXELS_FLOAT 0
#define ESR_PIXELS_ROUND 1
#define ESR_PIXELS_RAW 2
int64_t esr_psnr_ssim_partials(int C, int H, int W, int border);
int esr_psnr_ssim(const float* a, const float* b, int B, int C, int H, int W, float lo, float hi, int quantize, int border, double* partial,
                  double* sums, esr_stream_t stream);
int64_t esr_sample_std_partials(int C, int H, int W);
int esr_sample_std(const float* x, int S, int B, int C, int H, int W, float* map, double* partial, double* sums, esr_stream_t stream);

int esr_version(void);

#ifdef __cplusplus
}
#endif
#endif
```

Baseline: 125.7 million.

## Fold final HR conv into HR_conv0 epilogue via per-tap MFMA plus tap-sum kernel

Result: no change. 126.9 million (median of 6 runs) (+1.0%).

```diff
diff --git a/explorable-super-resolution_amd/csrc/esr_conv.hip b/explorable-super-resolution_amd/csrc/esr_conv.hip
--- a/explorable-super-resolution_amd/csrc/esr_conv.hip
+++ b/explorable-super-resolution_amd/csrc/esr_conv.hip
@@ -15,6 +15,7 @@
 constexpr int EPI_RES1 = 1, EPI_RES2 = 2, EPI_MASK = 4, EPI_NCHW = 8, EPI_OUT2 = 16;
 constexpr int EPI_RESIN = 32;
 constexpr int EPI_PS = 64;
+constexpr int EPI_FOLD = 128;
 
 struct ConvArgs {
     int tiles_x, tiles_y, ntiles;
@@ -52,6 +53,9 @@
     int stages_hint;
     unsigned* range_flag;
     unsigned range_tag;
+    const uint4* fold_w;
+    float* fold_out;
+    int fold_rows;
 #ifdef ESR_TRACE
     unsigned long long* trace;
 #endif
@@ -316,18 +320,27 @@
         const bool valid = (rr < (unsigned)a.TH) && (cc < (unsigned)a.TW) && (Y < (unsigned)a.H) && (X < (unsigned)a.W);
         e.lim[r] = valid ? (KIND == 1 ? a.ncg_out : a.ncg_out - half) : (KIND == 1 ? 0 : -1);
         if (KIND == 1) e.poff[r] = (__umul24(Y, a.W) + X) * 4;
-        else if (KIND == 2) e.poff[r] = (Y << 16) | X;
+        else if (KIND == 2 || KIND == 4) e.poff[r] = (Y << 16) | X;
         else if (KIND == 3) e.poff[r] = valid ? (__umul24(2 * Y + 1, 2 * a.W + 2) + 2 * X + 1) * 16 : 0;
         else e.poff[r] = valid ? (__umul24(Y + 1, a.W + 2) + X + 1) * 16 : 0;
     }
     return e;
 }
 
-template <int NPL, int MT, int R, int EPI, int FMT, bool PARTLO, bool PHASE = false>
+template <int NPL, int MT, int R, int EPI, int FMT, bool PARTLO, bool PHASE = false, int NPW = 1>
 __device__ __forceinline__ void conv_epilogue(const ConvArgs& a, f32x16 (&acc)[MT][R], const int b, const EpiCoord<R>& ec, const int lane) {
     constexpr bool HAS_R1 = (EPI & EPI_RES1) != 0, HAS_R2 = (EPI & EPI_RES2) != 0, HAS_MK = (EPI & EPI_MASK) != 0;
-    constexpr bool NCHW = (EPI & EPI_NCHW) != 0, OUT2 = (EPI & EPI_OUT2) != 0, PS = (EPI & EPI_PS) != 0;
+    constexpr bool NCHW = (EPI & EPI_NCHW) != 0, OUT2 = (EPI & EPI_OUT2) != 0, PS = (EPI & EPI_PS) != 0, FOLD = (EPI & EPI_FOLD) != 0;
+    static_assert(!FOLD || (EPI == EPI_FOLD && MT == 2 && !PHASE && !PARTLO), "the fold: all 64 channels in one workgroup, plain epilogue");
     const int half = lane >> 5;
+    uint4 fw[FOLD ? 4 : 1][FOLD ? NPW : 1];
+    if constexpr (FOLD) {
+#pragma unroll
+        for (int ks = 0; ks < 4; ++ks)
+#pragma unroll
+            for (int pl = 0; pl < NPW; ++pl) fw[ks][pl] = a.fold_w[(ks * NPW + pl) * 64 + lane];
+    }
+    const bool has_out = !FOLD || a.out.hi != nullptr;
     const long long bl = b;
     const f32x2 slope2 = {a.act_slope, a.act_slope}, alpha2 = {a.alpha, a.alpha};
     const char *r1h = nullptr, *r1l = nullptr, *r2h = nullptr, *r2l = nullptr, *mkh = nullptr;
@@ -394,12 +407,22 @@
     for (int r = 0; r < R; ++r) {
         if constexpr (!ALL_FIRST && (HAS_R1 || HAS_R2 || HAS_MK)) issue(r);
         const int rq = ALL_FIRST ? r : 0;
+        f32x16 facc = {};
+        const bool inimg = ec.lim[r] >= 0;
+        unsigned poff_r = ec.poff[r], poff_f = 0;
+        if constexpr (FOLD) {
+            const unsigned Y = ec.poff[r] >> 16, X = ec.poff[r] & 0xFFFF;
+            poff_r = inimg ? (__umul24(Y + 1, a.W + 2) + X + 1) * 16 : 0;
+            poff_f = (__umul24(Y, a.W) + X) * 4;
+        }
 #pragma unroll
         for (int m = 0; m < MT; ++m) {
 #pragma unroll
             for (int gp = 0; gp < 2; ++gp) {
                 const int cg0 = (PHASE ? 0 : m * 4) + gp * 2;
-                if (!(cg0 < ec.lim[r] + (NCHW ? 0 : half))) continue;
+                if constexpr (!FOLD) {
+                    if (!(cg0 < ec.lim[r] + (NCHW ? 0 : half))) continue;
+                }
                 const bool store = cg0 < ec.lim[r];
                 f32x2 v[2][2];
 #pragma unroll
@@ -461,7 +484,7 @@
                     for (int j = 0; j < 2; ++j) {
                         const uint32_t h = cvt_pk<FMT>(v[k][j].x, v[k][j].y);
                         hi[k][j] = h;
-                        if constexpr (FMT == 1) big |= (h & 0x7FFF7FFFu) + 0x08000800u;
+                        if constexpr (FMT == 1) big |= (FOLD && !inimg) ? 0u : (h & 0x7FFF7FFFu) + 0x08000800u;
                         lo[k][j] = 0;
                         if (NPL == 2) lo[k][j] = cvt_pk<FMT>(v[k][j].x - e2f<FMT>(h & 0xFFFF), v[k][j].y - e2f<FMT>(h >> 16));
                     }
@@ -474,13 +497,19 @@
                     const auto t1 = __builtin_amdgcn_permlane32_swap(lo[0][1], lo[1][1], false, false);
                     lv = make_uint4(t0[0], t1[0], t0[1], t1[1]);
                 }
+                if constexpr (FOLD) {
+                    const int ks = m * 2 + gp;
+                    if constexpr (NPW == 2) facc = mfma<FMT>(fw[ks][1], hv, facc);
+                    if constexpr (NPL == 2) facc = mfma<FMT>(fw[ks][0], lv, facc);
+                    facc = mfma<FMT>(fw[ks][0], hv, facc);
+                }
                 unsigned off;
                 if constexpr (PS) {
                     const int cgs = cg0 + half, rg = a.ps_rg0 + cgs, r2 = a.ps * a.ps, sp = rg % r2;
                     const int Y = ec.poff[r] >> 16, X = ec.poff[r] & 0xFFFF;
                     off = ((unsigned)(rg / r2) * (unsigned)a.out.cs + (unsigned)(a.ps * Y + sp / a.ps + 1) * (a.ps * a.W + 2) + (a.ps * X + sp % a.ps + 1)) * 16;
-                } else off = ec.poff[r] + ho + cg0 * ((unsigned)a.out.cs * 16) + (PHASE ? (unsigned)a.ph_off + m * 16 : 0u);
-                if (store) {
+                } else off = poff_r + ho + cg0 * ((unsigned)a.out.cs * 16) + (PHASE ? (unsigned)a.ph_off + m * 16 : 0u);
+                if (store && has_out) {
                     *(uint4*)(oh + off) = hv;
                     if (NPL == 2 && (!PARTLO || ol)) *(uint4*)(ol + off) = lv;
                     if constexpr (OUT2) {
@@ -489,6 +518,15 @@
                         if (NPL == 2 && o2l) *(uint4*)(o2l + off2) = lv;
                     }
                 }
+            }
+        }
+        if constexpr (FOLD) {
+            char* const fb = (char*)(a.fold_out + bl * a.fold_rows * a.H * a.W);
+            const unsigned hw4 = (unsigned)(a.H * a.W) * 4;
+#pragma unroll
+            for (int i = 0; i < 16; ++i) {
+                const int row = (i & 3) + 8 * (i >> 2) + 4 * half;
+                if (inimg && row < a.fold_rows) *(float*)(fb + (poff_f + (unsigned)row * hw4)) = facc[i];
             }
         }
     }
@@ -598,7 +636,7 @@
         for (int c = 0; c < 3; ++c)
             if (c < a.ncp) issue(c, lds0 + c * stage_bytes, true);
     }
-    constexpr int EKIND = TMODE == 3 ? 3 : ((EPI & EPI_NCHW) ? 1 : ((EPI & EPI_PS) ? 2 : 0));
+    constexpr int EKIND = TMODE == 3 ? 3 : ((EPI & EPI_NCHW) ? 1 : ((EPI & EPI_PS) ? 2 : ((EPI & EPI_FOLD) ? 4 : 0)));
     constexpr bool EARLY_COORDS = NST >= 2 || (MT == 1 && NPL == 1);
     f32x16 acc[MT][R];
     EpiCoord<R> ec;
@@ -672,7 +710,7 @@
         for (int cp = lo_end; cp < a.ncp; ++cp) step(std::false_type{}, cp);
     ESR_TR();
     if constexpr (!EARLY_COORDS) ec = epi_coords<R, EKIND>(a, x0, y0, wave, lane);
-    conv_epilogue<NPL, MT, R, EPI, FMT, PARTLO, TMODE == 3>(a, acc, b, ec, lane);
+    conv_epilogue<NPL, MT, R, EPI, FMT, PARTLO, TMODE == 3, NPW>(a, acc, b, ec, lane);
     ESR_TR();
 #ifdef ESR_TRACE
     if (tr && tid == 0) tr[127] = wall_clock64();
@@ -693,11 +731,29 @@
     }
     return a;
 }
+__device__ __forceinline__ void fold_taps_vec(const float* __restrict__ w, int dim0, int dim1, const int* __restrict__ kmap, int ncg_in, int cp, int lane,
+                                              float scale, float (&v8)[8]) {
+    const int row = lane & 31, cg = 2 * cp + (lane >> 5);
+    const int t = row / dim0, c = row - t * dim0;
+#pragma unroll
+    for (int e = 0; e < 8; ++e) {
+        const int kch = cg < ncg_in ? kmap[cg * 8 + e] : -1;
+        v8[e] = (kch >= 0 && t < 9) ? w[((long long)c * dim1 + kch) * 9 + t] * scale : 0.f;
+    }
+}
+constexpr int PACK_FOLD_TAPS = ESR_PACK_FOLD_TAPS;
 __global__ void pack_weights_kernel(const float* __restrict__ w, int dim0, int dim1, const int* __restrict__ kmap, int ncg_in,
                                     const int* __restrict__ mmap, int mtiles, int transposed, int npl, int f16, float scale, uint4* __restrict__ out, int total) {
     const int idx = blockIdx.x * blockDim.x + threadIdx.x;
     if (idx >= total) return;
     const int lane = idx & 63;
+    if (transposed == PACK_FOLD_TAPS) {
+        float f8[8];
+        fold_taps_vec(w, dim0, dim1, kmap, ncg_in, idx >> 6, lane, scale, f8);
+        uint4* o = out + (size_t)(idx >> 6) * npl * 64 + lane;
+        store8(o, npl == 2 ? o + 64 : nullptr, 0, f8, f16 ? ESR_FMT_F16 : ESR_FMT_BF16);
+        return;
+    }
     const int m = (idx >> 6) % mtiles;
     const int ks = (idx >> 6) / mtiles;
     const int cp = ks / 9, t = ks % 9;
@@ -729,6 +785,15 @@
     const int2 m = map[blockIdx.x];
     const PackEntry e = table[m.x];
     const int cp = m.y / e.mtiles, mt = m.y % e.mtiles;
+    if (e.transposed == PACK_FOLD_TAPS) {
+        if (threadIdx.x < 64) {
+            float f8[8];
+            fold_taps_vec(e.w, e.dim0, e.dim1, e.kmap, e.ncg_in, cp, threadIdx.x, e.scale, f8);
+            uint4* o = e.out + (size_t)cp * e.npl * 64 + threadIdx.x;
+            store8(o, e.npl == 2 ? o + 64 : nullptr, 0, f8, e.f16 ? ESR_FMT_F16 : ESR_FMT_BF16);
+        }
+        return;
+    }
     if (threadIdx.x < 16) {
         const int cg = 2 * cp + (threadIdx.x >> 3);
         kch_s[threadIdx.x] = cg < e.ncg_in ? e.kmap[cg * 8 + (threadIdx.x & 7)] : -1;
@@ -855,13 +920,17 @@
 template <int... V> struct Ints {};
 template <int... V> constexpr bool among(Ints<V...>, int v) { return ((v == V) || ...); }
 
-typedef Ints<0, EPI_RES1, EPI_RES1 | EPI_RES2, EPI_RESIN, EPI_RESIN | EPI_RES2, EPI_NCHW, EPI_OUT2, EPI_RES1 | EPI_MASK, EPI_MASK, EPI_PS> ConvEpis;
+typedef Ints<0, EPI_RES1, EPI_RES1 | EPI_RES2, EPI_RESIN, EPI_RESIN | EPI_RES2, EPI_NCHW, EPI_OUT2, EPI_RES1 | EPI_MASK, EPI_MASK, EPI_PS, EPI_FOLD> ConvEpis;
+constexpr bool has_fold(int npl, int mt, int nst, int fmt, int npw, bool partlo, int tmode) {
+    return mt == 2 && tmode == 0 && nst != 4 && !partlo && npw == npl && (fmt == 1 || npl == 2);
+}
 constexpr bool has_ring4(int mt, int epi, int fmt, bool partlo, int tmode) { return (epi == 0 || epi == EPI_NCHW) && !partlo && fmt == 0 && mt == 2 && tmode != 3; }
 constexpr bool two_stages_only(int npl, int tmode) { return (tmode == 1 || tmode == 2) && npl == 2; }
 
 constexpr bool conv_kernel_exists(int npl, int mt, int epi, int nst, int fmt, int npw, bool partlo, int tmode) {
     if (fmt == 0 ? (npw != npl || partlo) : (npw > npl || (partlo && npl == 1))) return false;
     if (nst == 4 ? !has_ring4(mt, epi, fmt, partlo, tmode) : (nst == 1 && two_stages_only(npl, tmode))) return false;
+    if (epi == EPI_FOLD) return has_fold(npl, mt, nst, fmt, npw, partlo, tmode);
     if (tmode == 0) return among(ConvEpis{}, epi);
     if (mt != 2 || partlo) return false;
     return tmode == 3 ? epi == 0 : (fmt == 0 && (epi == 0 || epi == EPI_NCHW));
@@ -903,6 +972,46 @@
     store8(mut(out.hi), mut(out.lo), act_off(out.bs, out.cs, W, b, cg, y, x), v8, ESR_FMT_BF16);
 }
 
+template <int NX>
+__global__ __launch_bounds__(256) void fold_sum_kernel(const float* __restrict__ P, const float* __restrict__ bias, int B, int C, int H, int W, int reverse,
+                                                       float* __restrict__ out) {
+    const unsigned bx = reverse ? gridDim.x - 1 - blockIdx.x : blockIdx.x, by = reverse ? gridDim.y - 1 - blockIdx.y : blockIdx.y;
+    const unsigned nq = W / NX, idx = bx * 256 + threadIdx.x;
+    if (idx >= (unsigned)H * nq) return;
+    const int y = idx / nq, x0 = (idx - y * nq) * NX;
+    const int b = by / C, c = by - b * C;
+    const float bz = bias ? bias[c] : 0.f;
+    float acc[NX];
+#pragma unroll
+    for (int j = 0; j < NX; ++j) acc[j] = bz;
+    const long long hw = (long long)H * W;
+    const float* const pb = P + ((long long)b * 9 * C + c) * hw;
+#pragma unroll
+    for (int ky = 0; ky < 3; ++ky) {
+        const int yy = y + ky - 1;
+        if (yy < 0 || yy >= H) continue;
+#pragma unroll
+        for (int kx = 0; kx < 3; ++kx) {
+            const float* const row = pb + (long long)((3 * ky + kx) * C) * hw + (long long)yy * W;
+            float v[NX];
+            if constexpr (NX == 4) {
+                const float4 q = *(const float4*)(row + x0);
+                if (kx == 1) { v[0] = q.x; v[1] = q.y; v[2] = q.z; v[3] = q.w; }
+                else if (kx == 0) { v[0] = x0 > 0 ? row[x0 - 1] : 0.f; v[1] = q.x; v[2] = q.y; v[3] = q.z; }
+                else { v[0] = q.y; v[1] = q.z; v[2] = q.w; v[3] = x0 + 4 < W ? row[x0 + 4] : 0.f; }
+            } else {
+                const int xx = x0 + kx - 1;
+                v[0] = (xx >= 0 && xx < W) ? row[xx] : 0.f;
+            }
+#pragma unroll
+            for (int j = 0; j < NX; ++j) acc[j] = __fadd_rn(acc[j], v[j]);
+        }
+    }
+    float* const o = out + (((long long)b * C + c) * H + y) * W + x0;
+    if constexpr (NX == 4) *(float4*)o = make_float4(acc[0], acc[1], acc[2], acc[3]);
+    else o[0] = acc[0];
+}
+
 }
 
 #ifdef ESR_TRACE
@@ -916,9 +1025,10 @@
 
 extern "C" int esr_pack_conv_weights(const float* w, int cout_w, int cin_w, const int32_t* kmap, int ncg_in, const int32_t* mmap,
                                      int mtiles, int transposed, int split, float scale, void* wpack, esr_stream_t stream) {
-    if (!w || !kmap || !mmap || !wpack || ncg_in <= 0 || mtiles <= 0 || transposed < 0 || transposed > 5) return ESR_E_ARG;
+    if (!w || !kmap || !mmap || !wpack || ncg_in <= 0 || mtiles <= 0 || transposed < 0 || transposed > PACK_FOLD_TAPS) return ESR_E_ARG;
+    if (transposed == PACK_FOLD_TAPS && (mtiles != 1 || cout_w < 1 || 9 * cout_w > 32)) return ESR_E_ARG;
     const int ncp = (ncg_in + 1) / 2;
-    const int total = ncp * 9 * mtiles * 64;
+    const int total = transposed == PACK_FOLD_TAPS ? ncp * 64 : ncp * 9 * mtiles * 64;
     ESR_CLEAR_ERR();
     hipLaunchKernelGGL(pack_weights_kernel, dim3((total + 255) / 256), dim3(256), 0, (hipStream_t)stream, w, cout_w, cin_w, kmap,
                        ncg_in, mmap, mtiles, transposed, (split == 1 || split == 3) ? 2 : 1, split >= 2 ? 1 : 0, scale, (uint4*)wpack, total);
@@ -930,8 +1040,9 @@
     int64_t nb = 0;
     for (int i = 0; i < n; ++i) {
         if (!descs[i].w || !descs[i].kmap || !descs[i].mmap || !descs[i].wpack || descs[i].ncg_in <= 0 || descs[i].mtiles <= 0 || descs[i].transposed < 0 ||
-            descs[i].transposed > 5)
+            descs[i].transposed > PACK_FOLD_TAPS)
             return ESR_E_ARG;
+        if (descs[i].transposed == PACK_FOLD_TAPS && (descs[i].mtiles != 1 || descs[i].cout_w < 1 || 9 * descs[i].cout_w > 32)) return ESR_E_ARG;
         nb += (int64_t)((descs[i].ncg_in + 1) / 2) * descs[i].mtiles;
     }
     return nb;
@@ -983,8 +1094,15 @@
 
 static int conv_validate(const esr_conv3x3_desc* d) {
     if (!d || !d->in1.hi || !d->wpack || d->B <= 0 || d->H <= 0 || d->W <= 0 || d->cout <= 0) return ESR_E_ARG;
-    if (!d->out.hi && !d->out_nchw) return ESR_E_ARG;
+    if (!d->out.hi && !d->out_nchw && !d->fold_w) return ESR_E_ARG;
     const int ups = d->upsample <= 0 ? 1 : d->upsample;
+    if (d->fold_w) {
+        if (!d->fold_out || d->fold_cout < 1) return ESR_E_ARG;
+        if (d->res1.hi || d->res2.hi || d->mask_src.hi || d->out2.hi || d->out_nchw || d->pixel_shuffle > 1 || ups > 1 || d->upsample_phases != 0 ||
+            !all_taps(d->tap_mask_k) || !all_taps(d->tap_mask_m) || d->k_split_ws || d->cout != 64 || 9 * d->fold_cout > 32)
+            return ESR_E_UNSUPPORTED;
+        if ((long long)9 * d->fold_cout * d->H * d->W * 4 >= 0x100000000ll) return ESR_E_UNSUPPORTED;
+    }
     if (ups > 8 || ups == 5 || ups == 7) return ESR_E_UNSUPPORTED;
     if (ups > 1 && d->in0.hi) return ESR_E_UNSUPPORTED;
     if (d->upsample_phases != 0 && d->upsample_phases != 2) return ESR_E_UNSUPPORTED;
@@ -1026,7 +1144,7 @@
     p.npl = d->in1.lo ? 2 : 1;
     p.ps = d->pixel_shuffle > 1 ? d->pixel_shuffle : 0;
     p.mslice = false;
-    if (p.nslices == 1 && p.mt == 2 && d->cout == 64 && !d->out_nchw && !p.ps && d->lds_stages == 0 && !d->k_split_ws && all_taps(d->tap_mask_k) &&
+    if (p.nslices == 1 && p.mt == 2 && d->cout == 64 && !d->out_nchw && !d->fold_w && !p.ps && d->lds_stages == 0 && !d->k_split_ws && all_taps(d->tap_mask_k) &&
         all_taps(d->tap_mask_m) && (!d->mask_src.hi || (d->mask_cg0 == 0 && d->mask_cg1 >= 8))) {
         const TileCfg t2 = pick_tile(d->H, d->W, p.npl, 2, WGS_MT2);
         p.mslice = t2.TH != 0 && (long long)t2.tiles_x * t2.tiles_y * d->B <= CONV_SMALL_WGS;
@@ -1066,7 +1184,8 @@
             p.epi = EPI_RESIN;
         }
     }
-    p.epi |= (d->res2.hi ? EPI_RES2 : 0) | (d->mask_src.hi ? EPI_MASK : 0) | (d->out_nchw ? EPI_NCHW : 0) | (d->out2.hi ? EPI_OUT2 : 0) | (p.ps ? EPI_PS : 0);
+    p.epi |= (d->res2.hi ? EPI_RES2 : 0) | (d->mask_src.hi ? EPI_MASK : 0) | (d->out_nchw ? EPI_NCHW : 0) | (d->out2.hi ? EPI_OUT2 : 0) | (p.ps ? EPI_PS : 0) |
+             (d->fold_w ? EPI_FOLD : 0);
     if ((p.epi & EPI_NCHW) && d->out.hi) return ESR_E_UNSUPPORTED;
     p.wpl = d->weight_planes ? d->weight_planes : (f16 ? 1 : p.npl);
     if (p.wpl < 1 || p.wpl > p.npl || (!f16 && p.wpl != p.npl)) return ESR_E_ARG;
@@ -1138,6 +1257,7 @@
     a.stages_hint = (d->lds_stages == 1 || d->lds_stages == 2) ? d->lds_stages : 0;
     a.range_flag = p.fmt ? d->range_flag : nullptr; a.range_tag = d->range_tag;
     a.ps = p.ps; a.ps_rg0 = d->ps_rowgroup0;
+    a.fold_w = (const uint4*)d->fold_w; a.fold_out = d->fold_out; a.fold_rows = 9 * d->fold_cout;
 #ifdef ESR_TRACE
     a.trace = g_trace;
 #endif
@@ -1180,6 +1300,19 @@
     return ESR_OK;
 }
 
+extern "C" int esr_conv3x3_fold_sum(const float* P, const float* bias, int B, int C, int H, int W, int reverse_order, float* out, esr_stream_t stream) {
+    if (!P || !out || B <= 0 || C <= 0 || H <= 0 || W <= 0) return ESR_E_ARG;
+    if ((long long)B * C > 65535 || (long long)H * W >= 0x7FFFFFFFll) return ESR_E_UNSUPPORTED;
+    const bool quads = W % 4 == 0 && ((uintptr_t)P | (uintptr_t)out) % 16 == 0;
+    const long long per_plane = (long long)H * (quads ? W / 4 : W);
+    const dim3 grid((unsigned)((per_plane + 255) / 256), (unsigned)(B * C));
+    ESR_CLEAR_ERR();
+    if (quads) hipLaunchKernelGGL(fold_sum_kernel<4>, grid, dim3(256), 0, (hipStream_t)stream, P, bias, B, C, H, W, reverse_order, out);
+    else hipLaunchKernelGGL(fold_sum_kernel<1>, grid, dim3(256), 0, (hipStream_t)stream, P, bias, B, C, H, W, reverse_order, out);
+    ESR_CHECK_LAUNCH();
+    return ESR_OK;
+}
+
 extern "C" int esr_conv3x3(const esr_conv3x3_desc* d, esr_stream_t stream) {
     if (int rc = conv_validate(d)) return rc;
     ConvPlan p{};
diff --git a/explorable-super-resolution_amd/csrc/esr_run.hip b/explorable-super-resolution_amd/csrc/esr_run.hip
--- a/explorable-super-resolution_amd/csrc/esr_run.hip
+++ b/explorable-super-resolution_amd/csrc/esr_run.hip
@@ -31,6 +31,10 @@
             case ESR_OP_PACK_BATCH_RUN: rc = esr_pack_batch_run(c.u.pack_batch_run.workspace, c.u.pack_batch_run.n, c.u.pack_batch_run.nblocks, stream); break;
             case ESR_OP_ZERO: rc = esr_zero(c.u.zero.p, c.u.zero.n16, stream); break;
             case ESR_OP_UNPACK_NCHW: rc = esr_unpack_nchw(&c.u.unpack_nchw.src, c.u.unpack_nchw.B, c.u.unpack_nchw.nc, c.u.unpack_nchw.dst, stream); break;
+            case ESR_OP_FOLD_SUM: {
+                const esr_cmd_fold_sum& a = c.u.fold_sum;
+                rc = esr_conv3x3_fold_sum(a.P, a.bias, a.B, a.C, a.H, a.W, a.reverse_order, a.out, stream);
+            } break;
             case ESR_OP_WGRAD: rc = esr_conv3x3_wgrad(&c.u.wgrad, stream); break;
             case ESR_OP_BN_REDUCE: rc = esr_bn_reduce(&c.u.bn.d, c.u.bn.mode, c.u.bn.sums, stream); break;
             case ESR_OP_BN_APPLY: rc = esr_bn_apply(&c.u.bn.d, c.u.bn.mode, stream); break;
diff --git a/explorable-super-resolution_amd/esr_hip/_lib.py b/explorable-super-resolution_amd/esr_hip/_lib.py
--- a/explorable-super-resolution_amd/esr_hip/_lib.py
+++ b/explorable-super-resolution_amd/esr_hip/_lib.py
@@ -24,7 +24,8 @@
                 ('reverse_order', C.c_int32), ('weight_planes', C.c_int32), ('in1_lo_groups', C.c_int32),
                 ('pixel_shuffle', C.c_int32), ('ps_rowgroup0', C.c_int32), ('tap_mask_k', C.c_int32 * 4), ('tap_mask_k_shift', C.c_int32),
                 ('tap_mask_m', C.c_int32 * 4), ('k_split_ws', C.c_void_p), ('k_split_ws_floats', C.c_int64), ('lds_stages', C.c_int32),
-                ('range_flag', C.c_void_p), ('range_tag', C.c_uint32), ('upsample_phases', C.c_int32)]
+                ('range_flag', C.c_void_p), ('range_tag', C.c_uint32), ('upsample_phases', C.c_int32),
+                ('fold_w', C.c_void_p), ('fold_cout', C.c_int32), ('fold_out', C.c_void_p)]
 
 
 class WgradDesc(C.Structure):
@@ -54,7 +55,7 @@
 
 OP_CONV3X3, OP_PACK_NCHW, OP_UNPACK_GRAD_NCHW, OP_ACT_COMBINE, OP_PIXEL_UNSHUFFLE, OP_GRAD_ABSMAX, OP_GRAD_SCALE, OP_WGRAD_BATCH_RUN, \
     OP_PACK_BATCH_RUN, OP_ZERO, OP_UNPACK_NCHW, OP_WGRAD, OP_BN_REDUCE, OP_BN_APPLY, OP_BN_FINALIZE, OP_BN_PARAM_GRADS, \
-    OP_BN_FINALIZE_APPLY = range(1, 18)
+    OP_BN_FINALIZE_APPLY, OP_FOLD_SUM = range(1, 19)
 
 
 class CmdPackNchw(C.Structure):
@@ -99,6 +100,11 @@
 
 class CmdUnpackNchw(C.Structure):
     _fields_ = [('src', ActView), ('B', C.c_int32), ('nc', C.c_int32), ('dst', C.c_void_p)]
+
+
+class CmdFoldSum(C.Structure):
+    _fields_ = [('P', C.c_void_p), ('bias', C.c_void_p), ('B', C.c_int32), ('C', C.c_int32), ('H', C.c_int32), ('W', C.c_int32),
+                ('reverse_order', C.c_int32), ('out', C.c_void_p)]
 
 
 class CmdBn(C.Structure):
@@ -124,7 +130,7 @@
     _fields_ = [('conv', Conv3x3Desc), ('pack_nchw', CmdPackNchw), ('unpack_grad_nchw', CmdUnpackGradNchw), ('act_combine', CmdActCombine),
                 ('pixel_unshuffle', CmdPixelUnshuffle), ('grad_absmax', CmdGradAbsmax), ('grad_scale', CmdGradScale),
                 ('wgrad_batch_run', CmdWgradBatchRun), ('pack_batch_run', CmdPackBatchRun), ('zero', CmdZero), ('unpack_nchw', CmdUnpackNchw),
-                ('wgrad', WgradDesc), ('bn', CmdBn), ('bn_finalize', CmdBnFinalize), ('bn_param_grads', CmdBnParamGrads), ('bn_finalize_apply', CmdBnFinalizeApply)]
+                ('fold_sum', CmdFoldSum), ('wgrad', WgradDesc), ('bn', CmdBn), ('bn_finalize', CmdBnFinalize), ('bn_param_grads', CmdBnParamGrads), ('bn_finalize_apply', CmdBnFinalizeApply)]
 
 
 class Cmd(C.Structure):
@@ -134,7 +140,8 @@
 CMD_MEMBER = {OP_CONV3X3: 'conv', OP_PACK_NCHW: 'pack_nchw', OP_UNPACK_GRAD_NCHW: 'unpack_grad_nchw', OP_ACT_COMBINE: 'act_combine',
               OP_PIXEL_UNSHUFFLE: 'pixel_unshuffle', OP_GRAD_ABSMAX: 'grad_absmax', OP_GRAD_SCALE: 'grad_scale',
               OP_WGRAD_BATCH_RUN: 'wgrad_batch_run', OP_PACK_BATCH_RUN: 'pack_batch_run', OP_ZERO: 'zero', OP_UNPACK_NCHW: 'unpack_nchw',
-              OP_WGRAD: 'wgrad', OP_BN_REDUCE: 'bn', OP_BN_APPLY: 'bn', OP_BN_FINALIZE: 'bn_finalize', OP_BN_PARAM_GRADS: 'bn_param_grads', OP_BN_FINALIZE_APPLY: 'bn_finalize_apply'}
+              OP_WGRAD: 'wgrad', OP_BN_REDUCE: 'bn', OP_BN_APPLY: 'bn', OP_BN_FINALIZE: 'bn_finalize', OP_BN_PARAM_GRADS: 'bn_param_grads', OP_BN_FINALIZE_APPLY: 'bn_finalize_apply',
+              OP_FOLD_SUM: 'fold_sum'}
 
 
 _SIGS = {
@@ -152,6 +159,7 @@
     'esr_cmd_bytes': (C.c_int64, []),
     'esr_version': (C.c_int, []),
     'esr_conv3x3': (C.c_int, [C.POINTER(Conv3x3Desc), C.c_void_p]),
+    'esr_conv3x3_fold_sum': (C.c_int, [C.c_void_p, C.c_void_p, C.c_int, C.c_int, C.c_int, C.c_int, C.c_int, C.c_void_p, C.c_void_p]),
     'esr_conv3x3_tiling': (C.c_int, [C.POINTER(Conv3x3Desc), C.POINTER(C.c_int32)]),
     'esr_pixel_unshuffle': (C.c_int, [C.POINTER(ActView), C.c_int, C.POINTER(ActView), C.c_int, C.c_void_p]),
     'esr_conv_wpack_bytes': (C.c_size_t, [C.c_int, C.c_int, C.c_int]),
@@ -294,6 +302,7 @@
 ESR_OK, ESR_E_ARG, ESR_E_UNSUPPORTED, ESR_E_LAUNCH = 0, -1, -2, -3
 PIXELS_FLOAT, PIXELS_ROUND, PIXELS_RAW = 0, 1, 2
 PACK_FOLD2 = 2
+PACK_FOLD_TAPS = 6
 _ERR = {-1: 'ESR_E_ARG (bad argument)', -2: 'ESR_E_UNSUPPORTED (unsupported shape)', -3: 'ESR_E_LAUNCH (HIP launch error)'}
 
 
diff --git a/explorable-super-resolution_amd/esr_hip/act.py b/explorable-super-resolution_amd/esr_hip/act.py
--- a/explorable-super-resolution_amd/esr_hip/act.py
+++ b/explorable-super-resolution_amd/esr_hip/act.py
@@ -424,6 +424,27 @@
         self._bind_bias(32 * (len(self.parts) // 2), dev)
 
 
+class PackedConvFold(_Pack):
+
+    def __init__(self, weight, split=True):
+        super().__init__(split, False, None)
+        self.weight = weight
+        self.fold_cout = weight.shape[0]
+        assert 9 * self.fold_cout <= 32, 'the nine taps of every output channel are rows of one 32-row tile'
+
+    def _build(self, dev):
+        cout, cin = self.weight.shape[0], self.weight.shape[1]
+        self.ncg_in, self.mtiles = (cin + 7) // 8, 1
+        self.kmap = torch.tensor([c if c < cin else -1 for c in range(self.ncg_in * 8)], dtype=torch.int32, device=dev)
+        self.mmap = torch.tensor([r % cout if r < 9 * cout else -1 for r in range(32)], dtype=torch.int32, device=dev)
+        self.wpack = torch.empty(_lib.lib.esr_conv_wpack_bytes(self.ncg_in, 32, fmt_code(self.split)) // 9, dtype=torch.uint8, device=dev)
+        self._bind_bias(32, dev)
+
+    def jobs(self):
+        self._wd = _fp32(self.weight)
+        return [(self._wd, self.kmap, self.ncg_in, self.mmap, 1, _lib.PACK_FOLD_TAPS, 1.0, self.wpack.data_ptr())]
+
+
 def run_pack_jobs(jobs, split):
     for wd, kmap, ncg_in, mmap, mtiles, transposed, scale, dst in jobs:
         check(_lib.lib.esr_pack_conv_weights(wd.data_ptr(), wd.shape[0], wd.shape[1], kmap.data_ptr(), ncg_in, mmap.data_ptr(), mtiles,
@@ -536,8 +557,11 @@
 
 def conv3x3(pc, in1, B, H, W, cout, in0=None, upsample=1, act_slope=1.0, alpha=1.0, res1=None, beta1=0.0, res2=None, beta2=0.0,
             out=None, out2=None, out_nchw=None, use_bias=True, mask_src=None, mask_cg=(0, 0), mask_slope=0.2, reverse=None, in1_lo_groups=0,
-            pixel_shuffle=0, ps_rowgroup0=0, tap_mask_k=None, tap_mask_k_shift=0, tap_mask_m=None, k_split_ws=None, name=None, upsample_phases=0):
+            pixel_shuffle=0, ps_rowgroup0=0, tap_mask_k=None, tap_mask_k_shift=0, tap_mask_m=None, k_split_ws=None, name=None, upsample_phases=0,
+            fold=None, fold_out=None):
     d = _lib.Conv3x3Desc()
+    if fold is not None:
+        d.fold_w, d.fold_cout, d.fold_out = fold.wpack.data_ptr(), fold.fold_cout, fold_out.data_ptr()
     d.upsample_phases = upsample_phases
     if _range_watch is not None:
         d.range_flag, d.range_tag = _range_watch.flag.data_ptr(), len(_range_watch.names)
@@ -583,6 +607,21 @@
     check(_lib.lib.esr_conv3x3(C.byref(d), stream_ptr()), 'esr_conv3x3')
 
 
+def fold_sum(P, bias, out, reverse=None):
+    B, C_, H, W = out.shape
+    assert tuple(P.shape) == (B, 9 * C_, H, W) and P.dtype == out.dtype == torch.float32 and P.is_contiguous() and out.is_contiguous()
+    global _launch_parity
+    if reverse is None:
+        reverse = bool(_launch_parity & 1)
+        _launch_parity += 1
+    bp = bias.data_ptr() if bias is not None else None
+    rec = _rec()
+    if rec is not None:
+        rec.emit(_lib.OP_FOLD_SUM, _lib.CmdFoldSum(P.data_ptr(), bp, B, C_, H, W, 1 if reverse else 0, out.data_ptr()), ('out',))
+        return
+    check(_lib.lib.esr_conv3x3_fold_sum(P.data_ptr(), bp, B, C_, H, W, 1 if reverse else 0, out.data_ptr(), stream_ptr()), 'esr_conv3x3_fold_sum')
+
+
 def pixel_unshuffle(src, r, dst, B):
     rec = _rec()
     if rec is not None:
diff --git a/explorable-super-resolution_amd/esr_hip/engine.py b/explorable-super-resolution_amd/esr_hip/engine.py
--- a/explorable-super-resolution_amd/esr_hip/engine.py
+++ b/explorable-super-resolution_amd/esr_hip/engine.py
@@ -153,6 +153,11 @@
             return self.split
         return 'f16x2' if rdb else 'f16x3'
 
+    def _folds_out(self):
+        net = self.net
+        lat_hr = net.latent_input is not None and net.num_latent_channels > 0 and net._lat_all_layers
+        return net.nf == 64 and not lat_hr and 9 * net.out_nc <= 32 and self.split in (True, 'mixed', 'f16')
+
     @property
     def _pshuf(self):
         return 0 if self.net.upsample_mode == 'upconv' else (3 if self.net.upscale == 3 else 2)
@@ -176,6 +181,8 @@
                     d[name] = A.PackedConvSlices(c.weight, c.bias, lat, split=self._wfmt(name.startswith('rrdb')))
                 else:
                     d[name] = A.PackedConv(c.weight, c.bias, lat, split=self._wfmt(name.startswith('rrdb')))
+                if name == 'hr1' and self._folds_out():
+                    d[name, 'fold'] = A.PackedConvFold(c.weight, split=self._wfmt(False))
             self._packed = d
             self._pack_sets += 1
             self._pack_gen[0] = self._pack_sets
@@ -272,7 +279,10 @@
             s *= 3 if sf == 3 else 2
             ups.append(A.ActBuf(B, ng, s * h, s * w, dev, sp))
         d['ups'] = ups
-        d['hr0'] = A.ActBuf(B, ng, sf * h, sf * w, dev, sp)
+        if keep is False and self._folds_out():
+            d['fold'] = torch.empty(B, 9 * net.out_nc, sf * h, sf * w, dtype=torch.float32, device=dev)
+        else:
+            d['hr0'] = A.ActBuf(B, ng, sf * h, sf * w, dev, sp)
         d['_plans'] = {}
         return d
 
@@ -397,8 +407,12 @@
                 conv(pk[('up%d' % j, 'taps9') if f == 2 else 'up%d' % j], src.view(), B, s * h, s * w, nf, upsample=f, act_slope=0.2, out=bufs['ups'][j].view(),
                      name='upconv%d' % j)
             src = bufs['ups'][j]
-        conv(pk['hr0'], src.view(), B, H, W, nf, in0=zhr, act_slope=0.2, out=bufs['hr0'].view(), name='HR_conv0')
-        conv(pk['hr1'], bufs['hr0'].view(), B, H, W, net.out_nc, in0=zhr, out_nchw=g)
+        if keep is False and self._folds_out():
+            conv(pk['hr0'], src.view(), B, H, W, nf, act_slope=0.2, fold=pk['hr1', 'fold'], fold_out=bufs['fold'], name='HR_conv0')
+            A.fold_sum(bufs['fold'], pk['hr1'].bias, g)
+        else:
+            conv(pk['hr0'], src.view(), B, H, W, nf, in0=zhr, act_slope=0.2, out=bufs['hr0'].view(), name='HR_conv0')
+            conv(pk['hr1'], bufs['hr0'].view(), B, H, W, net.out_nc, in0=zhr, out_nchw=g)
         A.host_op(lambda ctx: self._ev and self._ev[1].record())
 
     @A.one_stream
diff --git a/include/esr_hip.h b/include/esr_hip.h
--- a/include/esr_hip.h
+++ b/include/esr_hip.h
@@ -58,10 +58,15 @@
     uint32_t* range_flag;
     uint32_t range_tag;
     int32_t upsample_phases;
+    const void* fold_w;
+    int32_t fold_cout;
+    float* fold_out;
 } esr_conv3x3_desc;
 
 int esr_conv3x3(const esr_conv3x3_desc* d, esr_stream_t stream);
 
+int esr_conv3x3_fold_sum(const float* P, const float* bias, int B, int C, int H, int W, int reverse_order, float* out, esr_stream_t stream);
+
 int esr_conv3x3_tiling(const esr_conv3x3_desc* d, int32_t* tiling);
 
 int esr_pixel_unshuffle(const esr_act_view* src, int r, const esr_act_view* dst, int B, esr_stream_t stream);
@@ -69,6 +74,7 @@
 size_t esr_conv_wpack_bytes(int ncg_in, int cout, int split);
 
 #define ESR_PACK_FOLD2 2
+#define ESR_PACK_FOLD_TAPS 6
 int esr_pack_conv_weights(const float* w, int cout_w, int cin_w, const int32_t* kmap, int ncg_in,
                           const int32_t* mmap, int mtiles, int transposed, int split, float scale, void* wpack,
                           esr_stream_t stream);
@@ -230,7 +236,7 @@
     ESR_OP_CONV3X3 = 1, ESR_OP_PACK_NCHW = 2, ESR_OP_UNPACK_GRAD_NCHW = 3, ESR_OP_ACT_COMBINE = 4, ESR_OP_PIXEL_UNSHUFFLE = 5,
     ESR_OP_GRAD_ABSMAX = 6, ESR_OP_GRAD_SCALE = 7, ESR_OP_WGRAD_BATCH_RUN = 8, ESR_OP_PACK_BATCH_RUN = 9, ESR_OP_ZERO = 10,
     ESR_OP_UNPACK_NCHW = 11, ESR_OP_WGRAD = 12, ESR_OP_BN_REDUCE = 13, ESR_OP_BN_APPLY = 14, ESR_OP_BN_FINALIZE = 15, ESR_OP_BN_PARAM_GRADS = 16,
-    ESR_OP_BN_FINALIZE_APPLY = 17
+    ESR_OP_BN_FINALIZE_APPLY = 17, ESR_OP_FOLD_SUM = 18
 };
 typedef struct { const float* src; int64_t src_batch_stride; int32_t B, C, h, w, c0, nc, pad, down; esr_act_view dst; } esr_cmd_pack_nchw;
 typedef struct { esr_act_view G; float* dst; int64_t dst_batch_stride; int32_t B, C, h, w, c0, nc, pad, down, accumulate; } esr_cmd_unpack_grad_nchw;
@@ -242,6 +248,7 @@
 typedef struct { const void* workspace; int32_t n; int64_t nblocks; } esr_cmd_pack_batch_run;
 typedef struct { void* p; int64_t n16; } esr_cmd_zero;
 typedef struct { esr_act_view src; int32_t B, nc; float* dst; } esr_cmd_unpack_nchw;
+typedef struct { const float* P; const float* bias; int32_t B, C, H, W, reverse_order; float* out; } esr_cmd_fold_sum;
 typedef struct { esr_bn_desc d; int32_t mode; double* sums; } esr_cmd_bn;
 typedef struct { const double* sums; int32_t groups, C; int64_t n_per_group; float eps, momentum; const float* gamma; const float* beta;
                  float* mean; float* rstd; float* scale; float* shift; float* running_mean; float* running_var; } esr_cmd_bn_finalize;
@@ -264,6 +271,7 @@
         esr_cmd_pack_batch_run pack_batch_run;
         esr_cmd_zero zero;
         esr_cmd_unpack_nchw unpack_nchw;
+        esr_cmd_fold_sum fold_sum;
         esr_wgrad_desc wgrad;
         esr_cmd_bn bn;
         esr_cmd_bn_finalize bn_finalize;
```
